# Li-Yuetao/ActiveSplat

Measured on AMD Instinct MI355X. Metric: render+backward frames/sec at 640x480, N Gaussians, higher is better.
Workload: dtype f32; 1 GPU; BASELINE configs[2]'s render (the north star's target configuration): 2000000 Gaussians, SH degree 3, 640x480, forward (colour+radii+depth+opacity) + backward (all input gradients), frames strictly one after the other; gaussians=2000000, sh_degree=3, width=640, height=480, tile_instances_D=4842856, streams=1, parallelism=single GPU

## Files before the change

activesplat_amd/_lib.py:

```python
from __future__ import annotations

import ctypes as C
import os

_HERE = os.path.dirname(os.path.abspath(__file__))
LIB_PATH = os.path.join(_HERE, "libgsplat_hip.so")

_lib = None
_emulated = False


class GsCamera(C.Structure):
    _fields_ = [("image_width", C.c_int32), ("image_height", C.c_int32), ("sh_degree", C.c_int32),
                ("sh_coeffs", C.c_int32), ("tanfovx", C.c_float), ("tanfovy", C.c_float),
                ("scale_modifier", C.c_float), ("num_views", C.c_int32), ("bg", C.c_void_p),
                ("viewmatrix", C.c_void_p), ("projmatrix", C.c_void_p), ("campos", C.c_void_p)]


class GsGeomLayout(C.Structure):
    _fields_ = [(n, C.c_uint64) for n in ("total_bytes", "geom", "rect", "tiles_touched", "offsets", "block_sums", "clamped",
                                          "tile_total", "tile_base", "sh_jac", "depth_bits")]


class GsImageLayout(C.Structure):
    _fields_ = [(n, C.c_uint64) for n in ("total_bytes", "ranges", "final_T", "n_contrib", "split_state")]


class GsAdamTensor(C.Structure):
    _fields_ = [("n", C.c_int64), ("param", C.c_void_p), ("grad", C.c_void_p), ("exp_avg", C.c_void_p), ("exp_avg_sq", C.c_void_p),
                ("lr", C.c_double), ("beta1", C.c_double), ("beta2", C.c_double), ("eps", C.c_double), ("step", C.c_int32),
                ("reserved", C.c_int32)]


class GsRowTensor(C.Structure):
    _fields_ = [("param", C.c_void_p), ("exp_avg", C.c_void_p), ("exp_avg_sq", C.c_void_p), ("grad", C.c_void_p),
                ("lr", C.c_double), ("beta1", C.c_double), ("beta2", C.c_double), ("eps", C.c_double), ("width", C.c_int32),
                ("step", C.c_int32)]


class GsBinLayout(C.Structure):
    _fields_ = [(n, C.c_uint64) for n in ("total_bytes", "path", "pairs", "keys_unsorted", "vals_unsorted", "keys_sorted",
                                          "sort_temp", "segments", "seg_T", "pairs_alt")]


class GsDbscanLayout(C.Structure):
    _fields_ = [(n, C.c_uint64) for n in ("total_bytes", "mask_bits", "core_bits", "root_bits", "word_prefix", "parent", "root", "row_range")]


class GsEvalLayout(C.Structure):
    _fields_ = [("total_bytes", C.c_uint64), ("ms_ssim_defined", C.c_int32), ("levels", C.c_int32), ("level_width", C.c_int32 * 5),
                ("level_height", C.c_int32 * 5)]


class GsHullLayout(C.Structure):
    _fields_ = [(n, C.c_uint64) for n in ("total_bytes", "cluster_status")]


class GsMeshLayout(C.Structure):
    _fields_ = [(n, C.c_uint64) for n in ("total_bytes", "total", "records", "rects", "tile_count", "tile_offset", "list")]


class GsImageGrads(C.Structure):
    _fields_ = [(n, C.c_void_p) for n in ("dL_dcolor", "dL_ddepth", "dL_dopacity", "dL_ddepth_sq")]


SORT_AUTO, SORT_TILE_LDS, SORT_RADIX = 0, 1, 2


ABI_VERSION = 23

vp, i32, u32, i64, u64, f32, f64, cint = C.c_void_p, C.c_int32, C.c_uint32, C.c_int64, C.c_uint64, C.c_float, C.c_double, C.c_int

BINDINGS = {
    "gs_atlas_layout": (cint, [i32, i32, i32, C.POINTER(i32), C.POINTER(i32), C.POINTER(i32)]),
    "gs_geom_layout": (cint, [i32, i32, i32, C.POINTER(GsGeomLayout)]),
    "gs_image_layout": (cint, [i32, i32, C.POINTER(GsImageLayout)]),
    "gs_bin_layout": (cint, [i64, u32, i32, i32, C.POINTER(GsBinLayout)]),
    "gs_set_sort_path": (cint, [i32]),
    "gs_set_forward_segments": (cint, [i32]),
    "gs_set_half_quadrants": (cint, [i32]),
    "gs_set_backward_chain": (cint, [i32, i32]),
    "gs_set_backward_chain_tickets": (cint, [i32]),
    "gs_set_backward_chain_polls": (cint, [i32]),
    "gs_set_forward_priority": (cint, [i32, f32]),
    "gs_async_status_word": (cint, [C.POINTER(C.POINTER(u32))]),
    "gs_async_status_clear": (cint, []),
    "gs_recorded_cut": (cint, [u32, C.POINTER(u32), C.POINTER(i32)]),
    "gs_set_backward_segments": (cint, [i32]),
    "gs_backward_scratch_bytes": (u64, [i32]),
    "gs_last_error": (C.c_char_p, []),
    "gs_version": (C.c_char_p, []),
    "gs_abi_version": (i32, []),
    "gs_profile_enable": (cint, [i32]),
    "gs_profile_stage_count": (i32, []),
    "gs_profile_stage_name": (C.c_char_p, [i32]),
    "gs_profile_collect": (cint, [vp, vp, i32]),
    "gs_preprocess_forward": (cint, [C.POINTER(GsCamera), i32] + [vp] * 12 + [i32, vp]),
    "gs_render_forward": (cint, [C.POINTER(GsCamera), i32, i64, u32] + [vp] * 10),
    "gs_render_backward": (cint, [C.POINTER(GsCamera), i32, i64] + [vp] * 21 + [i32, i32, vp]),
    "gs_preprocess_forward_raw": (cint, [C.POINTER(GsCamera), i32] + [vp] * 7 + [i32] + [vp] * 7 + [i32, vp]),
    "gs_render_backward_raw": (cint, [C.POINTER(GsCamera), i32, i64] + [vp] * 7 + [i32, i32] + [vp] * 14 + [i32, i32, vp]),
    "gs_pose_grad_scratch_bytes": (u64, [i32]),
    "gs_render_backward_raw_pose": (cint, [C.POINTER(GsCamera), i32, i64] + [vp] * 7 + [i32, i32] + [vp] * 14 + [i32, i32, i32, vp, vp, vp]),
    "gs_render_backward_grads": (cint, [C.POINTER(GsCamera), i32, i64] + [vp] * 10 + [C.POINTER(GsImageGrads)] + [vp] * 9 + [i32, i32, vp]),
    "gs_render_backward_raw_grads": (cint, [C.POINTER(GsCamera), i32, i64] + [vp] * 7 + [i32, i32] + [vp] * 4 + [C.POINTER(GsImageGrads)] + [vp] * 8 + [i32, i32, vp]),
    "gs_render_backward_raw_pose_grads": (cint, [C.POINTER(GsCamera), i32, i64] + [vp] * 7 + [i32, i32] + [vp] * 4 + [C.POINTER(GsImageGrads)] + [vp] * 8 + [i32, i32, i32, vp, vp, vp]),
    "gs_adam_step": (cint, [i64] + [vp] * 4 + [f64] * 4 + [i32, vp]),
    "gs_adam_step_multi": (cint, [i32, C.POINTER(GsAdamTensor), vp]),
    "gs_render_backward_raw_adam": (cint, [C.POINTER(GsCamera), i32, i64] + [vp] * 7 + [i32] + [vp] * 8 + [i32, i32, C.POINTER(GsAdamTensor), vp]),
    "gs_pack_columns": (cint, [i32, C.POINTER(GsRowTensor), i64, i64, vp, vp]),
    "gs_adam_rows": (cint, [i32, C.POINTER(GsRowTensor), i64, i64, i64, vp, vp, vp]),
    "gs_unpack_columns": (cint, [i32, C.POINTER(GsRowTensor), i64, vp, vp]),
    "gs_activate_forward": (cint, [i32, i32] + [vp] * 10),
    "gs_activate_backward": (cint, [i32, i32] + [vp] * 13),
    "gs_activate_backward_accumulate": (cint, [i32, i32] + [vp] * 13),
    "gs_activate_backward_pose": (cint, [i32, i32] + [vp] * 13 + [i32, i32, vp, vp, vp]),
    "gs_mapping_loss_scratch_bytes": (u64, [i32, i32]),
    "gs_mapping_loss": (cint, [i32, i32] + [vp] * 5 + [f32, f32] + [vp] * 4 + [i64, vp]),
    "gs_depth_error_median_scratch_bytes": (u64, [i32, i32]),
    "gs_depth_error_median": (cint, [i32, i32] + [vp] * 5),
    "gs_depth_error_median_grid": (cint, [i32, i32] + [vp] * 4 + [i32, vp]),
    "gs_depth_error_median_workgroups": (i32, [i32, i32]),
    "gs_mapping_loss_outlier": (cint, [i32, i32] + [vp] * 5 + [f32, f32] + [vp] * 4 + [i64, vp, vp]),
    "gs_tracking_loss_scratch_bytes": (u64, [i32, i32]),
    "gs_tracking_loss": (cint, [i32, i32] + [vp] * 6 + [i32, f32, f32, f32] + [vp] * 5),
    "gs_tracking_loss_outlier": (cint, [i32, i32] + [vp] * 6 + [i32, f32, f32, f32] + [vp] * 6),
    "gs_preprocess_forward_raw_dev": (cint, [C.POINTER(GsCamera), i32] + [vp] * 8 + [i64, i64, i32] + [vp] * 7 + [i32, vp]),
    "gs_preprocess_forward_topdown": (cint, [C.POINTER(GsCamera), i32] + [vp] * 5 + [i32, f32, f32] + [vp] * 6),
    "gs_render_forward_topdown": (cint, [C.POINTER(GsCamera), i32, i64, u32] + [vp] * 9),
    "gs_render_backward_raw_pose_dev": (cint, [C.POINTER(GsCamera), i32, i64] + [vp] * 8 + [i64, i64, i32] + [vp] * 8 + [i32, i32, vp, vp, vp]),
    "gs_tracking_state_bytes": (u64, []),
    "gs_tracking_begin": (cint, [vp, vp, i64, i64, vp, vp]),
    "gs_tracking_step": (cint, [i32, vp, i32, i32, vp, f32, f32, vp, vp, i64, i64, f64, f64, i32, vp, vp, vp]),
    "gs_compact_scratch_bytes": (u64, [i64]),
    "gs_compact_index": (cint, [i64] + [vp] * 5),
    "gs_gather_rows": (cint, [i64, i32] + [vp] * 4),
    "gs_gather_rows_zero_tail": (cint, [i64, i64, i32] + [vp] * 4),
    "gs_densify_classify": (cint, [i32, i32] + [vp] * 5 + [f32, f32, i32, i32] + [vp] * 5),
    "gs_densify_children": (cint, [i32, i32, i32, vp, vp, u64, vp, vp, vp]),
    "gs_compact3_scratch_bytes": (u64, [i64]),
    "gs_compact_index3": (cint, [i64, vp, vp, vp, i32] + [vp] * 4),
    "gs_visibility_stats": (cint, [i32] + [vp] * 4),
    "gs_accumulate_grad2d": (cint, [i32] + [vp] * 5),
    "gs_grid_dbscan_layout": (cint, [i32] * 4 + [C.POINTER(GsDbscanLayout)]),
    "gs_grid_dbscan": (cint, [i32, i32, i32, vp, i64, i64, f32] + [i32] * 4 + [vp] * 7),
    "gs_cluster_hulls_layout": (cint, [i32] * 5 + [C.POINTER(GsHullLayout)]),
    "gs_cluster_hulls": (cint, [i32, i32, i32, vp, vp, i64, i64, vp, vp, i32, C.POINTER(u32), i32, i32, f32, f64, f64, i32] + [vp] * 8),
    "gs_high_loss_grid": (cint, [i32, i32, vp, vp, vp, f32, f32, i32, i32, vp, vp, vp]),
    "gs_grow_scratch_bytes": (u64, [i32, i32]),
    "gs_grow_gaussians": (cint, [i32, i32] + [vp] * 6 + [f32, i32] + [vp] * 8),
    "gs_keyframe_overlap": (cint, [i32, vp, i32, vp, vp, i32, i32, i32, vp, vp]),
    "gs_frame_ingest": (cint, [i32, i32, vp, vp, vp, i32, C.POINTER(i32)] + [vp] * 5),
    "gs_mesh_render_layout": (cint, [i32, i32, i32, u32, C.POINTER(GsMeshLayout)]),
    "gs_mesh_render": (cint, [i32, vp, i32, vp, vp, C.POINTER(f32), C.POINTER(f32), f32, i32, i32, vp, u32, vp, vp, vp, vp, vp]),
    "gs_depth_cloud": (cint, [i32, i32, vp, C.POINTER(f32), C.POINTER(f32), vp, vp, vp]),
    "gs_cloud_nearest_scratch_bytes": (u64, [i64, i64]),
    "gs_cloud_nearest": (cint, [i64, vp, vp, i64, vp, vp, i32, vp, vp, vp]),
    "gs_completion_row_scratch_bytes": (u64, []),
    "gs_completion_row": (cint, [i64, vp, i64, vp, vp, f64, vp, vp, vp]),
    "gs_eval_frame_layout": (cint, [i32, i32, i32, C.POINTER(GsEvalLayout)]),
    "gs_eval_frame": (cint, [i32, i32] + [vp] * 5 + [f32, i32, vp, vp, vp]),
}

SYMBOLS = tuple(BINDINGS)


def _bind(lib):
# ... 95 lines not shown
```

activesplat_amd/csrc/api.hip:

```cpp
#include <stdio.h>
#include <string.h>

#include <mutex>

#include "gs_common.h"

namespace {

thread_local char g_err[512] = "";

int fail(int code, const char* fmt, const char* a = "")
{
    snprintf(g_err, sizeof(g_err), fmt, a);
    return code;
}

int launched(const char* who, const char* what, hipError_t e)
{
    if (e == hipSuccess) return GS_OK;
    snprintf(g_err, sizeof(g_err), "%s: %s%s%s", who, what, *what ? " " : "", hipGetErrorString(e));
    return GS_ELAUNCH;
}

bool adam_aligned16(const void* p, const void* g, const void* m, const void* v)
{
    return (((uintptr_t)p | (uintptr_t)g | (uintptr_t)m | (uintptr_t)v) & 15u) == 0;
}

int fail_adam_alignment(const char* who, int tensor)
{
    snprintf(g_err, sizeof(g_err), "%s: tensor %d: param / grad / exp_avg / exp_avg_sq must be 16-byte aligned (the kernel makes 128-bit accesses)", who, tensor);
    return GS_EINVAL;
}

uint64_t align_up(uint64_t v, uint64_t a = 256) { return (v + a - 1) / a * a; }

enum Stage { ST_PREPROCESS = 0, ST_TILE_COUNT, ST_EMIT, ST_SORT, ST_RANGES, ST_TILE_SCATTER_SORT, ST_BLEND_FWD, ST_BLEND_BWD, ST_PREPROCESS_BWD, ST_ADAM, ST_COUNT };
const char* kStageNames[ST_COUNT] = {"preprocess_forward+scan", "tile_count+scan", "emit", "sort", "ranges",
                                     "tile_scatter+sort", "blend_forward", "blend_backward", "preprocess_backward", "adam"};
std::atomic<int> g_sort_path{GS_SORT_AUTO};
std::atomic<bool> g_segments_enabled{true};

int choose_path(int tiles, uint32_t max_tile_instances)
{
    const bool fits = tiles <= gs::kMaxLdsTiles && max_tile_instances <= 65535u * (uint32_t)gs::kSortChunk;
    if (g_sort_path == GS_SORT_RADIX) return GS_SORT_RADIX;
    return fits ? GS_SORT_TILE_LDS : GS_SORT_RADIX;
}
constexpr int kMaxPairs = 8192;
struct Prof {
    bool on = false;
    int n = 0;
    hipEvent_t ev[kMaxPairs][2];
    int stage[kMaxPairs];
    int created = 0;
} g_prof;

struct ScopedStage {
    int idx = -1;
    hipStream_t st;
    ScopedStage(int stage, hipStream_t s) : st(s)
    {
        if (!g_prof.on || g_prof.n >= kMaxPairs) return;
        idx = g_prof.n++;
        if (idx >= g_prof.created) { (void)hipEventCreate(&g_prof.ev[idx][0]); (void)hipEventCreate(&g_prof.ev[idx][1]); g_prof.created = idx + 1; }
        g_prof.stage[idx] = stage;
        (void)hipEventRecord(g_prof.ev[idx][0], st);
    }
    ~ScopedStage() { if (idx >= 0) (void)hipEventRecord(g_prof.ev[idx][1], st); }
};

int tile_bits(int tiles)
{
    int b = 1;
    while ((1 << b) < tiles) b++;
    return b;
}

int32_t tiles_across(int32_t pixels) { return (pixels + gs::kTile - 1) / gs::kTile; }
uint64_t tiles_of(int32_t width, int32_t height) { return (uint64_t)tiles_across(width) * tiles_across(height); }
int32_t atlas_view_stride(int32_t view_width, int32_t V) { return V > 1 ? tiles_across(view_width) * gs::kTile : view_width; }
int32_t blocks_of(int32_t P) { return (P + gs::kBlock - 1) / gs::kBlock; }
int32_t virtual_rows(int32_t P, int32_t V) { return V > 1 ? V * blocks_of(P) * gs::kBlock : P; }

bool make_cam(const GsCamera* c, gs::Cam& k)
{
    if (!c || c->image_width <= 0 || c->image_height <= 0 || !c->bg || !c->viewmatrix || !c->projmatrix) return false;
    if (!(c->tanfovx > 0.f) || !(c->tanfovy > 0.f)) return false;
    if (c->num_views < 0 || c->num_views > 64) return false;
    k.V = c->num_views > 1 ? c->num_views : 1;
    k.Wv = c->image_width; k.H = c->image_height;
    k.gxv = tiles_across(k.Wv);
    k.gx = k.V * k.gxv; k.gy = tiles_across(k.H);
    k.W = k.V * atlas_view_stride(k.Wv, k.V);
    k.nbv = 0;
    if (k.gx >= 65536 || k.gy >= 65536) return false;
    k.tanfovx = c->tanfovx; k.tanfovy = c->tanfovy;
    k.fx = (float)k.Wv / (2.0f * c->tanfovx); k.fy = (float)k.H / (2.0f * c->tanfovy);
    k.mod = c->scale_modifier;
    k.sh_degree = c->sh_degree; k.sh_coeffs = c->sh_coeffs;
    k.bg = c->bg; k.view = c->viewmatrix; k.proj = c->projmatrix; k.campos = c->campos;
    k.half = 0; k.split = 0;
    k.act = k.act_iso = k.act_accumulate = 0;
    return true;
}

int32_t virtual_count(gs::Cam& k, int32_t P)
{
    k.nbv = blocks_of(P);
    return virtual_rows(P, k.V);
}

gs::GeomPtrs carve_geom(void* base, int32_t P, const gs::Cam& k)
{
    GsGeomLayout L;
    gs_geom_layout(P, k.W, k.H, &L);
    char* b = (char*)base;
    gs::GeomPtrs g;
    g.geom = (float4*)(b + L.geom); g.rect = (uint2*)(b + L.rect); g.tiles = (uint32_t*)(b + L.tiles_touched);
    g.offsets = (uint32_t*)(b + L.offsets); g.block_sums = (uint32_t*)(b + L.block_sums);
    g.clamped = (uint32_t*)(b + L.clamped);
    g.tile_total = (uint32_t*)(b + L.tile_total); g.tile_base = (uint32_t*)(b + L.tile_base);
    g.sh_jac = (float2*)(b + L.sh_jac);
    g.depth_bits = (uint32_t*)(b + L.depth_bits);
    g.vis_max = nullptr; g.vis_seen = nullptr;
    return g;
}

}

extern "C" {

const char* gs_last_error(void) { return g_err; }
const char* gs_version(void) { return "activesplat_amd gsplat_hip 0.4 (gfx950)"; }
int32_t gs_abi_version(void) { return GS_ABI_VERSION; }

int gs_profile_enable(int32_t on)
{
    g_prof.on = on != 0;
    g_prof.n = 0;
    return GS_OK;
}

int32_t gs_profile_stage_count(void) { return ST_COUNT; }

const char* gs_profile_stage_name(int32_t stage) { return stage >= 0 && stage < ST_COUNT ? kStageNames[stage] : ""; }

int gs_profile_collect(float* ms_sum, int32_t* calls, int32_t n_stages)
{
    if (!ms_sum || !calls || n_stages < ST_COUNT) return fail(GS_EINVAL, "gs_profile_collect: bad argument");
    for (int i = 0; i < n_stages; i++) { ms_sum[i] = 0.f; calls[i] = 0; }
    for (int i = 0; i < g_prof.n; i++) {
        if (hipEventSynchronize(g_prof.ev[i][1]) != hipSuccess) return fail(GS_ELAUNCH, "gs_profile_collect: event sync failed");
        float ms = 0.f;
        if (hipEventElapsedTime(&ms, g_prof.ev[i][0], g_prof.ev[i][1]) != hipSuccess) return fail(GS_ELAUNCH, "gs_profile_collect: elapsed failed");
        ms_sum[g_prof.stage[i]] += ms; calls[g_prof.stage[i]]++;
    }
    g_prof.n = 0;
    return GS_OK;
}

int gs_set_sort_path(int32_t path)
{
    if (path < GS_SORT_AUTO || path > GS_SORT_RADIX) return fail(GS_EINVAL, "gs_set_sort_path: bad path");
    g_sort_path = path;
    return GS_OK;
}

int gs_set_half_quadrants(int32_t max_tiles)
{
    gs::g_half_quadrant_tiles = max_tiles < 0 ? 0 : max_tiles;
    return GS_OK;
}

int gs_set_backward_chain(int32_t pieces, int32_t min_tiles)
{
    if (pieces < 1 || pieces > gs::kChainPieces) return fail(GS_EINVAL, "gs_set_backward_chain: pieces out of range");
    gs::g_chain_pieces = pieces;
    gs::g_chain_min_tiles = min_tiles < 0 ? gs::kChainMinTiles : min_tiles;
    return GS_OK;
}

int gs_set_backward_chain_tickets(int32_t on)
{
    gs::g_chain_tickets = on != 0;
    return GS_OK;
}

int gs_set_backward_chain_polls(int32_t polls)
{
    gs::g_chain_polls = polls == -1 ? gs::kChainPollsDefault : polls;
    return GS_OK;
}

int gs_set_forward_priority(int32_t mode, float param)
{
    if (mode > gs::kFwdPrioChunk) return fail(GS_EINVAL, "gs_set_forward_priority: mode out of range");
    if (mode == gs::kFwdPrioT && param >= 1.0f) return fail(GS_EINVAL, "gs_set_forward_priority: a transmittance threshold lies below 1");
    if (mode < 0) { mode = gs::kFwdPrioDefault; param = gs::kFwdPrioDefaultParam; }
    gs::g_fwd_prio_param = param > 0.0f ? param : 0.0f;
    gs::g_fwd_prio = mode;
    return GS_OK;
}

int gs_async_status_word(uint32_t** host_word)
{
    static uint32_t* word = nullptr;
    static std::mutex mu;
    std::lock_guard<std::mutex> lock(mu);
    if (!word) {
        void* h = nullptr;
        if (hipHostMalloc(&h, 64, hipHostMallocMapped | hipHostMallocPortable) != hipSuccess) {
            (void)hipGetLastError();
            return fail(GS_ELAUNCH, "gs_async_status_word: hipHostMalloc failed");
        }
        memset(h, 0, 64);
        void* d = nullptr;
        if (hipHostGetDevicePointer(&d, h, 0) != hipSuccess) { (void)hipGetLastError(); return fail(GS_ELAUNCH, "gs_async_status_word: no device view of the host word"); }
        void* f = nullptr;
        if (hipMalloc(&f, 64) == hipSuccess && hipMemset(f, 0, 64) == hipSuccess && hipGetDevice(&gs::g_chain_fail_device) == hipSuccess) gs::g_chain_fail_dev = (uint32_t*)f;
        else (void)hipGetLastError();
        word = (uint32_t*)h;
        gs::g_async_status_dev = (uint32_t*)d;
    }
    if (host_word) *host_word = word;
    return GS_OK;
}

int gs_async_status_clear(void)
{
    if (hipDeviceSynchronize() != hipSuccess) { (void)hipGetLastError(); return fail(GS_ELAUNCH, "gs_async_status_clear: device synchronisation failed"); }
    if (gs::g_chain_fail_dev && hipMemset(gs::g_chain_fail_dev, 0, 4) != hipSuccess) { (void)hipGetLastError(); return fail(GS_ELAUNCH, "gs_async_status_clear: hipMemset failed"); }
    return GS_OK;
}

int gs_recorded_cut(uint32_t target, uint32_t* nearest, int32_t* level)
{
    const uint32_t pos = gs::cut_nearest(target);
    if (nearest) *nearest = pos;
    if (level) *level = pos ? gs::cut_level(pos) : -1;
    return GS_OK;
}

int gs_set_backward_segments(int32_t segments)
{
    if (segments < 1 || segments > gs::kFewSegmentsMax) return fail(GS_EINVAL, "gs_set_backward_segments: 1, 2 or 3");
    gs::g_few_segments = segments;
    return GS_OK;
}

int gs_set_forward_segments(int32_t on)
{
    g_segments_enabled = on != 0;
    return GS_OK;
}

int gs_atlas_layout(int32_t P, int32_t view_width, int32_t num_views, int32_t* virtual_P, int32_t* atlas_width, int32_t* view_stride)
{
    if (P < 0 || view_width <= 0 || num_views < 1 || num_views > 64) return fail(GS_EINVAL, "gs_atlas_layout: bad argument");
    const int32_t stride = atlas_view_stride(view_width, num_views);
    if (virtual_P) *virtual_P = virtual_rows(P, num_views);
    if (atlas_width) *atlas_width = num_views * stride;
    if (view_stride) *view_stride = stride;
    return GS_OK;
}

int gs_geom_layout(int32_t P, int32_t width, int32_t height, GsGeomLayout* out)
{
    if (!out || P < 0 || width <= 0 || height <= 0) return fail(GS_EINVAL, "gs_geom_layout: bad argument");
    const uint64_t n = (uint64_t)(P > 0 ? P : 1);
    const uint64_t nb = (n + gs::kBlock - 1) / gs::kBlock;
    const uint64_t tiles = tiles_of(width, height);
    const uint64_t rows = (n + 1023) / 1024;
    uint64_t o = 0;
    out->geom = o; o = align_up(o + n * GS_GEOM_FLOATS * 4);
    out->rect = o; o = align_up(o + n * 8);
    out->tiles_touched = o; o = align_up(o + n * 4);
    out->offsets = o; o = align_up(o + n * 4);
    out->block_sums = o; o = align_up(o + (nb + 1) * 4);
    out->clamped = o; o = align_up(o + n * 4);
    out->tile_total = o; o = align_up(o + tiles * 4);
    out->tile_base = o; o = align_up(o + (tiles <= (uint64_t)gs::kMaxLdsTiles ? rows * tiles * 4 : 4));
    out->sh_jac = o; o = align_up(o + n * gs::kShJacFloats * 4);
    out->depth_bits = o; o = align_up(o + n * 4);
    out->total_bytes = o;
    return GS_OK;
}

int gs_image_layout(int32_t width, int32_t height, GsImageLayout* out)
{
    if (!out || width <= 0 || height <= 0) return fail(GS_EINVAL, "gs_image_layout: bad argument");
    const uint64_t tiles = tiles_of(width, height);
    const uint64_t hw = (uint64_t)width * height;
    uint64_t o = 0;
    out->ranges = o; o = align_up(o + tiles * 8);
    out->final_T = o; o = align_up(o + hw * 4);
    out->n_contrib = o; o = align_up(o + hw * 4);
    out->split_state = o; o = align_up(o + (tiles <= (uint64_t)gs::kFewTiles ? ((uint64_t)gs::kCutLevels * 5 + 4) * hw + 4
                                             : (uint64_t)gs::chain_state_words(tiles)) * 4);
    out->total_bytes = o;
    return GS_OK;
}

int gs_bin_layout(int64_t D, uint32_t max_tile_instances, int32_t width, int32_t height, GsBinLayout* out)
{
    if (!out || D < 0 || width <= 0 || height <= 0) return fail(GS_EINVAL, "gs_bin_layout: bad argument");
    const int tiles = (int)tiles_of(width, height);
    const uint64_t n = (uint64_t)(D > 0 ? D : 1);
    memset(out, 0, sizeof(*out));
    out->path = (uint64_t)choose_path(tiles, max_tile_instances);
    uint64_t o = 0;
    if (out->path == GS_SORT_TILE_LDS) {
        out->pairs = o; o = align_up(o + n * 8);
        if (max_tile_instances > (uint32_t)gs::kSortCapMax) { out->pairs_alt = o; o = align_up(o + n * 8); }
    } else {
        out->keys_unsorted = o; o = align_up(o + n * 8);
        out->vals_unsorted = o; o = align_up(o + n * 4);
        out->keys_sorted = o; o = align_up(o + n * 8);
        out->sort_temp = o; o = align_up(o + gs::sort_temp_bytes(D, 32 + tile_bits(tiles)));
    }
    out->segments = 1;
    const bool few_tiles = tiles * 4 * 8 <= gs::kWaveSlots && max_tile_instances >= 8192;
    const bool long_lists = tiles * 4 * 2 <= gs::kWaveSlots && max_tile_instances >= 32768;
    if (g_segments_enabled && max_tile_instances != 0xffffffffu && (few_tiles || long_lists)) {
        uint64_t S = 3 * (uint64_t)gs::kWaveSlots / ((uint64_t)tiles * 4);
        const uint64_t by_len = max_tile_instances / 1024;
        if (S > by_len) S = by_len;
        if (S > 32) S = 32;
        if (S >= 2) { out->segments = S; out->seg_T = o; o = align_up(o + (uint64_t)tiles * S * gs::kBlock * 4 + (uint64_t)tiles * 16); }
    }
    out->total_bytes = o;
    return GS_OK;
}

uint64_t gs_backward_scratch_bytes(int32_t P) { return align_up((uint64_t)(P > 0 ? P : 1) * gs::kGradStride * 4); }

static void set_input_activation(gs::Cam& k, const gs::PoseRequest& pose, int32_t isotropic, int32_t accumulate)
{
    static const float world[7] = {1.f, 0.f, 0.f, 0.f, 0.f, 0.f, 0.f};
    const float* p = pose.source == gs::POSE_HOST ? pose.pose7 : world;
    k.act = pose.source != gs::POSE_NONE;
    k.act_iso = k.act && isotropic != 0; k.act_accumulate = k.act && accumulate != 0;
    for (int c = 0; c < 4; c++) k.act_q[c] = p[c];
    for (int c = 0; c < 3; c++) k.act_t[c] = p[4 + c];
}

static bool dev_pose(const float* cam_unnorm_rots, const float* cam_trans, int64_t num_frames, int64_t time_idx, gs::DevPose& dp)
{
    if (!cam_unnorm_rots || !cam_trans || num_frames < 1 || time_idx < 0 || time_idx >= num_frames) return false;
    dp.q = cam_unnorm_rots + time_idx; dp.t = cam_trans + time_idx; dp.stride = num_frames;
    return true;
}

static gs::CamDP with_dev_pose(const gs::Cam& k, const gs::DevPose& dp)
{
    gs::CamDP kd;
    static_cast<gs::Cam&>(kd) = k;
    kd.dev_q = dp.q; kd.dev_t = dp.t; kd.stride = dp.stride;
    return kd;
}

struct ForwardCall {
    int32_t P;
    gs::GaussianInputs in;
    gs::PoseRequest pose;
    int32_t isotropic;
    float* max_2D_radius; uint8_t* seen;
    int32_t* radii;
    void* geom_state; void* image_state;
    uint32_t* d_counts; uint32_t* h_counts;
    int32_t want_backward;
};

static int preprocess_forward_impl(const GsCamera* cam, const ForwardCall& c, gs_stream_t stream)
{
    const gs::GaussianInputs& in = c.in;
    const int32_t P = c.P;
    gs::Cam k;
    if (!make_cam(cam, k)) return fail(GS_EINVAL, "gs_preprocess_forward: invalid camera settings");
    set_input_activation(k, c.pose, c.isotropic, 0);
    if (k.act && k.V != 1) return fail(GS_EINVAL, "gs_preprocess_forward_raw: one view only");
    if (k.act && (in.cov3D || (in.shs && k.sh_coeffs != 16)))
        return fail(GS_EINVAL, "gs_preprocess_forward_raw: scale / rotation parameters with colours or 16-coefficient SH rows only");
    if (P < 0 || !c.geom_state || !c.image_state || !c.d_counts) return fail(GS_EINVAL, "gs_preprocess_forward: null state pointer");
    if (P > 0 && (!in.means3D || !in.opac || !c.radii)) return fail(GS_EINVAL, "gs_preprocess_forward: null input pointer");
    if ((in.shs == nullptr) == (in.colors == nullptr) && P > 0)
        return fail(GS_EINVAL, "Please provide excatly one of either SHs or precomputed colors!");
    const bool have_sr = in.scales != nullptr && in.rots != nullptr;
    if (P > 0 && (have_sr == (in.cov3D != nullptr) || ((in.scales != nullptr) != (in.rots != nullptr))))
        return fail(GS_EINVAL, "Please provide exactly one of either scale/rotation pair or precomputed 3D covariance!");
    if (in.shs && (k.sh_degree < 0 || k.sh_degree > 3 || k.sh_coeffs < (k.sh_degree + 1) * (k.sh_degree + 1) || k.sh_coeffs > 16 || !k.campos))
        return fail(GS_EINVAL, "gs_preprocess_forward: sh_degree / sh_coeffs / campos inconsistent");
    hipStream_t st = (hipStream_t)stream;
    const int32_t Pv = virtual_count(k, P);
    gs::GeomPtrs gp = carve_geom(c.geom_state, Pv, k);
    if (!(c.want_backward && in.shs)) gp.sh_jac = nullptr;
    gp.vis_max = k.act ? c.max_2D_radius : nullptr; gp.vis_seen = k.act ? c.seen : nullptr;
    GsImageLayout IL; gs_image_layout(k.W, k.H, &IL);
    uint2* ranges = (uint2*)((char*)c.image_state + IL.ranges);
    const int tiles = k.gx * k.gy;
    hipError_t e;
    {
        ScopedStage ps(ST_PREPROCESS, st);
        if (c.pose.source == gs::POSE_BAND) {
            gs::CamBand kb;
            static_cast<gs::Cam&>(kb) = k;
            kb.band_upper = c.pose.band_upper; kb.band_lower = c.pose.band_lower;
            e = gs::launch_preprocess_forward(kb, P, in, c.radii, gp, st);
        } else if (c.pose.source == gs::POSE_DEVICE)
            e = gs::launch_preprocess_forward(with_dev_pose(k, c.pose.dev), P, in, c.radii, gp, st);
        else
            e = gs::launch_preprocess_forward(k, P, in, c.radii, gp, st);
    }
    if (int rc = launched("gs_preprocess_forward", "", e)) return rc;
    bool mirrored = false;
    if (tiles <= gs::kMaxLdsTiles) {
        uint32_t* host_dev = nullptr;
        if (c.h_counts && hipHostGetDevicePointer((void**)&host_dev, c.h_counts, 0) != hipSuccess) { host_dev = nullptr; (void)hipGetLastError(); }
        mirrored = host_dev != nullptr;
        ScopedStage ps(ST_TILE_COUNT, st);
        e = gs::launch_tile_count(k, Pv, gp, gp.tile_total, gp.tile_base, ranges, c.d_counts, host_dev, st);
        if (int rc = launched("gs_preprocess_forward", "tile count", e)) return rc;
    } else {
        e = gs::launch_scan_block_sums(Pv, gp, c.d_counts, st);
        if (int rc = launched("gs_preprocess_forward", "scan", e)) return rc;
        e = hipMemsetAsync(c.d_counts + 1, 0xff, sizeof(uint32_t), st);
        if (int rc = launched("gs_preprocess_forward", "memset", e)) return rc;
    }
    if (c.h_counts && !mirrored) {
        e = hipMemcpyAsync(c.h_counts, c.d_counts, 2 * sizeof(uint32_t), hipMemcpyDeviceToHost, st);
        if (int rc = launched("gs_preprocess_forward", "D2H", e)) return rc;
    }
    return GS_OK;
}

int gs_preprocess_forward(const GsCamera* cam, int32_t P, const float* means3D, const float* shs,
                          const float* colors_precomp, const float* opacities, const float* scales,
                          const float* rotations, const float* cov3D_precomp, int32_t* radii, void* geom_state,
                          void* image_state, uint32_t* d_counts, uint32_t* h_counts, int32_t want_backward, gs_stream_t stream)
{
    ForwardCall c{};
    c.in.means3D = means3D; c.in.shs = shs; c.in.colors = colors_precomp; c.in.opac = opacities; c.in.scales = scales; c.in.rots = rotations;
    c.in.cov3D = cov3D_precomp; c.P = P;
    c.radii = radii; c.geom_state = geom_state; c.image_state = image_state; c.d_counts = d_counts; c.h_counts = h_counts; c.want_backward = want_backward;
    return preprocess_forward_impl(cam, c, stream);
}

int gs_preprocess_forward_raw(const GsCamera* cam, int32_t P, const float* means3D, const float* shs, const float* colors_precomp,
                              const float* logit_opacities, const float* log_scales, const float* unnorm_rotations,
                              const float* h_pose7, int32_t isotropic, float* max_2D_radius, uint8_t* seen, int32_t* radii, void* geom_state,
                              void* image_state, uint32_t* d_counts, uint32_t* h_counts, int32_t want_backward, gs_stream_t stream)
{
    if (!h_pose7) return fail(GS_EINVAL, "gs_preprocess_forward_raw: null pose");
    ForwardCall c{};
    c.in.means3D = means3D; c.in.shs = shs; c.in.colors = colors_precomp; c.in.opac = logit_opacities; c.in.scales = log_scales; c.in.rots = unnorm_rotations;
    c.P = P; c.pose.source = gs::POSE_HOST; c.pose.pose7 = h_pose7; c.isotropic = isotropic; c.max_2D_radius = max_2D_radius; c.seen = seen;
    c.radii = radii; c.geom_state = geom_state; c.image_state = image_state; c.d_counts = d_counts; c.h_counts = h_counts; c.want_backward = want_backward;
    return preprocess_forward_impl(cam, c, stream);
}

int gs_preprocess_forward_raw_dev(const GsCamera* cam, int32_t P, const float* means3D, const float* shs, const float* colors_precomp,
                                  const float* logit_opacities, const float* log_scales, const float* unnorm_rotations,
                                  const float* cam_unnorm_rots, const float* cam_trans, int64_t num_frames, int64_t time_idx, int32_t isotropic,
                                  float* max_2D_radius, uint8_t* seen, int32_t* radii, void* geom_state, void* image_state, uint32_t* d_counts,
                                  uint32_t* h_counts, int32_t want_backward, gs_stream_t stream)
{
    ForwardCall c{};
    c.pose.source = gs::POSE_DEVICE;
    if (!dev_pose(cam_unnorm_rots, cam_trans, num_frames, time_idx, c.pose.dev))
        return fail(GS_EINVAL, "gs_preprocess_forward_raw_dev: null pose columns or time index outside [0, num_frames)");
    if (P > 0 && (!log_scales || !unnorm_rotations)) return fail(GS_EINVAL, "gs_preprocess_forward_raw_dev: null scale / rotation parameters");
    c.in.means3D = means3D; c.in.shs = shs; c.in.colors = colors_precomp; c.in.opac = logit_opacities; c.in.scales = log_scales; c.in.rots = unnorm_rotations;
    c.P = P; c.isotropic = isotropic; c.max_2D_radius = max_2D_radius; c.seen = seen;
    c.radii = radii; c.geom_state = geom_state; c.image_state = image_state; c.d_counts = d_counts; c.h_counts = h_counts; c.want_backward = want_backward;
    return preprocess_forward_impl(cam, c, stream);
}

static int bin_tile_lists(const char* who, const gs::Cam& k, int32_t P, int64_t D, uint32_t max_tile_instances, gs::GeomPtrs gp, uint2* ranges,
                          const GsBinLayout& BL, char* bb, uint32_t* point_list, hipStream_t st)
{
    hipError_t e;
    if (BL.path == GS_SORT_TILE_LDS) {
        if (D > 0) {
            ScopedStage ps(ST_TILE_SCATTER_SORT, st);
            e = gs::launch_tile_scatter_sort(k, P, gp, gp.tile_base, ranges, max_tile_instances,
                                             (unsigned long long*)(bb + BL.pairs), (unsigned long long*)(bb + BL.pairs_alt), point_list, (uint32_t)D, st);
            if (int rc = launched(who, "tile scatter/sort", e)) return rc;
        }
    } else {
        e = hipMemsetAsync(ranges, 0, (size_t)k.gx * k.gy * 8, st);
        if (int rc = launched(who, "memset", e)) return rc;
        if (k.gx * k.gy <= gs::kMaxLdsTiles) {
            e = gs::launch_scan_block_sums(P, gp, gp.block_sums + (P + gs::kBlock - 1) / gs::kBlock, st);
            if (int rc = launched(who, "scan", e)) return rc;
        }
        if (D == 0) {
            e = gs::launch_emit(k, P, gp, nullptr, nullptr, st);
            if (int rc = launched(who, "emit", e)) return rc;
        } else {
            uint64_t* ku = (uint64_t*)(bb + BL.keys_unsorted); uint32_t* vu = (uint32_t*)(bb + BL.vals_unsorted);
            uint64_t* ks = (uint64_t*)(bb + BL.keys_sorted);
            { ScopedStage ps(ST_EMIT, st); e = gs::launch_emit(k, P, gp, ku, vu, st); }
            if (int rc = launched(who, "emit", e)) return rc;
            const int end_bit = 32 + tile_bits(k.gx * k.gy);
            {
                ScopedStage ps(ST_SORT, st);
                e = gs::sort_pairs(bb + BL.sort_temp, (size_t)(BL.total_bytes - BL.sort_temp), ku, ks, vu, point_list, D, end_bit, st);
            }
            if (int rc = launched(who, "sort", e)) return rc;
            { ScopedStage ps(ST_RANGES, st); e = gs::launch_ranges(D, ks, ranges, st); }
            if (int rc = launched(who, "ranges", e)) return rc;
        }
    }
    return GS_OK;
}

int gs_render_forward(const GsCamera* cam, int32_t P, int64_t D, uint32_t max_tile_instances, void* geom_state,
                      void* bin_state, uint32_t* point_list, void* image_state, float* out_color, float* out_depth,
                      float* out_opacity, float* out_depth_sq, void* backward_scratch, gs_stream_t stream)
{
    gs::Cam k;
    if (!make_cam(cam, k)) return fail(GS_EINVAL, "gs_render_forward: invalid camera settings");
    if (P < 0 || D < 0 || !geom_state || !image_state || !out_color || !out_depth || !out_opacity)
        return fail(GS_EINVAL, "gs_render_forward: null pointer");
    if (D > 0 && (!bin_state || !point_list)) return fail(GS_EINVAL, "gs_render_forward: null binning workspace");
    if (D >= (int64_t)1 << 32) return fail(GS_ECAPACITY, "gs_render_forward: more than 2^32 tile instances");
    hipStream_t st = (hipStream_t)stream;
    const int32_t Pin = P;
    P = virtual_count(k, Pin);
    gs::GeomPtrs gp = carve_geom(geom_state, P, k);
    GsImageLayout IL; gs_image_layout(k.W, k.H, &IL);
    char* ib = (char*)image_state;
    uint2* ranges = (uint2*)(ib + IL.ranges);
    GsBinLayout BL; gs_bin_layout(D, max_tile_instances, k.W, k.H, &BL);
    char* bb = (char*)bin_state;
    if (int rc = bin_tile_lists("gs_render_forward", k, P, D, max_tile_instances, gp, ranges, BL, bb, point_list, st)) return rc;
    ScopedStage ps(ST_BLEND_FWD, st);
    return launched("gs_render_forward", "blend", gs::launch_blend_forward(k, ranges, point_list, gp.geom, out_color, out_depth, out_opacity,
                    (float*)(ib + IL.final_T), (uint32_t*)(ib + IL.n_contrib), out_depth_sq, BL.path == GS_SORT_TILE_LDS ? (uint32_t)D : 0xffffffffu,
                    (int)BL.segments, BL.segments > 1 ? (float*)(bb + BL.seg_T) : nullptr, (float*)(ib + IL.split_state), (uint32_t)P,
                    (float*)backward_scratch, st));
}

int gs_preprocess_forward_topdown(const GsCamera* cam, int32_t P, const float* means3D, const float* colors_precomp, const float* logit_opacities,
                                  const float* log_scales, const float* unnorm_rotations, int32_t isotropic, float band_upper, float band_lower,
                                  int32_t* radii, void* geom_state, void* image_state, uint32_t* d_counts, uint32_t* h_counts, gs_stream_t stream)
{
    if (cam && cam->num_views > 1) return fail(GS_EINVAL, "gs_preprocess_forward_topdown: one view only");
    if (P > 0 && (!colors_precomp || !log_scales || !unnorm_rotations))
        return fail(GS_EINVAL, "gs_preprocess_forward_topdown: null colour / scale / rotation parameters");
    if (band_upper != band_upper || band_lower != band_lower) return fail(GS_EINVAL, "gs_preprocess_forward_topdown: NaN height band");
    ForwardCall c{};
    c.in.means3D = means3D; c.in.colors = colors_precomp; c.in.opac = logit_opacities; c.in.scales = log_scales; c.in.rots = unnorm_rotations;
    c.P = P; c.pose.source = gs::POSE_BAND; c.pose.band_upper = band_upper; c.pose.band_lower = band_lower; c.isotropic = isotropic;
    c.radii = radii; c.geom_state = geom_state; c.image_state = image_state; c.d_counts = d_counts; c.h_counts = h_counts;
    return preprocess_forward_impl(cam, c, stream);
}

int gs_render_forward_topdown(const GsCamera* cam, int32_t P, int64_t D, uint32_t max_tile_instances, void* geom_state, void* bin_state,
                              uint32_t* point_list, void* image_state, float* free_opacity, uint8_t* free_map_binary, uint8_t* visible_rgb,
                              uint8_t* visible_map_binary, gs_stream_t stream)
{
    gs::Cam k;
    if (!make_cam(cam, k)) return fail(GS_EINVAL, "gs_render_forward_topdown: invalid camera settings");
    if (k.V != 1) return fail(GS_EINVAL, "gs_render_forward_topdown: one view only");
    if (P < 0 || D < 0 || !geom_state || !image_state || !free_opacity || !free_map_binary || !visible_rgb || !visible_map_binary)
        return fail(GS_EINVAL, "gs_render_forward_topdown: null pointer");
    if (((uintptr_t)free_map_binary | (uintptr_t)visible_rgb | (uintptr_t)visible_map_binary | (uintptr_t)free_opacity) & 3)
        return fail(GS_EINVAL, "gs_render_forward_topdown: output maps must be 4-byte aligned");
    if (D > 0 && (!bin_state || !point_list)) return fail(GS_EINVAL, "gs_render_forward_topdown: null binning workspace");
    if (D >= (int64_t)1 << 32) return fail(GS_ECAPACITY, "gs_render_forward_topdown: more than 2^32 tile instances");
    hipStream_t st = (hipStream_t)stream;
    virtual_count(k, P);
    gs::GeomPtrs gp = carve_geom(geom_state, P, k);
    GsImageLayout IL; gs_image_layout(k.W, k.H, &IL);
    uint2* ranges = (uint2*)((char*)image_state + IL.ranges);
    GsBinLayout BL; gs_bin_layout(D, max_tile_instances, k.W, k.H, &BL);
    if (int rc = bin_tile_lists("gs_render_forward_topdown", k, P, D, max_tile_instances, gp, ranges, BL, (char*)bin_state, point_list, st)) return rc;
    ScopedStage ps(ST_BLEND_FWD, st);
    return launched("gs_render_forward_topdown", "blend", gs::launch_blend_topdown(k, ranges, point_list, gp.geom, free_opacity, free_map_binary, visible_rgb,
                    visible_map_binary, BL.path == GS_SORT_TILE_LDS ? (uint32_t)D : 0xffffffffu, (uint32_t)P, st));
}

struct BackwardCall {
    int32_t P;
    int64_t D;
    gs::GaussianBackward g;
    gs::PoseRequest pose;
    int32_t isotropic, accumulate;
    const void* geom_state; const uint32_t* point_list; const void* image_state;
    const float* dL_dcolor; const float* dL_ddepth;
    const float* dL_dopacity; const float* dL_ddepth_sq;
    void* scratch; int32_t scratch_zeroed, have_sh_jacobian;
    const GsAdamTensor* adam5;
};

static int render_backward_impl(const GsCamera* cam, const BackwardCall& c, gs_stream_t stream)
{
    gs::GaussianBackward g = c.g;
    const gs::GaussianInputs& in = g.in;
    const gs::GaussianGrads& out = g.out;
    const gs::PoseRequest& pose = c.pose;
    const int32_t P = c.P;
    const bool pose_only = pose.grad == gs::POSE_GRAD_ONLY;
    gs::Cam k;
    if (!make_cam(cam, k)) return fail(GS_EINVAL, "gs_render_backward: invalid camera settings");
    set_input_activation(k, pose, c.isotropic, pose_only ? 0 : c.accumulate);
    if (k.act && k.V != 1) return fail(GS_EINVAL, "gs_render_backward_raw: one view only");
    if (k.act && (!in.opac || in.cov3D || (in.shs && k.sh_coeffs != 16)))
        return fail(GS_EINVAL, "gs_render_backward_raw: scale / rotation parameters with colours or 16-coefficient SH rows only");
    if (k.V > 1) return fail(GS_EINVAL, "gs_render_backward: multi-view atlas renders are forward-only");
    if (P < 0 || c.D < 0 || !c.geom_state || !c.image_state || !c.dL_dcolor || !c.scratch)
        return fail(GS_EINVAL, "gs_render_backward: null pointer");
    if (pose.grad && (!k.act || c.adam5 || (!pose.dL_dpose7 && pose.source != gs::POSE_DEVICE) || !pose.pose_scratch))
        return fail(GS_EINVAL, "gs_render_backward_raw_pose: raw-parameter mode with a pose-gradient output and its scratch only");
    if (pose.source == gs::POSE_DEVICE && !pose_only) return fail(GS_EINVAL, "gs_render_backward_raw_pose_dev: the pose-only backward only");
    if ((c.dL_dopacity || c.dL_ddepth_sq) && (c.adam5 || pose.source == gs::POSE_DEVICE))
        return fail(GS_EINVAL, "gs_render_backward: opacity / depth_sq gradients have no optimiser-step or device-pose form");
    if (P == 0) {
        if (pose.grad && pose.dL_dpose7)
            return launched("gs_render_backward_raw_pose", "memset", hipMemsetAsync(pose.dL_dpose7, 0, 7 * sizeof(float), (hipStream_t)stream));
        return GS_OK;
    }
    gs::FusedAdam fa{};
    if (c.adam5) {
        if (!k.act || c.accumulate) return fail(GS_EINVAL, "gs_render_backward_raw_adam: raw-parameter mode without accumulation only");
        if (!in.means3D || !g.radii || !out.dmeans2D || !in.scales || !in.rots || (in.shs == nullptr) == (in.colors == nullptr))
            return fail(GS_EINVAL, "gs_render_backward_raw_adam: null input/output pointer");
        if (in.shs && !c.have_sh_jacobian) return fail(GS_EINVAL, "gs_render_backward_raw_adam: SH rows need the forward's saved Jacobian (have_sh_jacobian = 1)");
        const float* par[5] = {in.means3D, in.opac, in.scales, in.rots, in.shs ? in.shs : in.colors};
        const int64_t width[5] = {3, 1, c.isotropic ? 1 : 3, 4, in.shs ? 48 : 3};
        for (int t = 0; t < 5; ++t) {
            const GsAdamTensor& a = c.adam5[t];
            if (a.param != par[t] || !a.exp_avg || !a.exp_avg_sq || a.step < 1 || a.n != width[t] * (int64_t)P)
                return fail(GS_EINVAL, "gs_render_backward_raw_adam: descriptor of %s does not describe the input tensor (param / moments / n / step)",
                            t == 0 ? "means3D" : t == 1 ? "logit_opacities" : t == 2 ? "log_scales" : t == 3 ? "unnorm_rotations" : "the colours");
            if (P > 0 && (t == 3 || (t == 4 && in.shs)) && !adam_aligned16(a.param, a.param, a.exp_avg, a.exp_avg_sq))
                return fail_adam_alignment("gs_render_backward_raw_adam", t);
            fa.p[t] = a.param; fa.m[t] = a.exp_avg; fa.v[t] = a.exp_avg_sq;
            fa.c[t] = gs::adam_coef(a.lr, a.beta1, a.beta2, a.eps, a.step);
        }
        fa.fail = gs::chain_fail_word();
        g.adam = &fa;
    } else if (pose_only) {
        if (!in.means3D || !g.radii || !out.dmeans2D || !in.scales || !in.rots || (in.shs == nullptr) == (in.colors == nullptr))
            return fail(GS_EINVAL, "gs_render_backward_raw_pose: null input/output pointer");
    } else {
        if (!in.means3D || !g.radii || !out.dmeans2D || !out.dmeans3D || !out.dopac)
            return fail(GS_EINVAL, "gs_render_backward: null input/output pointer");
        if (in.shs ? !out.dshs : !out.dcolors) return fail(GS_EINVAL, "gs_render_backward: missing colour gradient output");
        if (in.cov3D ? !out.dcov3D : (!in.scales || !in.rots || !out.dscales || !out.drots))
            return fail(GS_EINVAL, "gs_render_backward: missing covariance inputs/outputs");
    }
    hipStream_t st = (hipStream_t)stream;
    gs::GeomPtrs gp = carve_geom(const_cast<void*>(c.geom_state), P, k);
    GsImageLayout IL; gs_image_layout(k.W, k.H, &IL);
    const char* ib = (const char*)c.image_state;
    float* grad2d = (float*)c.scratch;
    hipError_t e = c.scratch_zeroed ? hipSuccess : hipMemsetAsync(grad2d, 0, (size_t)P * gs::kGradStride * 4, st);
    if (int rc = launched("gs_render_backward", "memset", e)) return rc;
    if (c.D > 0) {
        ScopedStage ps(ST_BLEND_BWD, st);
        e = gs::launch_blend_backward(k, (const uint2*)(ib + IL.ranges), c.point_list, gp.geom,
                                      (const float*)(ib + IL.split_state),
                                      (const float*)(ib + IL.final_T),
                                      (const uint32_t*)(ib + IL.n_contrib), c.dL_dcolor, c.dL_ddepth, grad2d, st, c.dL_dopacity, c.dL_ddepth_sq);
        if (int rc = launched("gs_render_backward", "blend", e)) return rc;
    }
    g.clamped = gp.clamped; g.sh_jac = (in.shs && c.have_sh_jacobian) ? gp.sh_jac : nullptr; g.grad2d = grad2d;
    {
        ScopedStage ps(ST_PREPROCESS_BWD, st);
        if (pose.source == gs::POSE_DEVICE) e = gs::launch_preprocess_backward(with_dev_pose(k, pose.dev), P, g, pose, st);
        else e = gs::launch_preprocess_backward(k, P, g, pose, st);
    }
    if (int rc = launched("gs_render_backward", "preprocess", e)) return rc;
    const int64_t pose_rows = gs::pose_rows_count(P);
    if (pose.source == gs::POSE_DEVICE) {
        if (pose.dL_dpose7)
            return launched("gs_render_backward_raw_pose_dev", "pose reduction", gs::launch_pose_grad_finish_dev(pose_rows, pose.dev.q, pose.dev.stride,
                            (const float*)pose.pose_scratch, pose.dL_dpose7, st));
    } else if (pose.grad)
        return launched("gs_render_backward_raw_pose", "pose reduction", gs::launch_pose_grad_finish(pose_rows, pose.pose7, (const float*)pose.pose_scratch,
                        pose.dL_dpose7, st));
    return GS_OK;
}

int gs_render_backward_grads(const GsCamera* cam, int32_t P, int64_t D, const float* means3D, const float* shs,
                       const float* colors_precomp, const float* scales, const float* rotations,
                       const float* cov3D_precomp, const int32_t* radii, const void* geom_state,
                       const uint32_t* point_list, const void* image_state, const GsImageGrads* grads, float* dL_dmeans2D, float* dL_dmeans3D, float* dL_dopacities, float* dL_dcolors_precomp,
                       float* dL_dshs, float* dL_dscales, float* dL_drotations, float* dL_dcov3D, void* scratch,
                       int32_t scratch_zeroed, int32_t have_sh_jacobian, gs_stream_t stream)
{
    if (!grads) return fail(GS_EINVAL, "gs_render_backward_grads: null image-gradient block");
    BackwardCall c{};
    c.P = P; c.D = D;
    c.g.in.means3D = means3D; c.g.in.shs = shs; c.g.in.colors = colors_precomp; c.g.in.scales = scales; c.g.in.rots = rotations; c.g.in.cov3D = cov3D_precomp;
    c.g.radii = radii; c.geom_state = geom_state; c.point_list = point_list; c.image_state = image_state; c.dL_dcolor = grads->dL_dcolor; c.dL_ddepth = grads->dL_ddepth; c.dL_dopacity = grads->dL_dopacity; c.dL_ddepth_sq = grads->dL_ddepth_sq;
    c.g.out.dmeans2D = dL_dmeans2D; c.g.out.dmeans3D = dL_dmeans3D; c.g.out.dopac = dL_dopacities; c.g.out.dcolors = dL_dcolors_precomp;
    c.g.out.dshs = dL_dshs; c.g.out.dscales = dL_dscales; c.g.out.drots = dL_drotations; c.g.out.dcov3D = dL_dcov3D;
    c.scratch = scratch; c.scratch_zeroed = scratch_zeroed; c.have_sh_jacobian = have_sh_jacobian;
    return render_backward_impl(cam, c, stream);
}

int gs_render_backward(const GsCamera* cam, int32_t P, int64_t D, const float* means3D, const float* shs,
                       const float* colors_precomp, const float* scales, const float* rotations,
                       const float* cov3D_precomp, const int32_t* radii, const void* geom_state,
                       const uint32_t* point_list, const void* image_state, const float* dL_dcolor,
                       const float* dL_ddepth, float* dL_dmeans2D, float* dL_dmeans3D, float* dL_dopacities, float* dL_dcolors_precomp,
                       float* dL_dshs, float* dL_dscales, float* dL_drotations, float* dL_dcov3D, void* scratch,
                       int32_t scratch_zeroed, int32_t have_sh_jacobian, gs_stream_t stream)
{
    const GsImageGrads grads{dL_dcolor, dL_ddepth, nullptr, nullptr};
    return gs_render_backward_grads(cam, P, D, means3D, shs, colors_precomp, scales, rotations, cov3D_precomp, radii, geom_state, point_list, image_state, &grads, dL_dmeans2D, dL_dmeans3D, dL_dopacities, dL_dcolors_precomp, dL_dshs, dL_dscales, dL_drotations, dL_dcov3D, scratch, scratch_zeroed, have_sh_jacobian, stream);
}

int gs_render_backward_raw_grads(const GsCamera* cam, int32_t P, int64_t D, const float* means3D, const float* shs, const float* colors_precomp,
                           const float* logit_opacities, const float* log_scales, const float* unnorm_rotations, const float* h_pose7,
                           int32_t isotropic, int32_t accumulate, const int32_t* radii, const void* geom_state, const uint32_t* point_list,
                           const void* image_state, const GsImageGrads* grads, float* dL_dmeans2D, float* dL_dmeans3D,
                           float* dL_dlogit_opacities, float* dL_dcolors_precomp, float* dL_dshs, float* dL_dlog_scales,
                           float* dL_dunnorm_rotations, void* scratch, int32_t scratch_zeroed, int32_t have_sh_jacobian, gs_stream_t stream)
{
    if (!grads) return fail(GS_EINVAL, "gs_render_backward_raw_grads: null image-gradient block");
    if (!h_pose7 || (P > 0 && !logit_opacities)) return fail(GS_EINVAL, "gs_render_backward_raw: null pose / opacity parameters");
    BackwardCall c{};
    c.g.in.means3D = means3D; c.g.in.shs = shs; c.g.in.colors = colors_precomp; c.g.in.opac = logit_opacities; c.g.in.scales = log_scales; c.g.in.rots = unnorm_rotations;
    c.P = P; c.D = D; c.pose.source = gs::POSE_HOST; c.pose.pose7 = h_pose7; c.isotropic = isotropic; c.accumulate = accumulate;
    c.g.radii = radii; c.geom_state = geom_state; c.point_list = point_list; c.image_state = image_state; c.dL_dcolor = grads->dL_dcolor; c.dL_ddepth = grads->dL_ddepth; c.dL_dopacity = grads->dL_dopacity; c.dL_ddepth_sq = grads->dL_ddepth_sq;
    c.g.out.dmeans2D = dL_dmeans2D; c.g.out.dmeans3D = dL_dmeans3D; c.g.out.dopac = dL_dlogit_opacities; c.g.out.dcolors = dL_dcolors_precomp;
    c.g.out.dshs = dL_dshs; c.g.out.dscales = dL_dlog_scales; c.g.out.drots = dL_dunnorm_rotations;
    c.scratch = scratch; c.scratch_zeroed = scratch_zeroed; c.have_sh_jacobian = have_sh_jacobian;
    return render_backward_impl(cam, c, stream);
}

int gs_render_backward_raw(const GsCamera* cam, int32_t P, int64_t D, const float* means3D, const float* shs, const float* colors_precomp,
                           const float* logit_opacities, const float* log_scales, const float* unnorm_rotations, const float* h_pose7,
                           int32_t isotropic, int32_t accumulate, const int32_t* radii, const void* geom_state, const uint32_t* point_list,
                           const void* image_state, const float* dL_dcolor, const float* dL_ddepth, float* dL_dmeans2D, float* dL_dmeans3D,
                           float* dL_dlogit_opacities, float* dL_dcolors_precomp, float* dL_dshs, float* dL_dlog_scales,
                           float* dL_dunnorm_rotations, void* scratch, int32_t scratch_zeroed, int32_t have_sh_jacobian, gs_stream_t stream)
{
    const GsImageGrads grads{dL_dcolor, dL_ddepth, nullptr, nullptr};
    return gs_render_backward_raw_grads(cam, P, D, means3D, shs, colors_precomp, logit_opacities, log_scales, unnorm_rotations, h_pose7, isotropic, accumulate, radii, geom_state, point_list, image_state, &grads, dL_dmeans2D, dL_dmeans3D, dL_dlogit_opacities, dL_dcolors_precomp, dL_dshs, dL_dlog_scales, dL_dunnorm_rotations, scratch, scratch_zeroed, have_sh_jacobian, stream);
}
// ... 669 lines not shown
```

activesplat_amd/csrc/blend.hip:

```cpp
#include "gs_common.h"
#include <atomic>

namespace gs {

constexpr int kFwdStreams = 4;

constexpr float kAlphaMin = 1.0f / 255.0f;
constexpr float kTmin = 0.0001f;
constexpr float kLog2e = 1.4426950408889634f;
constexpr uint32_t kNoId = 0xffffffffu;

struct TileCtx {
    int tile, tx, ty, px, py, quad, seg;
    float qx0, qy0, pxf, pyf;
    bool inside;
};

template <int NW>
__device__ __forceinline__ bool tile_ctx_at(const Cam& cam, unsigned block, int wave, int lane, TileCtx& c, int segments = 0)
{
    const int G = (segments > 1 ? 4 * segments : 4) / NW;
    const int ntiles = cam.gx * cam.gy, per = (ntiles + 7) >> 3;
    const int idx = (int)(block >> 3);
    c.tile = (int)(block & 7) * per + idx / G;
// ... 143 lines not shown
template <bool DEPTH_SQ>
__device__ __forceinline__ void store_pixel_outputs(const Cam& cam, int px, int py, float T, uint32_t last, float C0, float C1, float C2, float Dp, float Dq,
                                                    float* out_color, float* out_depth, float* out_opacity, float* final_T, uint32_t* n_contrib,
                                                    float* out_depth_sq)
{
    const size_t pix = (size_t)py * cam.W + px, HW = (size_t)cam.H * cam.W;
    final_T[pix] = T;
    n_contrib[pix] = last;
    out_color[pix] = C0 + T * cam.bg[0];
    out_color[HW + pix] = C1 + T * cam.bg[1];
    out_color[2 * HW + pix] = C2 + T * cam.bg[2];
    out_depth[pix] = Dp;
    out_opacity[pix] = 1.0f - T;
    if (DEPTH_SQ) out_depth_sq[pix] = Dq;
}
__device__ __forceinline__ void set_wave_priority(int level)
{
    level = __builtin_amdgcn_readfirstlane(level);
    if (level >= 3) __builtin_amdgcn_s_setprio(3);
    else if (level == 2) __builtin_amdgcn_s_setprio(2);
    else if (level == 1) __builtin_amdgcn_s_setprio(1);
    else __builtin_amdgcn_s_setprio(0);
}
constexpr int kRoundSlack = 4;

template <bool DEPTH_SQ, int NS, int SEG, int NW>
__global__ __launch_bounds__(NW * kWave) void blend_forward_streams_kernel(
    Cam cam, const uint2* __restrict__ ranges, const uint32_t* __restrict__ point_list,
    const float4* __restrict__ geom, float* __restrict__ out_color, float* __restrict__ out_depth,
    float* __restrict__ out_opacity, float* __restrict__ final_T, uint32_t* __restrict__ n_contrib,
    float* __restrict__ out_depth_sq, uint32_t cap, float* __restrict__ seg_T, float* __restrict__ split_state, uint32_t P,
    float4* __restrict__ zero_fill)
{
    static_assert(NS == 4 && kWave / NS == 16, "the scan tests the four 4x4 blocks of a quadrant");
    __shared__ float4 s_rec[NW][3][kWave + 1];
    __shared__ __attribute__((aligned(16))) uint8_t s_list[NW][4 * kWave + 16];
    const int tid = threadIdx.x, lane = tid & 63, wave = tid >> 6;
    GradFill fill = grad_fill_start(SEG == 0 ? zero_fill : nullptr, P, tid);
    TileCtx c;
    if (SEG == 0 && cam.chain > 1 && split_state && blockIdx.x == 0 && tid < 8)
        reinterpret_cast<uint32_t*>(split_state)[(size_t)cam.gx * cam.gy * 4 * (kChainStateFloats + kChainPieces - 1) + (size_t)tid * kChainTicketStride] = 0u;
    if (!tile_ctx_nw<NW>(cam, wave, lane, c)) { if (SEG == 0) grad_fill_rest(zero_fill, fill, NW * kWave); return; }
    if (SEG == 0 && cam.chain > 1 && split_state && lane < kChainPieces - 1)
        reinterpret_cast<uint32_t*>(split_state)[(size_t)cam.gx * cam.gy * 4 * kChainStateFloats + (size_t)(c.tile * 4 + c.quad) * (kChainPieces - 1) + lane] = 0u;
    const StreamPixel sp = stream_pixel(cam, c.qx0, c.qy0, lane);
    const int px = sp.px, py = sp.py;
    const bool inside = sp.inside;
    const float pxf = sp.pxf, pyf = sp.pyf;
    float4* s0 = s_rec[wave][0]; float4* s1 = s_rec[wave][1]; float4* s2 = s_rec[wave][2];
    write_sentinel(s0, s1, s2, lane);
    uint8_t* my_list = s_list[wave] + sp.sid * kWave;
    uint2 range = ranges[c.tile];
    range.x = min(range.x, cap); range.y = min(range.y, cap);
    const uint32_t n_all = range.y - range.x;
    const uint32_t* list = point_list + range.x;
    uint32_t first = 0, n = n_all;
    float T = 1.0f;
    bool next_stopped = true;
    float* my_seg_T = nullptr;
    uint32_t* seg_flag = nullptr;
    if (SEG != 0) {
        const uint32_t S = gridDim.y, seg = blockIdx.y;
        const uint32_t L = (((n_all + S - 1) / S + kWave - 1) / kWave) * kWave;
        first = min(n_all, seg * L);
        n = min(n_all, first + L);
        float* tile_T = seg_T + ((size_t)c.tile * S) * kBlock + c.quad * kWave + lane;
        my_seg_T = tile_T + (size_t)seg * kBlock;
        if (SEG == 1) {
            seg_flag = reinterpret_cast<uint32_t*>(seg_T + (size_t)cam.gx * cam.gy * S * kBlock) + c.tile * 4 + c.quad;
            const uint32_t f = __hip_atomic_load(seg_flag, __ATOMIC_RELAXED, __HIP_MEMORY_SCOPE_AGENT);
            if (f & ((1u << seg) - 1u)) { my_seg_T[0] = 1.0f; return; }
        }
        if (SEG == 2) {
            for (uint32_t q = 0; q < seg; q++) T *= tile_T[(size_t)q * kBlock];
            next_stopped = seg + 1 == S ? true : (T * my_seg_T[0] < kTmin);
        }
    }
    float C0 = 0.f, C1 = 0.f, C2 = 0.f, Dp = 0.f, Dq = 0.f;
    uint32_t last = 0;
    const bool stopped_at_entry = SEG == 2 && T < kTmin;
    bool done = !inside || stopped_at_entry;

    if (SEG == 1 || !__all(done)) {
        uint32_t id_next = first + (uint32_t)lane < n ? list[first + lane] : kNoId;
        uint32_t id_next2 = first + (uint32_t)lane + 64u < n ? list[first + lane + 64] : kNoId;
        if (id_next >= P) id_next = kNoId;
        if (id_next2 >= P) id_next2 = kNoId;
        float4 r0 = make_float4(0.f, 0.f, 0.f, 0.f), r1 = r0, r2 = make_float4(0.f, 0.f, -1.f, -1.f);
        if (first < n) {
            const float4* gr = geom + (size_t)(id_next != kNoId ? id_next : 0u) * 3;
            r0 = gr[0]; r1 = gr[1]; r2 = gr[2];
        }
        for (uint32_t base = first; base < n; base += kWave) {
            if (SEG == 0) fill = grad_fill_step(zero_fill, fill, NW * kWave);
            if (SEG == 0 && cam.fwd_prio != kFwdPrioOff) {
                const float chunks = (float)((base - first) >> 6);
                const float p = cam.fwd_prio_param;
                int level;
                if (cam.fwd_prio == kFwdPrioChunk) {
                    level = (chunks >= p ? 1 : 0) + (chunks >= 2.0f * p ? 1 : 0) + (chunks >= 3.0f * p ? 1 : 0);
                } else {
                    float t1 = p, t2 = p * p, t3 = p * p * p;
                    if (cam.fwd_prio == kFwdPrioDecay) {
                        constexpr float kLog2Tmin = -13.287712f;
                        t1 = __builtin_amdgcn_exp2f(kLog2Tmin * chunks * __builtin_amdgcn_rcpf(chunks + p));
                        t2 = __builtin_amdgcn_exp2f(kLog2Tmin * chunks * __builtin_amdgcn_rcpf(chunks + 2.0f * p));
                        t3 = __builtin_amdgcn_exp2f(kLog2Tmin * chunks * __builtin_amdgcn_rcpf(chunks + 4.0f * p));
                    }
                    level = (__ballot(!done && T > t1) != 0ull ? 1 : 0) + (__ballot(!done && T > t2) != 0ull ? 1 : 0) +
                            (__ballot(!done && T > t3) != 0ull ? 1 : 0);
                    const uint32_t left = (n - base) >> 6;
                    level = min(level, (left > kFwdPrioListChunks ? 1 : 0) + (left > 2u * kFwdPrioListChunks ? 1 : 0) + (left > 3u * kFwdPrioListChunks ? 1 : 0));
                }
                set_wave_priority(level);
            }
            const float4 q0 = r0, q1 = r1, q2 = r2;
            const uint32_t id_cur = id_next;
            id_next = id_next2;
            id_next2 = base + 128u + (uint32_t)lane < n ? list[base + 128u + lane] : kNoId;
            if (id_next2 >= P) id_next2 = kNoId;
            {
                const float4* gr = geom + (size_t)(id_next != kNoId ? id_next : 0u) * 3;
                r0 = gr[0]; r1 = gr[1]; r2 = gr[2];
            }

            const unsigned long long going = SEG == 1 ? ~0ull : ~__ballot(done);
            unsigned long long m_any, mb[4];
            scan_going_blocks(q0, q2, id_cur != kNoId, c.qx0, c.qy0, going, m_any, mb);
            if (m_any == 0ull) continue;
            stage_record(s0, s1, s2, lane, q0, q1, q2, id_cur);
            const int ntrips = build_stream_lists(s_list[wave], mb, lane);
            __builtin_amdgcn_wave_barrier();
            uint32_t jj2_next = *reinterpret_cast<const uint16_t*>(my_list);
            int lj = -1;
            for (int t = 0; t < ntrips; t += 2) {
                const uint32_t jj2 = jj2_next;
                jj2_next = *reinterpret_cast<const uint16_t*>(my_list + t + 2);
                const int jj[2] = {(int)(jj2 & 0xffu), (int)(jj2 >> 8)};
                float4 a0[2], a1[2], a2[2];
#pragma unroll
                for (int u = 0; u < 2; u++) { a0[u] = s0[jj[u]]; a1[u] = s1[jj[u]]; a2[u] = s2[jj[u]]; }
#pragma unroll
                for (int u = 0; u < 2; u++) {
                    const SplatAlpha a = splat_alpha(a0[u], a1[u].x, a1[u].y, pxf, pyf);
                    if (SEG == 1) {
                        T = a.hit ? T * (1.0f - a.alpha) : T;
                        continue;
                    }
                    const Composite k = composite_step(T, done, a.alpha, a.hit);
                    T = k.T; done = k.done;
                    C0 += a1[u].z * k.w; C1 += a1[u].w * k.w; C2 += a2[u].x * k.w; Dp += a2[u].y * k.w;
                    if (DEPTH_SQ) Dq += a2[u].y * a2[u].y * k.w;
                    lj = k.ok ? jj[u] : lj;
                }
            }
            last = lj >= 0 ? base + (uint32_t)lj + 1u : last;
            __builtin_amdgcn_wave_barrier();
            if (SEG != 1 && __all(done)) break;
            if (SEG == 1 && __all(!inside || T < kTmin)) break;
        }
        if (SEG == 0 && cam.fwd_prio != kFwdPrioOff) __builtin_amdgcn_s_setprio(0);
    }
    if (SEG == 0) grad_fill_rest(zero_fill, fill, NW * kWave);
    if (SEG == 1) {
        my_seg_T[0] = T;
        if (__all(!inside || T < kTmin) && lane == 0) atomicOr(seg_flag, 1u << blockIdx.y);
        return;
    }
    if (SEG == 2) {
        if (inside && !stopped_at_entry) {
            const size_t pix = (size_t)py * cam.W + px, HW = (size_t)cam.H * cam.W;
            const float tb = next_stopped ? T : 0.0f;
            atomicAdd(out_color + pix, C0 + tb * cam.bg[0]);
            atomicAdd(out_color + HW + pix, C1 + tb * cam.bg[1]);
            atomicAdd(out_color + 2 * HW + pix, C2 + tb * cam.bg[2]);
            atomicAdd(out_depth + pix, Dp);
            if (DEPTH_SQ) atomicAdd(out_depth_sq + pix, Dq);
            if (last) atomicMax(n_contrib + pix, last);
            if (next_stopped) { final_T[pix] = T; out_opacity[pix] = 1.0f - T; }
        }
        return;
    }
    if (inside) store_pixel_outputs<DEPTH_SQ>(cam, px, py, T, last, C0, C1, C2, Dp, Dq, out_color, out_depth, out_opacity, final_T, n_contrib, out_depth_sq);
}

__host__ __device__ __forceinline__ uint32_t rgb_to_grey_u8(uint32_t r, uint32_t g, uint32_t b)
{
    return (4899u * r + 9617u * g + 1868u * b + 8192u) >> 14;
}
__device__ __forceinline__ uint32_t unit_to_u8(float c)
{
    return (uint32_t)(fminf(fmaxf(c, 0.0f), 1.0f) * 255.0f);
}

__global__ __launch_bounds__(kBlock) void blend_topdown_kernel(
    Cam cam, const uint2* __restrict__ ranges, const uint32_t* __restrict__ point_list, const float4* __restrict__ geom,
    float* __restrict__ free_opacity, uint8_t* __restrict__ free_binary, uint8_t* __restrict__ visible_rgb, uint8_t* __restrict__ visible_binary,
    uint32_t cap, uint32_t P)
{
    constexpr int NW = 4;
    static_assert(kFwdStreams == 4, "the scan tests the four 4x4 blocks of a quadrant");
    __shared__ float4 s_rec[NW][3][kWave + 1];
    __shared__ __attribute__((aligned(16))) uint8_t s_list[NW][4 * kWave + 16];
    const int tid = threadIdx.x, lane = tid & 63, wave = tid >> 6;
    TileCtx c;
    if (!tile_ctx_nw<NW>(cam, wave, lane, c)) return;
    const StreamPixel sp = stream_pixel(cam, c.qx0, c.qy0, lane);
    const int px = sp.px, py = sp.py, l = sp.l;
    const bool inside = sp.inside;
    const float pxf = sp.pxf, pyf = sp.pyf;
    float4* s0 = s_rec[wave][0]; float4* s1 = s_rec[wave][1]; float4* s2 = s_rec[wave][2];
    write_sentinel(s0, s1, s2, lane);
    uint8_t* my_list = s_list[wave] + sp.sid * kWave;
// ... 328 lines not shown
    uint32_t wmax = last;
#pragma unroll
    for (int m = 32; m >= 1; m >>= 1) wmax = max(wmax, (uint32_t)__shfl_xor(wmax, m));
    if (wmax == 0) return;
    uint32_t seg_lo = 0u, seg_hi = wmax;
    int k_hi = -1;
    if (nseg > 1) {
        const bool recorded = split_state && reinterpret_cast<const uint32_t*>(split_state + (kCutLevels * 5 + 4) * HW)[0] == 1u;
        uint32_t cut1 = recorded ? cut_nearest((uint32_t)((unsigned long long)wmax / (unsigned)nseg)) : 0u;
        if (cut1 >= wmax) cut1 = 0u;
        uint32_t cut2 = (recorded && nseg > 2) ? cut_nearest((uint32_t)((unsigned long long)wmax * 2u / (unsigned)nseg)) : cut1;
        if (cut2 >= wmax || cut2 <= cut1) cut2 = cut1;
        const int s_ = c.seg;
        seg_lo = s_ == 0 ? 0u : (s_ == 1 ? cut1 : cut2);
        seg_hi = s_ >= nseg - 1 ? wmax : (s_ == 0 ? cut1 : cut2);
        if (s_ >= nseg || seg_hi <= seg_lo) return;
        if (seg_hi < wmax) k_hi = cut_level(seg_hi);
    }
    const bool resumed = k_hi >= 0 && last > seg_hi;
    if (k_hi >= 0) { last = min(last, seg_hi); wmax = min(wmax, seg_hi); }
    const float d0 = inside ? dL_dcolor[pix] : 0.f, d1 = inside ? dL_dcolor[HW + pix] : 0.f,
                d2 = inside ? dL_dcolor[2 * HW + pix] : 0.f;
    float dz_ = 0.f, do_ = 0.f, dq_ = 0.f;
    if constexpr (OUT != 0) {
        const float* const dL_dopacity = extra_image(0, extra...);
        const float* const dL_ddepth_sq = extra_image(1, extra...);
        if (inside && dL_ddepth) dz_ = dL_ddepth[pix];
        if (inside && dL_dopacity) do_ = dL_dopacity[pix];
        if (DSQ && inside && dL_ddepth_sq) dq_ = dL_ddepth_sq[pix];
    } else {
        dz_ = (DEPTH_GRAD && inside) ? dL_ddepth[pix] : 0.f;
    }
    const float tfbg = OUT != 0 ? Tf * ((cam.bg[0] * d0 + cam.bg[1] * d1 + cam.bg[2] * d2) - do_)
                                : Tf * (cam.bg[0] * d0 + cam.bg[1] * d1 + cam.bg[2] * d2);
    float T = Tf, S = 0.f;
    if (resumed) {
        const float* st = split_state + (size_t)k_hi * 5 * HW + pix;
        const float* tot = split_state + (size_t)kCutLevels * 5 * HW + pix;
        T = st[0];
        const float it = 1.0f / T;
        S = ((tot[0] - st[HW]) * it) * d0 + ((tot[HW] - st[2 * HW]) * it) * d1 + ((tot[2 * HW] - st[3 * HW]) * it) * d2;
        if (DEPTH_GRAD) S += ((tot[3 * HW] - st[4 * HW]) * it) * dz_;
    }
    int cmin = (int)(seg_lo / kWave);
    int ctop = (int)((wmax - 1) / kWave);
    const int chain_q = __builtin_amdgcn_readfirstlane(c.tile * 4 + c.quad);
    float* const chain_st = const_cast<float*>(split_state) + (size_t)chain_q * kChainStateFloats;
    uint32_t* const chain_fl = reinterpret_cast<uint32_t*>(const_cast<float*>(split_state) + (size_t)cam.gx * cam.gy * 4 * kChainStateFloats) +
                               (size_t)chain_q * (kChainPieces - 1);
    if (pieces > 1) {
        const int n = __builtin_amdgcn_readfirstlane(ctop + 1);
        ctop = n - (n * piece) / pieces - 1; cmin = n - (n * (piece + 1)) / pieces;
    }
    uint32_t rmax = last;
#pragma unroll
    for (int m = 8; m >= 1; m >>= 1) rmax = max(rmax, (uint32_t)__shfl_xor(rmax, m));
    const uint32_t rm0 = (uint32_t)__builtin_amdgcn_readlane((int)rmax, 0), rm1 = (uint32_t)__builtin_amdgcn_readlane((int)rmax, 16);
    const uint32_t rm2 = (uint32_t)__builtin_amdgcn_readlane((int)rmax, 32), rm3 = (uint32_t)__builtin_amdgcn_readlane((int)rmax, 48);

    const int tb = lane >> 2, rb = lane & 3;
    const int bxb = (int)c.qx0 + (rb & 1) * 4, byb = (int)c.qy0 + (rb >> 1) * 4;
    float e0[16], e1[16], e2[16];
    {
        float* xs = s_m[wave][0];
        xs[lane] = d0; xs[kWave + lane] = d1; xs[2 * kWave + lane] = d2;
        if (DEPTH_GRAD) s_ez[wave][lane] = dz_;
        if (DSQ) s_eq[wave][lane] = dq_;
        __builtin_amdgcn_wave_barrier();
        const float4* x4 = reinterpret_cast<const float4*>(xs + rb * 16);
#pragma unroll
        for (int v = 0; v < 4; v++) {
            const float4 a = x4[v], b = x4[kWave / 4 + v], cc = x4[2 * (kWave / 4) + v];
            e0[4 * v] = a.x; e0[4 * v + 1] = a.y; e0[4 * v + 2] = a.z; e0[4 * v + 3] = a.w;
            e1[4 * v] = b.x; e1[4 * v + 1] = b.y; e1[4 * v + 2] = b.z; e1[4 * v + 3] = b.w;
            e2[4 * v] = cc.x; e2[4 * v + 1] = cc.y; e2[4 * v + 2] = cc.z; e2[4 * v + 3] = cc.w;
        }
        __builtin_amdgcn_wave_barrier();
    }
    const float bxf = (float)bxb, byf = (float)byb;
    const int m_rd = tb * kMT + rb * 16;
    const uint8_t* list_b = s_list[wave] + rb * kWave + tb;

    const int cmax = ctop;
    uint32_t id_next = (cmax >= cmin && (uint32_t)cmax * kWave + lane < wmax) ? list[cmax * kWave + lane] : kNoId;
    uint32_t id_next2 = cmax >= cmin + 1 ? list[(cmax - 1) * kWave + lane] : kNoId;
    float4 r0 = make_float4(0.f, 0.f, 0.f, 0.f), r1 = r0, r2 = make_float4(0.f, 0.f, -1.f, -1.f);
    if (id_next != kNoId) { r0 = geom[(size_t)id_next * 3]; r1 = geom[(size_t)id_next * 3 + 1]; r2 = geom[(size_t)id_next * 3 + 2]; }
    if (pieces > 1 && piece > 0) {
        int polls = 0;
        bool handed = cam.chain_polls >= 0;
        while (handed && __hip_atomic_load(chain_fl + piece - 1, __ATOMIC_RELAXED, __HIP_MEMORY_SCOPE_AGENT) != cam.chain_epoch) {
            __builtin_amdgcn_s_sleep(16);
            if (++polls > cam.chain_polls) handed = false;
        }
        if (!handed && lane == 0) {
            if (cam.async_status) __hip_atomic_store(cam.async_status, 1u, __ATOMIC_RELAXED, __HIP_MEMORY_SCOPE_SYSTEM);
            if (cam.chain_fail) __hip_atomic_store(cam.chain_fail, 1u, __ATOMIC_RELAXED, __HIP_MEMORY_SCOPE_AGENT);
        }
        GS_WAIT_VMEM();
        const float* in = chain_st + (piece - 1) * 2 * kWave;
        T = __hip_atomic_load(in + lane, __ATOMIC_RELAXED, __HIP_MEMORY_SCOPE_AGENT);
        S = __hip_atomic_load(in + kWave + lane, __ATOMIC_RELAXED, __HIP_MEMORY_SCOPE_AGENT);
        if (!handed) T = __builtin_nanf("");
    }
    int cnt = 0;
    int upto = kWave;
    const int cmin_u = __builtin_amdgcn_readfirstlane(cmin);
    for (int ch = __builtin_amdgcn_readfirstlane(cmax); ch >= cmin_u;) {
        const float4 q0 = r0, q1 = r1, q2 = r2;
        const uint32_t id_cur = id_next;
        id_next = id_next2;
        id_next2 = ch >= cmin_u + 2 ? list[(ch - 2) * kWave + lane] : kNoId;
        {
            const float4* gr = geom + (size_t)(id_next != kNoId ? id_next : 0u) * 3;
            r0 = gr[0]; r1 = gr[1]; r2 = gr[2];
        }

        const uint32_t cpos = (uint32_t)ch * kWave;
        unsigned long long m_any;
        const unsigned hf = scan_blocks(q0, q2, id_cur != kNoId && lane < upto, c.qx0, c.qy0, cpos < rm0, cpos < rm1, cpos < rm2, cpos < rm3, m_any);
        const int n_hit = (int)__popcll(m_any);
        bool split = false;
        if (m_any != 0ull) {
            const int room = kWave - cnt;
            split = n_hit > room;
            const int n_stage = split ? room : n_hit;
            const int rel = n_hit - 1 - (int)__builtin_amdgcn_mbcnt_hi((uint32_t)(m_any >> 32), __builtin_amdgcn_mbcnt_lo((uint32_t)m_any, 0u));
            const bool stage = hf != 0u && rel < n_stage;
            if (stage) {
                const int slot = cnt + rel;
                const StagedConic k = staged_conic(q0, q1);
                s0[slot] = k.s0;
                s1[slot] = make_float4(k.c, q1.y, q1.z, q1.w);
                s2[slot] = make_float4(q2.x, __uint_as_float(cpos + (uint32_t)lane), q2.y, __uint_as_float(id_cur));
                s_flag[wave][slot] = (uint8_t)hf;
            }
            cnt = __builtin_amdgcn_readfirstlane(cnt + n_stage);
            if (split) upto = (int)__ffsll((unsigned long long)__ballot(stage)) - 1;
        }
        if (!split) upto = kWave;
        if (split) {
            r0 = q0; r1 = q1; r2 = q2; id_next2 = id_next; id_next = id_cur;
        } else {
            ch--;
        }
        if (cnt == 0 || !(split || ch < cmin_u || (m_any != 0ull && cnt + n_hit + kRoundSlack > kWave))) continue;

        __builtin_amdgcn_wave_barrier();
        const unsigned fl = lane < cnt ? (unsigned)s_flag[wave][lane] : 0u;
        const unsigned long long mb[4] = {__ballot((fl & 1u) != 0u), __ballot((fl & 2u) != 0u), __ballot((fl & 4u) != 0u), __ballot((fl & 8u) != 0u)};
        int rank[4];
        const int ntrips = build_stream_lists(s_list[wave], mb, lane, rank);
        const int p0 = rank[0], p1 = rank[1], p2 = rank[2], p3 = rank[3];
        float racc[10] = {0.f, 0.f, 0.f, 0.f, 0.f, 0.f, 0.f, 0.f, 0.f, 0.f};
        __builtin_amdgcn_wave_barrier();
        for (int t0 = 0; t0 < ntrips; t0 += kBT) {
            const int tend = min(kBT, ntrips - t0);
            uint32_t jj2_next = *reinterpret_cast<const uint16_t*>(my_list + t0);
            for (int t = 0; t < tend; t += 2) {
                const uint32_t jj2 = jj2_next;
                jj2_next = *reinterpret_cast<const uint16_t*>(my_list + t0 + t + 2);
                const int jj[2] = {(int)(jj2 & 0xffu), (int)(jj2 >> 8)};
                float4 a0[2], a1[2], a2[2];
                float G[2], alpha[2];
                bool ok[2];
#pragma unroll
                for (int u = 0; u < 2; u++) { a0[u] = s0[jj[u]]; a1[u] = s1[jj[u]]; a2[u] = s2[jj[u]]; }
#pragma unroll
                for (int u = 0; u < 2; u++) {
                    const SplatAlpha a = splat_alpha(a0[u], a1[u].x, a1[u].y, pxf, pyf);
                    G[u] = a.G; alpha[u] = a.alpha;
                    ok[u] = __float_as_uint(a2[u].y) < last && a.hit;
                }
                float* w1 = m1p + (t * kMT + lane); float* w2 = m2p + (t * kMT + lane);
#pragma unroll
                for (int u = 0; u < 2; u++) {
                    const float a_eff = ok[u] ? alpha[u] : 0.0f;
                    const float G_eff = ok[u] ? G[u] : 0.0f;
                    const float rcp = __builtin_amdgcn_rcpf(1.0f - a_eff);
                    T = T * rcp;
                    float cd = a1[u].z * d0 + a1[u].w * d1 + a2[u].x * d2;
                    if (DEPTH_GRAD) cd += a2[u].z * dz_;
                    if (DSQ) cd += (a2[u].z * a2[u].z) * dq_;
                    const float dot = cd - S;
                    const float dL_dalpha = dot * T - tfbg * rcp;
                    S += a_eff * dot;
                    const float GdA = G_eff * dL_dalpha;
                    w1[u * kMT] = GdA;
                    w2[u * kMT] = a_eff * T;
                }
            }
            __builtin_amdgcn_wave_barrier();
            {
                const int jjb = (int)list_b[t0];
                const float4 rc = s0[jjb];
                const float opb = s1[jjb].y;
                const float4* gp4 = reinterpret_cast<const float4*>(m1p + m_rd);
                const float4* wp4 = reinterpret_cast<const float4*>(m2p + m_rd);
                const float4 g0 = gp4[0], g1 = gp4[1], g2 = gp4[2], g3 = gp4[3];
                const float4 v0 = wp4[0], v1 = wp4[1], v2 = wp4[2], v3 = wp4[3];
                const float gg[16] = {g0.x, g0.y, g0.z, g0.w, g1.x, g1.y, g1.z, g1.w, g2.x, g2.y, g2.z, g2.w, g3.x, g3.y, g3.z, g3.w};
                const float ww[16] = {v0.x, v0.y, v0.z, v0.w, v1.x, v1.y, v1.z, v1.w, v2.x, v2.y, v2.z, v2.w, v3.x, v3.y, v3.z, v3.w};
                const float ddx[4] = {rc.x - bxf, rc.x - (bxf + 1.0f), rc.x - (bxf + 2.0f), rc.x - (bxf + 3.0f)};
                const float ddy[4] = {rc.y - byf, rc.y - (byf + 1.0f), rc.y - (byf + 2.0f), rc.y - (byf + 3.0f)};
                float gc[4], gr[4], rx[4];
#pragma unroll
                for (int q = 0; q < 4; q++) {
                    gc[q] = (gg[q] + gg[4 + q]) + (gg[8 + q] + gg[12 + q]);
                    gr[q] = (gg[4 * q] + gg[4 * q + 1]) + (gg[4 * q + 2] + gg[4 * q + 3]);
                    rx[q] = fmaf(gg[4 * q + 3], ddx[3], fmaf(gg[4 * q + 2], ddx[2], fmaf(gg[4 * q + 1], ddx[1], gg[4 * q] * ddx[0])));
                }
                const float t0x = gc[0] * ddx[0], t1x = gc[1] * ddx[1], t2x = gc[2] * ddx[2], t3x = gc[3] * ddx[3];
                const float u0 = gr[0] * ddy[0], u1 = gr[1] * ddy[1], u2 = gr[2] * ddy[2], u3 = gr[3] * ddy[3];
                float sm[10];
                sm[0] = opb * ((rx[0] + rx[1]) + (rx[2] + rx[3]));
                sm[1] = opb * ((u0 + u1) + (u2 + u3));
                sm[2] = opb * fmaf(t3x, ddx[3], fmaf(t2x, ddx[2], fmaf(t1x, ddx[1], t0x * ddx[0])));
// ... 11 lines not shown
                    for (int v = 0; v < 4; v++) {
                        const float4 z = z4[v];
                        sm[9] = fmaf(ww[4 * v + 3], z.w, fmaf(ww[4 * v + 2], z.z, fmaf(ww[4 * v + 1], z.y, fmaf(ww[4 * v], z.x, sm[9]))));
                    }
                }
                if (DSQ) {
                    const float4* q4 = reinterpret_cast<const float4*>(s_eq[wave] + rb * 16);
                    float sq = 0.0f;
#pragma unroll
                    for (int v = 0; v < 4; v++) {
                        const float4 z = q4[v];
                        sq = fmaf(ww[4 * v + 3], z.w, fmaf(ww[4 * v + 2], z.z, fmaf(ww[4 * v + 1], z.y, fmaf(ww[4 * v], z.x, sq))));
                    }
                    sm[9] = fmaf(2.0f * s2[jjb].z, sq, sm[9]);
                }
                __builtin_amdgcn_wave_barrier();
                float4* ps = reinterpret_cast<float4*>(pair_lds + lane * kPairStride);
                ps[0] = make_float4(sm[0], sm[1], sm[2], sm[3]);
                ps[1] = make_float4(sm[4], 0.f, sm[5], sm[6]);
                ps[2] = make_float4(sm[7], sm[8], sm[9], 0.f);
            }
            __builtin_amdgcn_wave_barrier();
            {
                const int pr[4] = {p0 - t0, p1 - t0, p2 - t0, p3 - t0};
#pragma unroll
                for (int r = 0; r < 4; r++) {
                    if ((unsigned)pr[r] < (unsigned)kBT) {
                        const float4* q = reinterpret_cast<const float4*>(pair_lds + (pr[r] * 4 + r) * kPairStride);
                        const float4 qa = q[0], qb = q[1], qc = q[2];
                        racc[0] += qa.x; racc[1] += qa.y; racc[2] += qa.z; racc[3] += qa.w; racc[4] += qb.x;
                        racc[5] += qb.z; racc[6] += qb.w; racc[7] += qc.x; racc[8] += qc.y; racc[9] += qc.z;
                    }
                }
            }
            __builtin_amdgcn_wave_barrier();
        }
        __builtin_amdgcn_wave_barrier();
        {
            float* fls = s_m[wave][0];
            if (lane < cnt) {
                float4* f4 = reinterpret_cast<float4*>(fls + lane * kPairStride);
                f4[0] = make_float4(racc[0], racc[1], racc[2], racc[3]);
                f4[1] = make_float4(racc[4], 0.f, racc[5], racc[6]);
                f4[2] = make_float4(racc[7], racc[8], racc[9], 0.f);
            }
            __builtin_amdgcn_wave_barrier();
            const int krec = min(fl_rec, 5);
            for (int g = 0; g < cnt; g += 24) {
                float val[4];
                uint32_t id[4];
#pragma unroll
                for (int u = 0; u < 4; u++) {
                    const int slot = g + 6 * u + krec, sl = min(slot, kWave);
                    const float v = fls[sl * kPairStride + fl_off];
                    id[u] = __float_as_uint(s2[sl].w);
                    val[u] = (lane < 60 && slot < cnt) ? v : 0.0f;
                }
                asm volatile("" ::: "memory");
#pragma unroll
                for (int u = 0; u < 4; u++)
                    if (val[u] != 0.0f) atomicAdd(grad2d + (size_t)id[u] * kGradStride + fl_comp, val[u]);
            }
        }
        __builtin_amdgcn_wave_barrier();
        cnt = 0;
    }
    if (pieces > 1 && piece < pieces - 1) {
        float* out = chain_st + piece * 2 * kWave;
        __hip_atomic_store(out + lane, T, __ATOMIC_RELAXED, __HIP_MEMORY_SCOPE_AGENT);
        __hip_atomic_store(out + kWave + lane, S, __ATOMIC_RELAXED, __HIP_MEMORY_SCOPE_AGENT);
        GS_WAIT_VMEM();
        __builtin_amdgcn_wave_barrier();
        if (lane == 0) __hip_atomic_store(chain_fl + piece, cam.chain_epoch, __ATOMIC_RELAXED, __HIP_MEMORY_SCOPE_AGENT);
    }
}

std::atomic<int> g_half_quadrant_tiles{256};
std::atomic<int> g_chain_pieces{kChainPieces};
std::atomic<int> g_chain_min_tiles{kChainMinTiles};
std::atomic<int> g_chain_tickets{0};
std::atomic<int> g_chain_polls{kChainPollsDefault};
std::atomic<int> g_fwd_prio{kFwdPrioDefault};
std::atomic<float> g_fwd_prio_param{kFwdPrioDefaultParam};
uint32_t* g_async_status_dev = nullptr;
uint32_t* g_chain_fail_dev = nullptr;
int g_chain_fail_device = -1;
std::atomic<int> g_few_segments{kFewSegmentsMax};

static hipError_t clear_handover_flags(const Cam& cam, float* split_state, hipStream_t st)
{
    return hipMemsetAsync(split_state + (size_t)cam.gx * cam.gy * 4 * kChainStateFloats, 0, chain_flag_words((size_t)cam.gx * cam.gy) * sizeof(uint32_t), st);
}
static hipError_t mark_nothing_recorded(const Cam& cam, float* split_state, hipStream_t st)
{
    return hipMemsetAsync(split_state + (kCutLevels * 5 + 4) * ((size_t)cam.W * cam.H), 0, sizeof(uint32_t), st);
}

hipError_t launch_blend_forward(const Cam& cam_in, const uint2* ranges, const uint32_t* point_list, const float4* geom,
                                float* out_color, float* out_depth, float* out_opacity, float* final_T,
                                uint32_t* n_contrib, float* out_depth_sq, uint32_t cap, int segments, float* seg_T, float* split_state, uint32_t P,
                                float* zero_fill, hipStream_t st)
{
    Cam cam = cam_in;
    const int k_half = g_half_quadrant_tiles.load(std::memory_order_relaxed), k_fseg = g_few_segments.load(std::memory_order_relaxed);
    cam.half = (segments <= 1 || !seg_T) && cam.gx * cam.gy <= k_half;
    cam.split = (cam.V == 1 && split_state && cam.gx * cam.gy <= min(k_half, kFewTiles)) && k_fseg > 1 ? k_fseg : 0;
    cam.chain = (cam.V == 1 && split_state && cam.gx * cam.gy > kFewTiles) ? kChainPieces : 0;
    cam.fwd_prio = g_fwd_prio.load(std::memory_order_relaxed);
    cam.fwd_prio_param = g_fwd_prio_param.load(std::memory_order_relaxed);
    if (!(cam.fwd_prio_param > 0.0f)) cam.fwd_prio_param = fwd_prio_default_param(cam.fwd_prio);
    const int nb = ((cam.gx * cam.gy + 7) >> 3) << 3;
#define GS_FWD(DSQ, SEG, GRID)                                                                                                     \
    hipLaunchKernelGGL((blend_forward_streams_kernel<DSQ, kFwdStreams, SEG, 4>), GRID, dim3(kBlock), 0, st, cam, ranges, point_list, geom, \
                       out_color, out_depth, out_opacity, final_T, n_contrib, out_depth_sq, cap, seg_T, split_state, P, (float4*)zero_fill)
    const size_t HW = (size_t)cam.W * cam.H;
    if (segments > 1 && seg_T) {
        hipError_t e = zero_fill ? hipMemsetAsync(zero_fill, 0, (size_t)P * kGradStride * sizeof(float), st) : hipSuccess;
        if (e == hipSuccess)
            e = hipMemsetAsync(seg_T + (size_t)cam.gx * cam.gy * segments * kBlock, 0, (size_t)cam.gx * cam.gy * 4 * sizeof(uint32_t), st);
        if (e == hipSuccess) e = hipMemsetAsync(out_color, 0, 3 * HW * sizeof(float), st);
        if (e == hipSuccess) e = hipMemsetAsync(out_depth, 0, HW * sizeof(float), st);
        if (e == hipSuccess && out_depth_sq) e = hipMemsetAsync(out_depth_sq, 0, HW * sizeof(float), st);
        if (e == hipSuccess) e = hipMemsetAsync(n_contrib, 0, HW * sizeof(uint32_t), st);
        if (e == hipSuccess && split_state && cam.gx * cam.gy <= kFewTiles) e = mark_nothing_recorded(cam, split_state, st);
        if (e == hipSuccess && cam.chain > 1) e = clear_handover_flags(cam, split_state, st);
        if (e != hipSuccess) return e;
        const dim3 grid(nb, segments);
        if (out_depth_sq) { GS_FWD(true, 1, grid); GS_FWD(true, 2, grid); }
        else { GS_FWD(false, 1, grid); GS_FWD(false, 2, grid); }
    } else if (cam.half || cam.split) {
        if (cam.chain > 1) {
            hipError_t e = clear_handover_flags(cam, split_state, st);
            if (e != hipSuccess) return e;
        }
        const dim3 grid(((cam.gx * cam.gy + 7) >> 3) << 3), block(kPcWaves * kWave);
        if (out_depth_sq)
            hipLaunchKernelGGL((blend_forward_pc_kernel<true>), grid, block, 0, st, cam, ranges, point_list, geom, out_color, out_depth, out_opacity,
                               final_T, n_contrib, out_depth_sq, cap, split_state, P, (float4*)zero_fill);
        else
            hipLaunchKernelGGL((blend_forward_pc_kernel<false>), grid, block, 0, st, cam, ranges, point_list, geom, out_color, out_depth, out_opacity,
                               final_T, n_contrib, out_depth_sq, cap, split_state, P, (float4*)zero_fill);
    } else {
        if (split_state && cam.gx * cam.gy <= kFewTiles) {
            hipError_t e = mark_nothing_recorded(cam, split_state, st);
            if (e != hipSuccess) return e;
        }
        if (out_depth_sq) GS_FWD(true, 0, dim3(nb)); else GS_FWD(false, 0, dim3(nb));
    }
#undef GS_FWD
    return hipGetLastError();
}

hipError_t launch_blend_topdown(const Cam& cam_in, const uint2* ranges, const uint32_t* point_list, const float4* geom, float* free_opacity,
                                uint8_t* free_binary, uint8_t* visible_rgb, uint8_t* visible_binary, uint32_t cap, uint32_t P, hipStream_t st)
{
    Cam cam = cam_in;
    cam.half = 0; cam.split = 0; cam.chain = 0;
    if (cam.V != 1) return hipErrorInvalidValue;
    const int nb = ((cam.gx * cam.gy + 7) >> 3) << 3;
    hipLaunchKernelGGL(blend_topdown_kernel, dim3(nb), dim3(kBlock), 0, st, cam, ranges, point_list, geom, free_opacity, free_binary, visible_rgb,
                       visible_binary, cap, P);
    return hipGetLastError();
}

hipError_t launch_blend_backward(const Cam& cam_in, const uint2* ranges, const uint32_t* point_list, const float4* geom, const float* split_state,
                                 const float* final_T, const uint32_t* n_contrib, const float* dL_dcolor,
                                 const float* dL_ddepth, float* grad2d, hipStream_t st, const float* dL_dopacity, const float* dL_ddepth_sq)
{
    Cam cam = cam_in;
    cam.half = 0;
    const int k_half = g_half_quadrant_tiles.load(std::memory_order_relaxed), k_fseg = g_few_segments.load(std::memory_order_relaxed);
    const int k_pieces = g_chain_pieces.load(std::memory_order_relaxed), k_min = g_chain_min_tiles.load(std::memory_order_relaxed);
    cam.split = (split_state != nullptr && cam.gx * cam.gy <= min(k_half, kFewTiles) && k_fseg > 1) ? k_fseg : 0;
    if (dL_ddepth_sq) cam.split = 0;
    cam.chain = (cam.V == 1 && split_state && cam.gx * cam.gy > max(k_min, kFewTiles) && k_pieces > 1) ? k_pieces : 0;
    static std::atomic<unsigned> epoch{0};
    do { cam.chain_epoch = ++epoch; } while (cam.chain_epoch == 0u);
    cam.chain_ticket = g_chain_tickets.load(std::memory_order_relaxed); cam.chain_polls = g_chain_polls.load(std::memory_order_relaxed);
    cam.async_status = g_async_status_dev;
    cam.chain_fail = chain_fail_word();
    const int per = ((cam.gx * cam.gy + 7) >> 3) * (cam.split ? cam.split : cam.chain > 1 ? cam.chain : 1);
#define GS_BWD(DG, FEW)                                                                                                          \
    hipLaunchKernelGGL((blend_backward_kernel<DG, 1, FEW>), dim3(per * 8 * 4), dim3(kWave), 0, st, cam, ranges, point_list, geom, final_T, \
                       n_contrib, dL_dcolor, dL_ddepth, grad2d, split_state)
#define GS_BWD_OUT(FEW, OUT)                                                                                                     \
    hipLaunchKernelGGL((blend_backward_kernel<true, 1, FEW, OUT, const float*, const float*>), dim3(per * 8 * 4), dim3(kWave), 0, st, cam, ranges, \
                       point_list, geom, final_T, n_contrib, dL_dcolor, dL_ddepth, grad2d, split_state, dL_dopacity, dL_ddepth_sq)
    if (dL_ddepth_sq) GS_BWD_OUT(false, 2);
// ... 10 lines not shown
```

activesplat_amd/csrc/gs_common.h:

```cpp
#pragma once
#include <hip/hip_runtime.h>
#include <stdint.h>
#include <math.h>

#include <atomic>
#include <type_traits>

#include "../../include/gsplat_hip.h"

namespace gs {

constexpr int kTile = GS_TILE;
constexpr int kBlock = 256;
constexpr int kWave = 64;
constexpr int kQuad = 8;
#ifndef GS_BIN_CHUNK
#define GS_BIN_CHUNK 2048
#endif
constexpr int kBinChunk = GS_BIN_CHUNK;
constexpr int kMaxLdsTiles = 8192;
constexpr int kSortChunk = 2048;
constexpr int kSortCapMax = 16384;

struct Cam {
    int W, H, gx, gy;
    int V, Wv, gxv, nbv;
    float tanfovx, tanfovy, fx, fy, mod;
    int sh_degree, sh_coeffs;
    const float* bg;
    const float* view;
    const float* proj;
    const float* campos;
    int half;
    int fwd_prio;
    float fwd_prio_param;
    int split;
    int chain;
    unsigned chain_epoch;
    int chain_ticket, chain_polls;
    uint32_t* async_status;
    uint32_t* chain_fail;
    int act, act_iso, act_accumulate;
    float act_q[4], act_t[3];
};

struct CamDP : Cam {
    const float* dev_q;
    const float* dev_t;
    int64_t stride;
};
struct CamBand : Cam {
    float band_upper, band_lower;
};
__device__ __forceinline__ void normalize_pose_column(const float* x, int64_t stride, float (&u)[4], float& norm)
{
#pragma clang fp contract(off)
    const float a = x[0], b = x[stride], c = x[2 * stride], d = x[3 * stride];
    norm = sqrtf(((a * a + b * b) + c * c) + d * d);
    const float n = fmaxf(norm, 1e-12f);
    u[0] = a / n; u[1] = b / n; u[2] = c / n; u[3] = d / n;
}
template <class T> struct CamArg { typedef T type; };
__device__ __forceinline__ void load_device_pose(Cam&) {}
__device__ __forceinline__ void load_device_pose(CamDP& c)
{
    float n;
    normalize_pose_column(c.dev_q, c.stride, c.act_q, n);
    for (int k = 0; k < 3; k++) c.act_t[k] = c.dev_t[k * c.stride];
}

__device__ __forceinline__ void quat_to_rot(const float* q, float (&R)[3][3])
{
    const float r = q[0], x = q[1], y = q[2], z = q[3];
    R[0][0] = 1.f - 2.f * (y * y + z * z); R[0][1] = 2.f * (x * y - r * z); R[0][2] = 2.f * (x * z + r * y);
    R[1][0] = 2.f * (x * y + r * z); R[1][1] = 1.f - 2.f * (x * x + z * z); R[1][2] = 2.f * (y * z - r * x);
    R[2][0] = 2.f * (x * z - r * y); R[2][1] = 2.f * (y * z + r * x); R[2][2] = 1.f - 2.f * (x * x + y * y);
}
__device__ __forceinline__ void qmul(const float* a, const float* b, float* m)
{
    m[0] = a[0] * b[0] - a[1] * b[1] - a[2] * b[2] - a[3] * b[3];
    m[1] = a[0] * b[1] + a[1] * b[0] + a[2] * b[3] - a[3] * b[2];
    m[2] = a[0] * b[2] - a[1] * b[3] + a[2] * b[0] + a[3] * b[1];
    m[3] = a[0] * b[3] + a[1] * b[2] - a[2] * b[1] + a[3] * b[0];
}
__device__ __forceinline__ void qmul_bwd_rhs(const float* a, const float* dm, float* du)
{
    du[0] = a[0] * dm[0] + a[1] * dm[1] + a[2] * dm[2] + a[3] * dm[3];
    du[1] = -a[1] * dm[0] + a[0] * dm[1] + a[3] * dm[2] - a[2] * dm[3];
    du[2] = -a[2] * dm[0] - a[3] * dm[1] + a[0] * dm[2] + a[1] * dm[3];
    du[3] = -a[3] * dm[0] + a[2] * dm[1] - a[1] * dm[2] + a[0] * dm[3];
}
__device__ __forceinline__ void activate_rotation(const float* cam_q, int iso, const float* q, float* out)
{
    const float inv = 1.0f / fmaxf(sqrtf(q[0] * q[0] + q[1] * q[1] + q[2] * q[2] + q[3] * q[3]), 1e-12f);
    const float u[4] = {q[0] * inv, q[1] * inv, q[2] * inv, q[3] * inv};
    if (iso) { for (int k = 0; k < 4; k++) out[k] = u[k]; return; }
    float m[4];
    qmul(cam_q, u, m);
    const float invm = 1.0f / fmaxf(sqrtf(m[0] * m[0] + m[1] * m[1] + m[2] * m[2] + m[3] * m[3]), 1e-12f);
    for (int k = 0; k < 4; k++) out[k] = m[k] * invm;
}
__device__ __forceinline__ void activate_rotation_bwd(const float* cam_q, int iso, const float* q, const float* g, float* dq)
{
    const float nq = fmaxf(sqrtf(q[0] * q[0] + q[1] * q[1] + q[2] * q[2] + q[3] * q[3]), 1e-12f);
    const float u[4] = {q[0] / nq, q[1] / nq, q[2] / nq, q[3] / nq};
    float du[4];
    if (iso) {
        for (int k = 0; k < 4; k++) du[k] = g[k];
    } else {
        float m[4];
        qmul(cam_q, u, m);
        const float nm = fmaxf(sqrtf(m[0] * m[0] + m[1] * m[1] + m[2] * m[2] + m[3] * m[3]), 1e-12f);
        const float r[4] = {m[0] / nm, m[1] / nm, m[2] / nm, m[3] / nm};
        const float dot = r[0] * g[0] + r[1] * g[1] + r[2] * g[2] + r[3] * g[3];
        float dm[4];
        for (int k = 0; k < 4; k++) dm[k] = (g[k] - r[k] * dot) / nm;
        qmul_bwd_rhs(cam_q, dm, du);
    }
    const float dotu = u[0] * du[0] + u[1] * du[1] + u[2] * du[2] + u[3] * du[3];
    for (int k = 0; k < 4; k++) dq[k] = (du[k] - u[k] * dotu) / nq;
}

__device__ __forceinline__ void qmul_bwd_lhs(const float* b, const float* dm, float* da)
{
    da[0] = b[0] * dm[0] + b[1] * dm[1] + b[2] * dm[2] + b[3] * dm[3];
    da[1] = -b[1] * dm[0] + b[0] * dm[1] - b[3] * dm[2] + b[2] * dm[3];
    da[2] = -b[2] * dm[0] + b[3] * dm[1] + b[0] * dm[2] - b[1] * dm[3];
    da[3] = -b[3] * dm[0] - b[2] * dm[1] + b[1] * dm[2] + b[0] * dm[3];
}
constexpr int kPoseAcc = 16;
__device__ __forceinline__ void pose_grad_accumulate(const float* cam_q, int iso, const float* w, const float* dmean, const float* q,
                                                     const float* g, float (&acc)[kPoseAcc])
{
    for (int a = 0; a < 3; a++) {
        acc[a] += dmean[a];
        for (int b = 0; b < 3; b++) acc[3 + 3 * a + b] += dmean[a] * w[b];
    }
    if (iso) return;
    const float nq = fmaxf(sqrtf(q[0] * q[0] + q[1] * q[1] + q[2] * q[2] + q[3] * q[3]), 1e-12f);
    const float u[4] = {q[0] / nq, q[1] / nq, q[2] / nq, q[3] / nq};
    float m[4];
    qmul(cam_q, u, m);
    const float nm = fmaxf(sqrtf(m[0] * m[0] + m[1] * m[1] + m[2] * m[2] + m[3] * m[3]), 1e-12f);
    const float r[4] = {m[0] / nm, m[1] / nm, m[2] / nm, m[3] / nm};
    const float dot = r[0] * g[0] + r[1] * g[1] + r[2] * g[2] + r[3] * g[3];
    float dm[4], da[4];
    for (int k = 0; k < 4; k++) dm[k] = (g[k] - r[k] * dot) / nm;
    qmul_bwd_lhs(u, dm, da);
    for (int k = 0; k < 4; k++) acc[12 + k] += da[k];
}

struct AdamCoef { float one_m_b1, b2, one_m_b2, step_size, inv_bc2s, eps; };
struct FusedAdam {
    float* p[5];
    float* m[5];
    float* v[5];
    AdamCoef c[5];
    const uint32_t* fail;
};

struct GeomPtrs {
    float4* geom;
    uint2* rect;
    uint32_t* tiles;
    uint32_t* offsets;
    uint32_t* block_sums;
    uint32_t* clamped;
    uint32_t* tile_total;
    uint32_t* tile_base;
    uint32_t* depth_bits;
    float2* sh_jac;
    float* vis_max;
    uint8_t* vis_seen;
};

#ifndef GS_WAIT_VMEM
#define GS_WAIT_VMEM() asm volatile("s_waitcnt vmcnt(0)" ::: "memory")
#endif

__device__ __forceinline__ float wave_sum(float v)
{
#pragma unroll
    for (int m = 32; m >= 1; m >>= 1) v += __shfl_xor(v, m);
    return v;
}
__device__ __forceinline__ uint32_t wave_sum_u32(uint32_t v)
{
#pragma unroll
    for (int m = 32; m >= 1; m >>= 1) v += __shfl_xor(v, m);
    return v;
}
__device__ __forceinline__ uint32_t wave_inclusive_scan(uint32_t v, int lane)
{
#pragma unroll
    for (int d = 1; d < 64; d <<= 1) {
        uint32_t o = __shfl_up(v, d);
        if (lane >= d) v += o;
    }
    return v;
}
__device__ __forceinline__ void pose_grad_block_row(float (&acc)[kPoseAcc], float* __restrict__ row)
{
    __shared__ float s_red[kBlock / kWave][kPoseAcc];
    const int lane = threadIdx.x & (kWave - 1), wave = threadIdx.x / kWave;
    for (int k = 0; k < kPoseAcc; k++) {
        const float v = wave_sum(acc[k]);
        if (lane == 0) s_red[wave][k] = v;
    }
    __syncthreads();
    if (threadIdx.x < kPoseAcc) {
        float s = 0.f;
        for (int w = 0; w < kBlock / kWave; w++) s += s_red[w][threadIdx.x];
        row[threadIdx.x] = s;
    }
}
template <class PoseT, class OutT>
__device__ __forceinline__ void pose_grad_finish_block(int64_t nrows, const PoseT& pose, const float* __restrict__ rows, OutT* __restrict__ out)
{
    constexpr int kSlices = kBlock / kPoseAcc;
    __shared__ double s[kSlices][kPoseAcc];
    const int c = threadIdx.x % kPoseAcc, sl = threadIdx.x / kPoseAcc;
    double acc = 0.0;
    for (int64_t r = sl; r < nrows; r += kSlices) acc += (double)rows[r * kPoseAcc + c];
    s[sl][c] = acc;
    __syncthreads();
    if (threadIdx.x != 0) return;
    double t[kPoseAcc];
    for (int k = 0; k < kPoseAcc; k++) {
        double v = 0.0;
        for (int j = 0; j < kSlices; j++) v += s[j][k];
        t[k] = v;
    }
    const double* dR = t + 3;
    const double q0 = pose.q[0], q1 = pose.q[1], q2 = pose.q[2], q3 = pose.q[3];
    const double nq = sqrt(q0 * q0 + q1 * q1 + q2 * q2 + q3 * q3);
    const double r = q0 / nq, x = q1 / nq, y = q2 / nq, z = q3 / nq;
    const double d0 = 2.0 * (-z * dR[1] + y * dR[2] + z * dR[3] - x * dR[5] - y * dR[6] + x * dR[7]);
    const double d1 = 2.0 * (y * dR[1] + z * dR[2] + y * dR[3] - 2.0 * x * dR[4] - r * dR[5] + z * dR[6] + r * dR[7] - 2.0 * x * dR[8]);
    const double d2 = 2.0 * (-2.0 * y * dR[0] + x * dR[1] + r * dR[2] + x * dR[3] + z * dR[5] - r * dR[6] + z * dR[7] - 2.0 * y * dR[8]);
    const double d3 = 2.0 * (-2.0 * z * dR[0] - r * dR[1] + x * dR[2] + r * dR[3] - 2.0 * z * dR[4] + y * dR[5] + x * dR[6] + y * dR[7]);
    const double dot = r * d0 + x * d1 + y * d2 + z * d3;
    out[0] = (OutT)((d0 - r * dot) / nq + t[12]); out[1] = (OutT)((d1 - x * dot) / nq + t[13]);
    out[2] = (OutT)((d2 - y * dot) / nq + t[14]); out[3] = (OutT)((d3 - z * dot) / nq + t[15]);
    out[4] = (OutT)t[0]; out[5] = (OutT)t[1]; out[6] = (OutT)t[2];
}

__device__ __forceinline__ double strided_record_sum(const double* __restrict__ part, int64_t records, int stride)
{
    double a = 0.0;
    for (int64_t r = threadIdx.x; r < records; r += kBlock) a += part[r * stride];
    return a;
}

template <int K>
__device__ __forceinline__ void block_tree_sum(double (&a)[K], double (&s_tree)[K][kBlock])
{
    const int tid = threadIdx.x;
// ... 327 lines not shown
__device__ __forceinline__ void store_sh_jac(float2* base, size_t i, const float (&J)[9], uint32_t clamp_bits)
{
    float2* o = base + i * (kShJacFloats / 2);
    o[0] = make_float2(J[0], J[1]); o[1] = make_float2(J[2], J[3]); o[2] = make_float2(J[4], J[5]); o[3] = make_float2(J[6], J[7]);
    o[4] = make_float2(J[8], __uint_as_float(clamp_bits));
}
__device__ __forceinline__ void load_sh_jac(const float2* base, size_t i, float (&J)[9], uint32_t& clamp_bits)
{
    const float2* o = base + i * (kShJacFloats / 2);
    const float2 a = o[0], b = o[1], c = o[2], d = o[3], e = o[4];
    J[0] = a.x; J[1] = a.y; J[2] = b.x; J[3] = b.y; J[4] = c.x; J[5] = c.y; J[6] = d.x; J[7] = d.y; J[8] = e.x;
    clamp_bits = __float_as_uint(e.y);
}

struct GaussianInputs {
    const float* means3D;
    const float* shs;
    const float* colors;
    const float* opac;
    const float* scales;
    const float* rots;
    const float* cov3D;
};
struct GaussianGrads { float *dmeans2D, *dmeans3D, *dopac, *dcolors, *dshs, *dscales, *drots, *dcov3D; };
struct DevPose { const float* q; const float* t; int64_t stride; };
enum PoseSource { POSE_NONE = 0, POSE_HOST, POSE_DEVICE, POSE_BAND };
enum PoseGrad { POSE_GRAD_NONE = 0, POSE_GRAD_WITH_PARAMS = 1, POSE_GRAD_ONLY = 2 };
struct PoseRequest {
    PoseSource source;
    const float* pose7;
    DevPose dev;
    float band_upper, band_lower;
    PoseGrad grad;
    float* dL_dpose7;
    void* pose_scratch;
};
struct GaussianBackward {
    GaussianInputs in;
    GaussianGrads out;
    const int32_t* radii;
    const uint32_t* clamped;
    const float2* sh_jac;
    const float* grad2d;
    const FusedAdam* adam;
};

template <class CamT>
hipError_t launch_preprocess_forward(const CamT& cam, int P, const GaussianInputs& in, int32_t* radii, GeomPtrs gp, hipStream_t st);
hipError_t launch_scan_block_sums(int P, GeomPtrs gp, uint32_t* d_total, hipStream_t st);
template <class CamT>
hipError_t launch_preprocess_backward(const CamT& cam, int P, const GaussianBackward& g, const PoseRequest& pose, hipStream_t st);
hipError_t launch_tile_count(const Cam& cam, int P, GeomPtrs gp, uint32_t* tile_total, uint32_t* tile_base,
                             uint2* ranges, uint32_t* d_counts, uint32_t* host_counts, hipStream_t st);
hipError_t launch_tile_scatter_sort(const Cam& cam, int P, GeomPtrs gp, uint32_t* tile_base, const uint2* ranges,
                                    uint32_t max_tile_instances, unsigned long long* pairs, unsigned long long* pairs_alt,
                                    uint32_t* point_list, uint32_t cap, hipStream_t st);
extern std::atomic<int> g_half_quadrant_tiles;
extern std::atomic<int> g_chain_pieces;
extern std::atomic<int> g_chain_min_tiles;
extern std::atomic<int> g_chain_tickets;
extern std::atomic<int> g_chain_polls;
enum { kFwdPrioOff = 0, kFwdPrioT = 1, kFwdPrioDecay = 2, kFwdPrioChunk = 3 };
constexpr int kFwdPrioDefault = kFwdPrioT;
constexpr float kFwdPrioDefaultParam = 0.0f;
constexpr uint32_t kFwdPrioListChunks = 3;
extern std::atomic<int> g_fwd_prio;
extern std::atomic<float> g_fwd_prio_param;
inline float fwd_prio_default_param(int mode)
{
    return mode == kFwdPrioT ? 0.1f : mode == kFwdPrioDecay ? 3.0f : 6.0f;
}
extern uint32_t* g_async_status_dev;
extern uint32_t* g_chain_fail_dev;
extern int g_chain_fail_device;
inline uint32_t* chain_fail_word()
{
    if (!g_chain_fail_dev) return nullptr;
    int dev = -1;
    if (hipGetDevice(&dev) != hipSuccess) { (void)hipGetLastError(); return nullptr; }
    return dev == g_chain_fail_device ? g_chain_fail_dev : nullptr;
}
extern std::atomic<int> g_few_segments;
constexpr int kFewTiles = 256;
constexpr int kChainPieces = 3;
constexpr int kChainMinTiles = 768;
constexpr int kChainStateFloats = (kChainPieces - 1) * 2 * kWave;
constexpr int kChainTicketStride = 32;
constexpr int kChainTicketWords = 8 * kChainTicketStride;
inline size_t chain_flag_words(size_t tiles) { return tiles * 4 * (kChainPieces - 1) + kChainTicketWords; }
inline size_t chain_state_words(size_t tiles) { return tiles * 4 * kChainStateFloats + chain_flag_words(tiles); }
constexpr int kChainPollsDefault = 1 << 21;
constexpr int kCutStep = 256;
constexpr int kCutLinear = 4096;
constexpr int kCutLast = 131072;
constexpr int kCutLevels = kCutLinear / kCutStep + 5;
constexpr int kFewSegmentsMax = 3;
__host__ __device__ inline int cut_level(uint32_t pos)
{
    if (pos >= (uint32_t)kCutStep && pos <= (uint32_t)kCutLinear) return pos % kCutStep == 0 ? (int)(pos / kCutStep) - 1 : -1;
    if (pos > (uint32_t)kCutLinear && pos <= (uint32_t)kCutLast && (pos & (pos - 1u)) == 0u) {
        int l = kCutLinear / kCutStep - 1;
        for (uint32_t q = kCutLinear; q < pos; q <<= 1) ++l;
        return l;
    }
    return -1;
}
__host__ __device__ inline uint32_t cut_nearest(uint32_t target)
{
    if (target < (uint32_t)kCutStep / 2) return 0u;
    if (target <= (uint32_t)kCutLinear + kCutStep / 2) {
        uint32_t k = (target + kCutStep / 2) / kCutStep;
        if (k < 1u) k = 1u;
        if (k > (uint32_t)(kCutLinear / kCutStep)) k = kCutLinear / kCutStep;
        return k * kCutStep;
    }
    uint32_t pos = kCutLinear;
    while (pos < (uint32_t)kCutLast && (unsigned long long)target * 46341ull >= ((unsigned long long)pos << 16)) pos <<= 1;
    return pos;
}
hipError_t launch_emit(const Cam& cam, int P, GeomPtrs gp, uint64_t* keys, uint32_t* vals, hipStream_t st);
hipError_t launch_ranges(int64_t D, const uint64_t* keys_sorted, uint2* ranges, hipStream_t st);
hipError_t launch_blend_forward(const Cam& cam, const uint2* ranges, const uint32_t* point_list, const float4* geom,
                                float* out_color, float* out_depth, float* out_opacity, float* final_T,
                                uint32_t* n_contrib, float* out_depth_sq, uint32_t cap, int segments, float* seg_T, float* split_state, uint32_t P, float* zero_fill,
                                hipStream_t st);
hipError_t launch_blend_topdown(const Cam& cam, const uint2* ranges, const uint32_t* point_list, const float4* geom, float* free_opacity,
                                uint8_t* free_binary, uint8_t* visible_rgb, uint8_t* visible_binary, uint32_t cap, uint32_t P, hipStream_t st);
hipError_t launch_blend_backward(const Cam& cam, const uint2* ranges, const uint32_t* point_list, const float4* geom, const float* split_state,
                                 const float* final_T, const uint32_t* n_contrib, const float* dL_dcolor,
                                 const float* dL_ddepth, float* grad2d, hipStream_t st, const float* dL_dopacity = nullptr,
                                 const float* dL_ddepth_sq = nullptr);
hipError_t launch_adam_multi(int count, const GsAdamTensor* tensors, hipStream_t st);
hipError_t launch_rows(int mode, int count, const GsRowTensor* t, int64_t row0, int64_t n_valid, int64_t n_rows, const float* in, float* out,
                       hipStream_t st);
hipError_t launch_adam(int64_t n, float* p, const float* g, float* m, float* v, double lr, double b1, double b2,
                       double eps, int step, hipStream_t st);

hipError_t launch_activate_forward(int P, int iso, const float* pose7, const float* means3D, const float* rots, const float* logit_op,
                                   const float* log_scales, float* o_means, float* o_rots, float* o_op, float* o_scales, hipStream_t st);
hipError_t launch_activate_backward(int P, int iso, const float* pose7, const float* rots, const float* o_op, const float* o_scales,
                                    const float* g_means, const float* g_rots, const float* g_op, const float* g_scales, float* d_means,
                                    float* d_rots, float* d_logit, float* d_logs, int accumulate, hipStream_t st);
hipError_t launch_activate_backward_pose(int P, int iso, const float* pose7, const float* means3D, const float* rots, const float* o_op,
                                         const float* o_scales, const float* g_means, const float* g_rots, const float* g_op,
                                         const float* g_scales, float* d_means, float* d_rots, float* d_logit, float* d_logs, int accumulate,
                                         int pose_mode, float* pose_rows, hipStream_t st);
inline int64_t pose_rows_count(int64_t P) { return (P + kBlock - 1) / kBlock; }
hipError_t launch_pose_grad_finish(int64_t nrows, const float* pose7, const float* pose_rows, float* dpose7, hipStream_t st);
hipError_t launch_pose_grad_finish_dev(int64_t nrows, const float* dev_q, int64_t stride, const float* pose_rows, float* dpose7, hipStream_t st);
constexpr int kTrackState = 32;
struct TrackAdam { float one_m_b1, b2, one_m_b2, bc2_sqrt, eps, neg_step_size[2]; };
hipError_t launch_tracking_begin(const float* rots_col, const float* trans_col, int64_t stride, float* state, hipStream_t st);
hipError_t launch_tracking_step(int64_t pose_nrows, const float* pose_rows, int64_t loss_nrows, const float* loss_rows, float w_im, float w_depth,
                                float* rots_col, float* trans_col, int64_t stride, const TrackAdam& c, float* state, float* history_row,
                                hipStream_t st);
inline int64_t tracking_loss_rows(int64_t npix) { return (npix + kBlock - 1) / kBlock; }
hipError_t launch_tracking_loss(int W, int H, const float* im, const float* gt, const float* depth, const float* depth_sq, const float* gt_depth,
                                const float* sil, int use_sil, float sil_thres, float w_im, float w_depth, float* dL_dim, float* dL_ddepth,
                                float* rows, float* losses, hipStream_t st, const float* d_median = nullptr);
constexpr int kLossAccSlots = 256;
hipError_t launch_mapping_loss(int W, int H, const float* im, const float* gt, const float* depth, const float* depth_sq,
                               const float* gt_depth, float w_im, float w_depth, float* losses, float* dL_dim,
                               float* dL_ddepth, float* scratch, int64_t persistent_call, hipStream_t st, const float* d_median = nullptr);
__device__ __forceinline__ float depth_error(float g, float d)
{
#pragma clang fp contract(off)
// ... 107 lines not shown
```

activesplat_amd/csrc/preprocess.hip:

```cpp
#include "gs_common.h"
#include <type_traits>

#pragma clang fp contract(off)

namespace gs {

__device__ __forceinline__ int clamp_tile(float v, int hi)
{
    v = fminf(fmaxf(v, -1048576.0f), 1048576.0f);
    int i = (int)v;
    return min(hi, max(0, i));
}

__device__ __forceinline__ void sh_basis(int deg, float x, float y, float z, float* b)
{
    b[0] = 0.28209479177387814f;
    if (deg > 0) {
        b[1] = -0.4886025119029199f * y; b[2] = 0.4886025119029199f * z; b[3] = -0.4886025119029199f * x;
        if (deg > 1) {
            const float xx = x * x, yy = y * y, zz = z * z, xy = x * y, yz = y * z, xz = x * z;
            b[4] = 1.0925484305920792f * xy;
            b[5] = -1.0925484305920792f * yz;
            b[6] = 0.31539156525252005f * (2.0f * zz - xx - yy);
            b[7] = -1.0925484305920792f * xz;
// ... 42 lines not shown
            const float cy_ = fminf(limy, fmaxf(-limy, tytz)) * tz;
            const float J00 = cam.fx / tz, J02 = -(cam.fx * cx_) / (tz * tz);
            const float J11 = cam.fy / tz, J12 = -(cam.fy * cy_) / (tz * tz);
            const float T00 = J00 * m[0] + J02 * m[2], T01 = J00 * m[4] + J02 * m[6], T02 = J00 * m[8] + J02 * m[10];
            const float T10 = J11 * m[1] + J12 * m[2], T11 = J11 * m[5] + J12 * m[6], T12 = J11 * m[9] + J12 * m[10];
            float k00, k01, k11, det;
            if (has_cov) {
                const float c0 = s_cov[tid * 6], c1 = s_cov[tid * 6 + 1], c2 = s_cov[tid * 6 + 2];
                const float c3 = s_cov[tid * 6 + 3], c4 = s_cov[tid * 6 + 4], c5 = s_cov[tid * 6 + 5];
                const float v00 = (c0 * T00 + c1 * T01) + c2 * T02;
                const float v01 = (c1 * T00 + c3 * T01) + c4 * T02;
                const float v02 = (c2 * T00 + c4 * T01) + c5 * T02;
                const float v10 = (c0 * T10 + c1 * T11) + c2 * T12;
                const float v11 = (c1 * T10 + c3 * T11) + c4 * T12;
                const float v12 = (c2 * T10 + c4 * T11) + c5 * T12;
                k00 = ((T00 * v00 + T01 * v01) + T02 * v02) + 0.3f;
                k01 = (T10 * v00 + T11 * v01) + T12 * v02;
                k11 = ((T10 * v10 + T11 * v11) + T12 * v12) + 0.3f;
                det = k00 * k11 - k01 * k01;
            } else {
                const float sx = cam.mod * s_scale[tid * 3], sy = cam.mod * s_scale[tid * 3 + 1], sz = cam.mod * s_scale[tid * 3 + 2];
                const float4 rq = reinterpret_cast<const float4*>(s_rot)[tid];
                const float r = rq.x, x = rq.y, y = rq.z, z = rq.w;
                const float R00 = 1.0f - 2.0f * (y * y + z * z), R01 = 2.0f * (x * y - r * z), R02 = 2.0f * (x * z + r * y);
                const float R10 = 2.0f * (x * y + r * z), R11 = 1.0f - 2.0f * (x * x + z * z), R12 = 2.0f * (y * z - r * x);
                const float R20 = 2.0f * (x * z - r * y), R21 = 2.0f * (y * z + r * x), R22 = 1.0f - 2.0f * (x * x + y * y);
                const float M00 = R00 * sx, M01 = R01 * sy, M02 = R02 * sz;
                const float M10 = R10 * sx, M11 = R11 * sy, M12 = R12 * sz;
                const float M20 = R20 * sx, M21 = R21 * sy, M22 = R22 * sz;
                const float a10 = (T00 * M00 + T01 * M10) + T02 * M20, a11 = (T00 * M01 + T01 * M11) + T02 * M21, a12 = (T00 * M02 + T01 * M12) + T02 * M22;
                const float a20 = (T10 * M00 + T11 * M10) + T12 * M20, a21 = (T10 * M01 + T11 * M11) + T12 * M21, a22 = (T10 * M02 + T11 * M12) + T12 * M22;
                const float n1 = (a10 * a10 + a11 * a11) + a12 * a12, n2 = (a20 * a20 + a21 * a21) + a22 * a22;
                const float xc = a11 * a22 - a12 * a21, yc = a12 * a20 - a10 * a22, zc = a10 * a21 - a11 * a20;
                k00 = n1 + 0.3f;
                k01 = (a10 * a20 + a11 * a21) + a12 * a22;
                k11 = n2 + 0.3f;
                det = (((xc * xc + yc * yc) + zc * zc) + 0.3f * (n1 + n2)) + 0.09f;
            }
            if (det > 0.0f) {
                const float det_inv = 1.0f / det;
                const float mid = 0.5f * (k00 + k11);
                const float sq = sqrtf(fmaxf(0.1f, mid * mid - det));
                const float lam = fmaxf(mid + sq, mid - sq);
                float rf = ceilf(3.0f * sqrtf(lam));
                rf = fminf(rf, 16777216.0f);
                const float pxv = ((ndcx + 1.0f) * (float)cam.Wv - 1.0f) * 0.5f;
                const float pyy = ((ndcy + 1.0f) * (float)cam.H - 1.0f) * 0.5f;
                const int xs = view * cam.gxv;
                const int x0 = clamp_tile((pxv - rf) / 16.0f, cam.gxv) + xs, x1 = clamp_tile(((pxv + rf) + 15.0f) / 16.0f, cam.gxv) + xs;
                const float pxx = cam.V > 1 ? pxv + (float)(xs * kTile) : pxv;
                const int y0 = clamp_tile((pyy - rf) / 16.0f, cam.gy), y1 = clamp_tile(((pyy + rf) + 15.0f) / 16.0f, cam.gy);
                const int area = (x1 - x0) * (y1 - y0);
                float cr, cg, cb;
                if (HAS_SH) { cr = sh_rgb[0]; cg = sh_rgb[1]; cb = sh_rgb[2]; }
                else { cr = s_col[tid * 3]; cg = s_col[tid * 3 + 1]; cb = s_col[tid * 3 + 2]; }
                const float con_a = k11 * det_inv, con_b = -k01 * det_inv, con_c = k00 * det_inv;
                const bool finite = __builtin_isfinite(pxx) && __builtin_isfinite(pyy) && __builtin_isfinite(con_a) && __builtin_isfinite(con_b) &&
                                    __builtin_isfinite(con_c) && __builtin_isfinite(o) && __builtin_isfinite(cr) && __builtin_isfinite(cg) &&
                                    __builtin_isfinite(cb) && __builtin_isfinite(tz);
                if (area > 0 && finite) {
                    radius = (int)rf;
                    ntiles = (uint32_t)area;
                    rc = make_uint2((uint32_t)x0 | ((uint32_t)x1 << 16), (uint32_t)y0 | ((uint32_t)y1 << 16));
                    if (HAS_SH) clampbits = sh_clamp;
                    float ex = -1.0f, ey = -1.0f;
                    const float o255 = o * 255.0f;
                    if (o255 > 1.0f) {
                        const float tau2 = 2.0f * (__logf(o255) + 0.02f);
                        ex = sqrtf(tau2 * k00) + 0.01f;
                        ey = sqrtf(tau2 * k11) + 0.01f;
                    }
                    g0 = make_float4(pxx, pyy, con_a, con_b);
                    g1 = make_float4(con_c, band ? -o : o, cr, cg);
                    g2 = make_float4(cb, tz, ex, ey);
                }
            }
        }
        radii[io] = radius;
        if (radius_out) *radius_out = radius;
        if (ntiles) {
            gp.geom[(size_t)io * 3] = g0; gp.geom[(size_t)io * 3 + 1] = g1; gp.geom[(size_t)io * 3 + 2] = g2;
            gp.rect[io] = rc;
            gp.depth_bits[io] = __float_as_uint(g2.y);
        }
        gp.tiles[io] = ntiles;
        if (HAS_SH && !gp.sh_jac) gp.clamped[io] = clampbits;
    } else if (cam.V > 1) {
        radii[io] = 0;
        gp.geom[(size_t)io * 3] = gp.geom[(size_t)io * 3 + 1] = gp.geom[(size_t)io * 3 + 2] = make_float4(0.f, 0.f, 0.f, 0.f);
        gp.rect[io] = make_uint2(0u, 0u);
        gp.tiles[io] = 0u;
        gp.depth_bits[io] = 0u;
        if (HAS_SH) gp.clamped[io] = 0u;
    }
    return ntiles;
}

__device__ __forceinline__ float activate_staged_rows(const Cam& cam, int tid, bool row, float* s_mean, float* s_scale, float* s_rot, float logit)
{
    const float ls0 = s_scale[cam.act_iso ? tid : tid * 3];
    if (cam.act_iso) __syncthreads();
    if (row) {
        float R[3][3];
        quat_to_rot(cam.act_q, R);
        const float px = s_mean[tid * 3], py = s_mean[tid * 3 + 1], pz = s_mean[tid * 3 + 2];
        s_mean[tid * 3] = R[0][0] * px + R[0][1] * py + R[0][2] * pz + cam.act_t[0];
        s_mean[tid * 3 + 1] = R[1][0] * px + R[1][1] * py + R[1][2] * pz + cam.act_t[1];
        s_mean[tid * 3 + 2] = R[2][0] * px + R[2][1] * py + R[2][2] * pz + cam.act_t[2];
        if (cam.act_iso) {
            const float e = __expf(ls0);
            s_scale[tid * 3] = e; s_scale[tid * 3 + 1] = e; s_scale[tid * 3 + 2] = e;
        } else {
            s_scale[tid * 3] = __expf(ls0); s_scale[tid * 3 + 1] = __expf(s_scale[tid * 3 + 1]); s_scale[tid * 3 + 2] = __expf(s_scale[tid * 3 + 2]);
        }
        const float4 q4 = reinterpret_cast<const float4*>(s_rot)[tid];
        const float q[4] = {q4.x, q4.y, q4.z, q4.w};
        float out[4];
        activate_rotation(cam.act_q, cam.act_iso, q, out);
        reinterpret_cast<float4*>(s_rot)[tid] = make_float4(out[0], out[1], out[2], out[3]);
    }
    return 1.0f / (1.0f + __expf(-logit));
}

template <int SH, bool ACT = false, class CamT = Cam>
__global__ __launch_bounds__(kBlock) void preprocess_forward_kernel(
    typename CamArg<CamT>::type cam, int P, const float* __restrict__ means3D, const float* __restrict__ shs,
    const float* __restrict__ colors, const float* __restrict__ opac, const float* __restrict__ scales,
    const float* __restrict__ rots, const float* __restrict__ cov3Dp, int32_t* __restrict__ radii, GeomPtrs gp)
{
    load_device_pose(cam);
    constexpr bool HAS_SH = SH != 0;
    constexpr bool SLAB = SH == 1;
    constexpr int kGeoFloats = kBlock * 7, kColFloats = SLAB ? 0 : kBlock * 3;
    constexpr int kSlabFloats = SLAB ? (kBlock / kWave) * kShHalf * kShPad : 0;
    constexpr int kPoolFloats = (kGeoFloats + kColFloats) > kSlabFloats ? (kGeoFloats + kColFloats) : kSlabFloats;
    __shared__ __attribute__((aligned(16))) float s_mean[kBlock * 3];
    __shared__ __attribute__((aligned(16))) float s_pool[kPoolFloats];
    __shared__ uint32_t s_wsum[kBlock / kWave];
    float* const s_scale = s_pool;
    float* const s_rot = s_pool + kBlock * 3;
    float* const s_cov = s_pool;
    float* const s_col = s_pool + kGeoFloats;
    float* const s_sh = s_pool;

    const int tid = threadIdx.x;
    const int vbase = blockIdx.x * kBlock;
    const int view = cam.V > 1 ? (int)blockIdx.x / cam.nbv : 0;
    const int base = (cam.V > 1 ? (int)blockIdx.x - view * cam.nbv : (int)blockIdx.x) * kBlock;
    const int nrows = max(0, min(kBlock, P - base));
    if (vbase + tid < cam.gx * cam.gy) gp.tile_total[vbase + tid] = 0u;
    const int i = base + tid, io = vbase + tid;
    float o_in = i < P ? opac[i] : 0.0f;
    stage_rows<3>(s_mean, means3D, base, nrows, tid);
    if (!SLAB) {
        if (cov3Dp) stage_rows<6>(s_cov, cov3Dp, base, nrows, tid);
        else {
            if (ACT && cam.act_iso) stage_rows<1>(s_scale, scales, base, nrows, tid); else stage_rows<3>(s_scale, scales, base, nrows, tid);
            stage_rows<4>(s_rot, rots, base, nrows, tid);
        }
        if (SH == 0) stage_rows<3>(s_col, colors, base, nrows, tid);
    }
    __syncthreads();
    constexpr bool BAND = std::is_same<CamT, CamBand>::value;
    bool in_band = false;
    if constexpr (BAND) {
        const float up = -s_mean[tid * 3 + 1];
// ... 206 lines not shown
```

activesplat_amd/csrc/tilebin.hip:

```cpp
#include "gs_common.h"


namespace gs {

template <class F>
__device__ __forceinline__ void expand_wave(const uint32_t* incl_w, const uint32_t* s_x0w, const uint32_t* s_y0,
                                            int wave, int lane, uint32_t total, int gx, F f)
{
    for (uint32_t t0 = 0; t0 < total; t0 += kWave) {
        const uint32_t t = t0 + lane;
        if (t < total) {
            int lo = 0, hi = 63;
#pragma unroll
            for (int s = 0; s < 6; s++) {
                const int mid = (lo + hi) >> 1;
                if (incl_w[mid] > t) hi = mid; else lo = mid + 1;
            }
            const int j = wave * kWave + lo;
            const uint32_t k = t - (lo ? incl_w[lo - 1] : 0u);
            const uint32_t xw = s_x0w[j];
            const uint32_t w = xw >> 16, x0 = xw & 0xffffu;
            const uint32_t tile = (s_y0[j] + k / w) * (uint32_t)gx + x0 + k % w;
            f(tile, j);
        }
    }
}

template <bool SCATTER, int THREADS>
__global__ __launch_bounds__(THREADS) void tile_bin_kernel(Cam cam, int P, GeomPtrs gp, int tiles, int chunk,
                                                          uint32_t* __restrict__ tile_total,
                                                          uint32_t* __restrict__ tile_base,
                                                          const uint2* __restrict__ ranges,
                                                          unsigned long long* __restrict__ pairs, uint32_t cap, int nchunks)
{
    __shared__ uint32_t s_hist[kMaxLdsTiles];
    __shared__ uint32_t s_incl[THREADS];
    __shared__ uint32_t s_x0w[THREADS];
    __shared__ uint32_t s_y0[THREADS];
    __shared__ uint32_t s_depth[THREADS];

    const int tid = threadIdx.x, lane = tid & 63, wave = tid >> 6;
  const int cper = (nchunks + 7) >> 3;
  for (int b = blockIdx.x; b < 8 * cper; b += gridDim.x) {
    const int cid = SCATTER ? (b & 7) * cper + (b >> 3) : b;
    if (cid >= nchunks) continue;
    uint32_t* my_base = tile_base + (size_t)cid * tiles;
    const int cbase = cid * chunk;
    constexpr int kBinRounds = SCATTER ? kBinChunk / THREADS : 1, kBinCursorRounds = SCATTER ? 2 : 1;
    uint32_t rn[kBinRounds], rd[kBinRounds], cur[kBinCursorRounds];
    uint2 rr[kBinRounds];
    if (SCATTER) {
#pragma unroll
        for (int q = 0; q < kBinRounds; q++) {
            const int ic = min(cbase + q * THREADS + tid, P - 1);
            rn[q] = gp.tiles[ic];
            rr[q] = gp.rect[ic];
            rd[q] = gp.depth_bits[ic];
        }
#pragma unroll
        for (int k = 0; k < kBinCursorRounds; k++) {
            const int tc = min(tid + k * THREADS, tiles - 1);
            cur[k] = ranges[tc].x + my_base[tc];
        }
    }
    __syncthreads();
    if (SCATTER) {
#pragma unroll
        for (int k = 0; k < kBinCursorRounds; k++) if (tid + k * THREADS < tiles) s_hist[tid + k * THREADS] = cur[k];
        for (int t = tid + kBinCursorRounds * THREADS; t < tiles; t += THREADS) s_hist[t] = ranges[t].x + my_base[t];
    } else {
        for (int t = tid; t < tiles; t += THREADS) s_hist[t] = 0u;
    }
    __syncthreads();
    for (int r = 0; r < chunk / THREADS; r++) {
        const int i = cbase + r * THREADS + tid;
        if (cbase + r * THREADS >= P) break;
        uint32_t n = 0, x0 = 0, w = 1, y0 = 0, dbits = 0;
        if (SCATTER) {
            uint32_t pn = rn[0], pd = rd[0];
            uint2 prc = rr[0];
#pragma unroll
            for (int q = 1; q < kBinRounds; q++) if (r == q) { pn = rn[q]; pd = rd[q]; prc = rr[q]; }
            n = i < P ? pn : 0u;
            if (n) { x0 = prc.x & 0xffffu; w = (prc.x >> 16) - x0; y0 = prc.y & 0xffffu; dbits = pd; }
        } else if (i < P) {
            n = gp.tiles[i];
            if (n) {
                const uint2 rc = gp.rect[i];
                x0 = rc.x & 0xffffu; w = (rc.x >> 16) - x0; y0 = rc.y & 0xffffu;
                if (SCATTER) dbits = gp.depth_bits[i];
            }
        }
        const int gbase = cbase + r * THREADS;
        auto place = [&](uint32_t tile, uint32_t depth_bits, uint32_t id) {
            if (SCATTER) {
                const uint32_t slot = atomicAdd(&s_hist[tile], 1u);
                if (slot < cap) pairs[slot] = ((unsigned long long)depth_bits << 32) | id;
            } else {
                atomicAdd(&s_hist[tile], 1u);
            }
        };
        if (!__any(n > 16u)) {
            uint32_t kx = 0, ky = 0;
            for (uint32_t k = 0; __any(k < n); k++) {
                if (k < n) {
                    place((y0 + ky) * (uint32_t)cam.gx + x0 + kx, dbits, (uint32_t)i);
                    if (++kx == w) { kx = 0; ++ky; }
                }
            }
            continue;
        }
        if (n) {
            s_x0w[tid] = x0 | (w << 16);
            s_y0[tid] = y0;
            if (SCATTER) s_depth[tid] = dbits;
        }
        const uint32_t incl = wave_inclusive_scan(n, lane);
        s_incl[tid] = incl;
        const uint32_t total = __shfl(incl, 63);
        __builtin_amdgcn_wave_barrier();
        expand_wave(s_incl + wave * kWave, s_x0w, s_y0, wave, lane, total, cam.gx, [&](uint32_t tile, int j) {
            place(tile, SCATTER ? s_depth[j] : 0u, (uint32_t)(gbase + j));
        });
        __builtin_amdgcn_wave_barrier();
    }
    if (!SCATTER) {
        __syncthreads();
        for (int t = tid; t < tiles; t += THREADS) my_base[t] = s_hist[t];
    }
  }
}

template <int TW>
__global__ __launch_bounds__(1024) void tile_colscan_kernel(uint32_t* __restrict__ base, int chunks, int tiles, uint32_t* __restrict__ tile_total)
{
    constexpr int SEG = 1024 / TW;
    __shared__ uint32_t s_sum[SEG][TW + 1];
    const int l = threadIdx.x % TW, sgm = threadIdx.x / TW;
    const int ngroups = (tiles + TW - 1) / TW, gper = (ngroups + 7) >> 3;
    const int grp = (int)(blockIdx.x & 7) * gper + (int)(blockIdx.x >> 3);
    const int t = ((int)(blockIdx.x >> 3) < gper && grp < ngroups) ? grp * TW + l : tiles;
    const int L = (chunks + SEG - 1) / SEG, r0 = min(chunks, sgm * L), r1 = min(chunks, r0 + L);
    uint32_t sum = 0;
    if (t < tiles) {
#pragma unroll 8
        for (int r = r0; r < r1; r++) sum += base[(size_t)r * tiles + t];
    }
    s_sum[sgm][l] = sum;
    __syncthreads();
    uint32_t run = 0;
    for (int q = 0; q < sgm; q++) run += s_sum[q][l];
    if (t < tiles) {
#pragma unroll 8
        for (int r = r0; r < r1; r++) {
            const size_t idx = (size_t)r * tiles + t;
            const uint32_t v = base[idx];
            base[idx] = run;
            run += v;
        }
        if (sgm == SEG - 1) tile_total[t] = run;
    }
}

constexpr int kScanPerThreadMax = 8;
__global__ __launch_bounds__(1024) void tile_scan_kernel(const uint32_t* __restrict__ tile_total, int tiles,
                                                         uint2* __restrict__ ranges, uint32_t* __restrict__ counts,
                                                         uint32_t* __restrict__ host_counts)
{
    __shared__ uint32_t s_w[16];
    __shared__ uint32_t s_m[16];
    const int tid = threadIdx.x, lane = tid & 63, wave = tid >> 6;
    const int per = (tiles + 1023) >> 10, t0 = tid * per;
    uint32_t v[kScanPerThreadMax];
    uint32_t sum = 0, vmax = 0;
#pragma unroll
    for (int k = 0; k < kScanPerThreadMax; k++) {
        v[k] = (k < per && t0 + k < tiles) ? tile_total[t0 + k] : 0u;
        sum += v[k];
        vmax = max(vmax, v[k]);
    }
    const uint32_t inc = wave_inclusive_scan(sum, lane);
#pragma unroll
    for (int m = 32; m >= 1; m >>= 1) vmax = max(vmax, (uint32_t)__shfl_xor(vmax, m));
    if (lane == 63) { s_w[wave] = inc; s_m[wave] = vmax; }
    __syncthreads();
    uint32_t start = inc - sum, total = 0, mx = 0;
    for (int w = 0; w < 16; w++) {
        if (w < wave) start += s_w[w];
        total += s_w[w];
        mx = max(mx, s_m[w]);
    }
#pragma unroll
    for (int k = 0; k < kScanPerThreadMax; k++) {
        if (k < per && t0 + k < tiles) ranges[t0 + k] = make_uint2(start, start + v[k]);
        start += v[k];
    }
    if (tid == 0) {
        counts[0] = total; counts[1] = mx;
        if (host_counts) { host_counts[0] = total; host_counts[1] = mx; }
    }
}

#ifndef GS_MIN_F64
#define GS_MIN_F64(a, b) ({ double r_; asm("v_min_f64 %0, %1, %2" : "=v"(r_) : "v"(a), "v"(b)); r_; })
#define GS_MAX_F64(a, b) ({ double r_; asm("v_max_f64 %0, %1, %2" : "=v"(r_) : "v"(a), "v"(b)); r_; })
// ... 482 lines not shown
```

activesplat_amd/rasterizer.py:

```python
from __future__ import annotations

import collections
import contextlib
import ctypes as C
import threading
from typing import NamedTuple

import torch
from torch import nn

from . import _lib


class GaussianRasterizationSettings(NamedTuple):
    image_height: int
    image_width: int
    tanfovx: float
    tanfovy: float
    bg: torch.Tensor
    scale_modifier: float
    viewmatrix: torch.Tensor
    projmatrix: torch.Tensor
    sh_degree: int
    campos: torch.Tensor
# ... 3 lines not shown

last_stats = {"num_rendered": 0, "P": 0}
_capacity = {}
optimistic = True

_tls = threading.local()
_capacity_lock = threading.Lock()


@contextlib.contextmanager
def capture():
    stack = getattr(_tls, "captures", None)
    if stack is None:
        stack = _tls.captures = []
    state = {}
    stack.append(state)
    try:
        yield state
    finally:
        stack.remove(state)


def _require_rocm(device):
    if device.type != "cuda":
        raise RuntimeError("activesplat_amd rasteriser needs ROCm device tensors (no CPU fallback)")


def _host_counters(device, stream_handle):
    pool = getattr(_tls, "pinned", None)
    if pool is None:
        pool = _tls.pinned = {}
    key = (device.index, stream_handle)
    buf = pool.get(key)
    if buf is None:
        if len(pool) >= 64:
            pool.pop(next(iter(pool)))
        buf = pool[key] = torch.zeros(2, dtype=torch.int32).pin_memory()
    return buf


def _ptr(t):
    return None if t is None else C.c_void_p(t.data_ptr())


def _f32(t, device):
    if t is None:
        return None
    if t.dtype != torch.float32 or t.device != device or not t.is_contiguous():
        t = t.to(device=device, dtype=torch.float32).contiguous()
    if t.data_ptr() % 16:
        t = t.clone()
    return t


def _stream(device):
    return _lib.stream_ptr(device)


_layouts = {}


def _frame_layouts(lib, P, W, H):
    key = (P, W, H)
    hit = _layouts.get(key)
    if hit is None:
        gl = _lib.GsGeomLayout(); _lib.check(lib.gs_geom_layout(P, W, H, C.byref(gl)))
        il = _lib.GsImageLayout(); _lib.check(lib.gs_image_layout(W, H, C.byref(il)))
        if len(_layouts) >= 64:
            _layouts.pop(next(iter(_layouts)))
        hit = _layouts[key] = (gl, il, int(lib.gs_backward_scratch_bytes(P)))
    return hit


def _camera(rs: GaussianRasterizationSettings, device, sh_coeffs: int):
    keep = dict(bg=_f32(rs.bg, device).reshape(-1), view=_f32(rs.viewmatrix, device).reshape(-1),
                proj=_f32(rs.projmatrix, device).reshape(-1), campos=_f32(rs.campos, device).reshape(-1))
    if keep["view"].numel() != 16 or keep["proj"].numel() != 16 or keep["bg"].numel() != 3:
        raise Exception("GaussianRasterizationSettings: viewmatrix/projmatrix must hold 16 values, bg 3")
    cam = _lib.GsCamera(int(rs.image_width), int(rs.image_height), int(rs.sh_degree), int(sh_coeffs),
                        float(rs.tanfovx), float(rs.tanfovy), float(rs.scale_modifier), 0,
                        keep["bg"].data_ptr(), keep["view"].data_ptr(), keep["proj"].data_ptr(),
                        keep["campos"].data_ptr())
    return cam, keep


def _capture_target():
    caps = getattr(_tls, "captures", None)
    return caps[-1] if caps else None


_Frame = collections.namedtuple("_Frame", "device cur st_handle st gl il scratch_bytes geom image radii d_num h_num")


def _begin_frame(lib, device, P, W, H, image_bytes=None):
    cur = torch.cuda.current_stream(device) if device.type == "cuda" else None
    st_handle = int(cur.cuda_stream) if cur is not None else 0
    gl, il, scratch_bytes = _frame_layouts(lib, P, W, H)
    return _Frame(device, cur, st_handle, C.c_void_p(st_handle), gl, il, scratch_bytes,
                  torch.empty(gl.total_bytes, dtype=torch.uint8, device=device),
                  torch.empty(il.total_bytes if image_bytes is None else image_bytes(il), dtype=torch.uint8, device=device),
                  torch.empty(P, dtype=torch.int32, device=device), torch.empty(2, dtype=torch.int32, device=device),
                  _host_counters(device, st_handle) if cur is not None else torch.zeros(2, dtype=torch.int32))


def _capacity_guess(key):
    if key is None or not optimistic:
        return None
    with _capacity_lock:
        return _capacity.get(key)


def _capacity_update(key, D, max_tile):
    with _capacity_lock:
        old = _capacity.get(key, (0, 0))
        if len(_capacity) >= 64 and key not in _capacity:
            _capacity.pop(next(iter(_capacity)))
        _capacity[key] = (max(old[0], int(D * 1.25) + 4096), max(old[1], max_tile + max_tile // 16 + 64))


def _record_launch(key, guess, hit, D, max_tile, P):
    if key is not None:
        if hit:
            last_stats["optimistic_hits"] = last_stats.get("optimistic_hits", 0) + 1
        else:
            last_stats["optimistic_misses"] = last_stats.get("optimistic_misses", 0) + (1 if guess is not None else 0)
        _capacity_update(key, D, max_tile)
    last_stats["num_rendered"], last_stats["P"], last_stats["max_tile_instances"] = D, P, max_tile


def _render_at(lib, frame, W, H, launch, cap_d, cap_tile, bl=None):
    if bl is None:
        bl = _lib.GsBinLayout(); _lib.check(lib.gs_bin_layout(cap_d, cap_tile, W, H, C.byref(bl)))
    binning = torch.empty(bl.total_bytes, dtype=torch.uint8, device=frame.device)
    point_list = torch.empty(max(cap_d, 1), dtype=torch.int32, device=frame.device)
    launch(cap_d, cap_tile, binning, point_list)
    return bl, binning, point_list


def _bin_and_render(lib, frame, key, P, W, H, launch, segmented_ok=False):
    cur, h_num = frame.cur, frame.h_num
    done = None
    guess = _capacity_guess(key)
    if guess is not None:
        if cur is not None:
            ev = torch.cuda.Event()
            ev.record(cur)
        bl_g = _lib.GsBinLayout(); _lib.check(lib.gs_bin_layout(guess[0], guess[1], W, H, C.byref(bl_g)))
        if bl_g.path == 1 and (segmented_ok or bl_g.segments <= 1):
            done = _render_at(lib, frame, W, H, launch, guess[0], guess[1], bl_g)
        if cur is not None:
            ev.synchronize()
    elif cur is not None:
        cur.synchronize()
    D = int(h_num[0].item()) & 0xFFFFFFFF
    max_tile = int(h_num[1].item()) & 0xFFFFFFFF
    hit = done is not None and D <= guess[0] and max_tile <= guess[1]
    if not hit:
        done = _render_at(lib, frame, W, H, launch, D, max_tile)
    _record_launch(key, guess, hit, D, max_tile, P)
    return (D, max_tile) + done


class RawInputs(NamedTuple):
    pose7: object
    isotropic: bool
    accumulate: bool = False
# ... 20 lines not shown
    return None if req == default else req


class _RasterizeGaussians(torch.autograd.Function):

    @staticmethod
    def forward(ctx, means3D, means2D, shs, colors_precomp, opacities, scales, rotations, cov3D_precomp, rs, fused=False, raw=None,
                cam_rot=None, cam_trans=None, outputs=None):
        lib = _lib.get()
        device = means3D.device
        leaves = (means3D, opacities, scales, rotations, colors_precomp)
        shs_in = shs
        _require_rocm(device)
        _lib.poll_async_status()
        P = int(means3D.shape[0])
        means3D = _f32(means3D, device)
        shs, colors_precomp = _f32(shs, device), _f32(colors_precomp, device)
        opacities, scales = _f32(opacities, device), _f32(scales, device)
        rotations, cov3D_precomp = _f32(rotations, device), _f32(cov3D_precomp, device)
        M = 0 if shs is None else int(shs.shape[1])
        cam, keep = _camera(rs, device, M)
        W, H = int(rs.image_width), int(rs.image_height)
        fr = _begin_frame(lib, device, P, W, H)
        st, geom, image, radii = fr.st, fr.geom, fr.image, fr.radii
        pose_req = None
        if raw is not None and cam_rot is not None and (cam_rot.requires_grad or cam_trans.requires_grad):
            pose_req = (not raw.gaussians_grad, cam_rot.shape, cam_trans.shape)
        ctx.pose_req = pose_req
        ctx.cam_inputs = cam_rot is not None
        ctx.outputs = outputs
        want_bwd = 1 if any(ctx.needs_input_grad[:8]) or pose_req is not None else 0
        pose = None
        ctx.devpose = raw.device_pose if raw is not None else None
        if raw is not None:
            iso = 1 if raw.isotropic else 0
            vis_max, vis_seen = raw.visibility if raw.visibility is not None else (None, None)
            tail = (_ptr(vis_max), _ptr(vis_seen), _ptr(radii), _ptr(geom), _ptr(image), _ptr(fr.d_num), _ptr(fr.h_num), want_bwd, st)
        if ctx.devpose is not None:
            rots_p, trans_p, t_idx = ctx.devpose
            _lib.check(lib.gs_preprocess_forward_raw_dev(C.byref(cam), P, _ptr(means3D), _ptr(shs), _ptr(colors_precomp), _ptr(opacities),
                                                         _ptr(scales), _ptr(rotations), _ptr(rots_p), _ptr(trans_p), int(rots_p.shape[-1]),
                                                         int(t_idx), iso, *tail))
        elif raw is not None:
            pose = (C.c_float * 7)(*[float(v) for v in raw.pose7])
            _lib.check(lib.gs_preprocess_forward_raw(C.byref(cam), P, _ptr(means3D), _ptr(shs), _ptr(colors_precomp), _ptr(opacities),
                                                     _ptr(scales), _ptr(rotations), pose, iso, *tail))
        else:
            _lib.check(lib.gs_preprocess_forward(C.byref(cam), P, _ptr(means3D), _ptr(shs), _ptr(colors_precomp),
                                                 _ptr(opacities), _ptr(scales), _ptr(rotations), _ptr(cov3D_precomp),
                                                 _ptr(radii), _ptr(geom), _ptr(image), _ptr(fr.d_num), _ptr(fr.h_num), want_bwd, st))
        color = torch.empty(3, H, W, dtype=torch.float32, device=device)
        depth = torch.empty(1, H, W, dtype=torch.float32, device=device)
        opacity = torch.empty(1, H, W, dtype=torch.float32, device=device)
        depth_sq = torch.empty(1, H, W, dtype=torch.float32, device=device) if fused else None
        scratch = None
        if want_bwd and P > 0:
            scratch = torch.empty(fr.scratch_bytes, dtype=torch.uint8, device=device)

        def launch(cap_d, cap_tile, binning_, plist_):
            _lib.check(lib.gs_render_forward(C.byref(cam), P, cap_d, cap_tile, _ptr(geom), _ptr(binning_), _ptr(plist_), _ptr(image),
                                             _ptr(color), _ptr(depth), _ptr(opacity), _ptr(depth_sq), _ptr(scratch), st))

        D, max_tile, bl, binning, point_list = _bin_and_render(lib, fr, (P, W, H, device.index), P, W, H, launch)
        ctx.rs, ctx.D, ctx.keep, ctx.fused, ctx.cam = rs, D, keep, fused, cam
        ctx.scratch, ctx.scratch_clean, ctx.sh_jac = scratch, scratch is not None, want_bwd
        ctx.has = (shs is not None, colors_precomp is not None, scales is not None, rotations is not None,
                   cov3D_precomp is not None)
        ctx.raw = None if raw is None else _RawCtx(pose, iso, bool(raw.accumulate), opacities)
        adam = raw.adam if raw is not None else None
        same = raw is not None and (raw.accumulate or adam is not None) and all(a is b for a, b in zip(leaves, (means3D, opacities, scales, rotations, colors_precomp)))
        ctx.leaves = leaves if same else None
        ctx.adam = None
        if adam is not None:
            if raw.accumulate:
                raise Exception("render_rgbd_raw: adam= and accumulate_grads= exclude each other")
            if pose_req is not None:
                raise Exception("render_rgbd_raw: adam= and a differentiable camera exclude each other (the library has no pose-gradient form of the "
                                "backward with the optimiser step)")
            if not same or (shs is not None and shs is not shs_in):
                raise Exception("render_rgbd_raw(adam=...): the parameters must be contiguous, 16-byte aligned fp32 tensors on the device (they are updated in place)")
            ctx.adam = (adam, leaves[:4] + (shs_in if shs_in is not None else leaves[4],))
        cap = _capture_target()
        if cap is not None:
            cap.update(geom=geom, image=image, binning=binning, point_list=point_list, gl=fr.gl, il=fr.il, bl=bl, D=D, P=P, W=W, H=H)
        e = torch.empty(0, device=device)
        ctx.save_for_backward(means3D, shs if shs is not None else e, colors_precomp if colors_precomp is not None else e,
                              scales if scales is not None else e, rotations if rotations is not None else e,
                              cov3D_precomp if cov3D_precomp is not None else e, radii, geom, point_list, image)
        ctx.set_materialize_grads(False)
        if outputs is not None:
            images = dict(depth=depth, opacity=opacity, depth_sq=depth_sq)
            ctx.mark_non_differentiable(radii, *[t for k, t in images.items() if t is not None and k not in outputs])
            return (color, radii, depth, opacity, depth_sq) if fused else (color, radii, depth, opacity)
        if fused:
            ctx.mark_non_differentiable(radii, opacity, depth_sq)
            return color, radii, depth, opacity, depth_sq
        ctx.mark_non_differentiable(radii, depth, opacity)
        return color, radii, depth, opacity

    @staticmethod
    def backward(ctx, grad_color, _gr=None, grad_depth=None, grad_opacity=None, grad_depth_sq=None):
        out = _RasterizeGaussians._backward(ctx, grad_color, grad_depth, grad_opacity, grad_depth_sq)
        if getattr(ctx, "cam_inputs", False) and len(out) == 11:
            out = out + (None, None)
        if getattr(ctx, "outputs", None) is not None:
            out = out + (None,) * (14 - len(out))
        return out

    @staticmethod
    def _backward(ctx, grad_color, grad_depth, grad_opacity=None, grad_depth_sq=None):
        lib = _lib.get()
        means3D, shs, colors, scales, rots, cov3Dp, radii, geom, point_list, image = ctx.saved_tensors
        has_sh, has_col, has_sc, has_rot, has_cov = ctx.has
        device = means3D.device
        P = int(means3D.shape[0])
        M = int(shs.shape[1]) if has_sh else 0
        cam = ctx.cam
        if grad_color is None:
            grad_color = torch.zeros(3, int(ctx.rs.image_height), int(ctx.rs.image_width), device=device)
        grad_color = _f32(grad_color, device)
        outs = getattr(ctx, "outputs", None)
        depth_on = ctx.fused if outs is None else "depth" in outs
        grad_depth = _f32(grad_depth, device) if (depth_on and grad_depth is not None) else None
        grad_opacity = _f32(grad_opacity, device) if (outs is not None and "opacity" in outs and grad_opacity is not None) else None
        grad_depth_sq = _f32(grad_depth_sq, device) if (outs is not None and "depth_sq" in outs and grad_depth_sq is not None) else None
        grads = None
        if grad_opacity is not None or grad_depth_sq is not None:
            grads = _lib.GsImageGrads(grad_color.data_ptr(), *[None if g is None else g.data_ptr() for g in (grad_depth, grad_opacity, grad_depth_sq)])
        scratch, clean = _take_scratch(ctx, lib, P, device)
        z = lambda *s: torch.empty(*s, dtype=torch.float32, device=device)
        pose_req = getattr(ctx, "pose_req", None)
        d_m2d = z(P, 3)
        if ctx.raw is not None:
            if ctx.adam == "stepped":
                raise RuntimeError("render_rgbd_raw(adam=...): this render's backward has already applied its optimiser step; a second backward "
                                   "through the same graph is refused -- render again, or use accumulate_grads / a separate optimizer.step()")
            rc = ctx.raw
            head = (C.byref(cam), P, ctx.D, _ptr(means3D), _ptr(shs if has_sh else None), _ptr(colors if has_col else None), _ptr(rc.logit),
                    _ptr(scales), _ptr(rots), rc.pose, rc.iso)
            mid = (_ptr(radii), _ptr(geom), _ptr(point_list), _ptr(image), _ptr(grad_color), _ptr(grad_depth), _ptr(d_m2d))
            if grads is not None:
                mid = mid[:4] + (C.byref(grads), mid[6])
            raw_backward = lib.gs_render_backward_raw if grads is None else lib.gs_render_backward_raw_grads
            pose_backward = lib.gs_render_backward_raw_pose if grads is None else lib.gs_render_backward_raw_pose_grads
            scr = (_ptr(scratch), 1 if clean else 0, int(ctx.sh_jac))
            if ctx.adam is not None:
                opt, tensors = ctx.adam
                desc = opt.backward_step_descriptors(tensors)
                ctx.adam = "stepped"
                try:
                    _lib.check(lib.gs_render_backward_raw_adam(*head, *mid, *scr, desc, _stream(device)))
                except Exception:
                    opt.rollback_backward_step(tensors)
                    ctx.adam = (opt, tensors)
                    raise
                torch.autograd.graph.increment_version([t for t in tensors if t is not None])
                return None, d_m2d, None, None, None, None, None, None, None, None, None
            if pose_req is not None:
                d_pose = z(7)
                pscr = torch.empty(int(lib.gs_pose_grad_scratch_bytes(P)), dtype=torch.uint8, device=device)
                pose_tail = (d_pose[:4].view(pose_req[1]), d_pose[4:].view(pose_req[2]))
                if pose_req[0]:
                    _lib.check(pose_backward(*head, 0, *mid, None, None, None, None, None, None, *scr, 1, _ptr(d_pose), _ptr(pscr), _stream(device)))
                    return (None, d_m2d) + (None,) * 9 + pose_tail
        d_m3d, d_op = z(P, 3), z(P, 1)
        d_col = z(P, 3) if has_col else None
        d_shs = z(P, M, 3) if has_sh else None
# ... 39 lines not shown
        return d_m3d, d_m2d, d_shs, d_col, d_op, d_sc, d_rot, d_cov, None, None, None


class _DirectCtx:
    needs_input_grad = (True,) * 8 + (False,) * (_RasterizeGaussians.forward.__code__.co_argcount - 1 - 8)
    saved_tensors = ()

    def save_for_backward(self, *tensors):
        self.saved_tensors = tensors

    def mark_non_differentiable(self, *tensors):
        pass

    def set_materialize_grads(self, value):
        pass


def render_rgbd_raw_direct(rs, means3D, means2D, logit_opacities, log_scales, unnorm_rotations, raw, shs=None, colors_precomp=None):
    ctx = _DirectCtx()
    return ctx, _RasterizeGaussians.forward(ctx, means3D, means2D, shs, colors_precomp, logit_opacities, log_scales, unnorm_rotations, None, rs,
                                            True, raw)


def backward_direct(ctx, grad_color, grad_depth):
    return _RasterizeGaussians._backward(ctx, grad_color, grad_depth)


def _take_scratch(ctx, lib, P, device):
    scratch, clean = ctx.scratch, ctx.scratch_clean
    if scratch is None:
        scratch, clean = torch.empty(int(lib.gs_backward_scratch_bytes(P)), dtype=torch.uint8, device=device), False
    ctx.scratch, ctx.scratch_clean = None, False
    return scratch, clean


def backward_pose_dev(ctx, grad_color, grad_depth, pose_scratch, d_pose=None):
    lib = _lib.get()
    means3D, shs, colors, scales, rots, _cov, radii, geom, point_list, image = ctx.saved_tensors
    has_sh, has_col = ctx.has[0], ctx.has[1]
    device = means3D.device
    P = int(means3D.shape[0])
    iso, logit = ctx.raw.iso, ctx.raw.logit
    rots_p, trans_p, t_idx = ctx.devpose
    scratch, clean = _take_scratch(ctx, lib, P, device)
    d_m2d = torch.empty(P, 3, dtype=torch.float32, device=device)
    _lib.check(lib.gs_render_backward_raw_pose_dev(
        C.byref(ctx.cam), P, ctx.D, _ptr(means3D), _ptr(shs if has_sh else None), _ptr(colors if has_col else None), _ptr(logit), _ptr(scales),
        _ptr(rots), _ptr(rots_p), _ptr(trans_p), int(rots_p.shape[-1]), int(t_idx), iso, _ptr(radii), _ptr(geom), _ptr(point_list), _ptr(image),
        _ptr(_f32(grad_color, device)), _ptr(None if grad_depth is None else _f32(grad_depth, device)), _ptr(d_m2d), _ptr(scratch),
        1 if clean else 0, int(ctx.sh_jac), _ptr(d_pose), _ptr(pose_scratch), _stream(device)))
    return d_m2d


use_frontend = True


_OUTPUT_BITS = {"depth": 1, "opacity": 2, "depth_sq": 4}


def _frontend_apply(means3D, means2D, shs, colors_precomp, opacities, scales, rotations, cov3D_precomp, rs, fused, outputs=None):
    if not use_frontend or _lib.emulated() or means3D.device.type != "cuda":
        return None
    cap = _capture_target()
    from . import _frontend
    _lib.get()
    ext = _frontend.get_or_none()
    if ext is None:
        return None
    device = means3D.device
    P, W, H = int(means3D.shape[0]), int(rs.image_width), int(rs.image_height)
    key = (P, W, H, device.index)
    guess = _capacity_guess(key)
    out, D, max_tile, hit, state, off = ext.rasterize(means3D, means2D, shs, colors_precomp, opacities, scales, rotations, cov3D_precomp, rs.bg,
                                                      rs.viewmatrix, rs.projmatrix, rs.campos, W, H, float(rs.tanfovx), float(rs.tanfovy),
                                                      float(rs.scale_modifier), int(rs.sh_degree), bool(fused), guess[0] if guess else 0,
                                                      guess[1] if guess else 0, cap is not None,
                                                      -1 if outputs is None else sum(_OUTPUT_BITS[k] for k in outputs))
    if cap is not None:
        lib = _lib.get()
        gl, il, _ = _frame_layouts(lib, P, W, H)
        ws, binning, plist2 = state
        cap_d, cap_tile = (guess if hit else (D, max_tile))
        bl = _lib.GsBinLayout(); _lib.check(lib.gs_bin_layout(cap_d, cap_tile, W, H, C.byref(bl)))
        cap.update(geom=ws[off[0]:off[0] + off[1]], image=ws[off[2]:off[2] + off[3]], gl=gl, il=il, bl=bl, D=D, P=P, W=W, H=H, binning=binning,
                   point_list=ws[off[4]:off[4] + 4 * off[5]].view(torch.int32) if hit else plist2)
    _record_launch(key, guess, hit, D, max_tile, P)
    return tuple(out)


def rasterize_gaussians(means3D, means2D, shs, colors_precomp, opacities, scales, rotations, cov3D_precomp,
                        raster_settings, differentiable_outputs=()):
    outputs = _output_request(differentiable_outputs, ("depth", "opacity"), frozenset(), "GaussianRasterizer") if differentiable_outputs else None
    out = _frontend_apply(means3D, means2D, shs, colors_precomp, opacities, scales, rotations, cov3D_precomp, raster_settings, False, outputs)
    if out is not None:
        return out
    if outputs is not None:
        return _RasterizeGaussians.apply(means3D, means2D, shs, colors_precomp, opacities, scales, rotations, cov3D_precomp, raster_settings,
                                         False, None, None, None, outputs)
    return _RasterizeGaussians.apply(means3D, means2D, shs, colors_precomp, opacities, scales, rotations,
                                     cov3D_precomp, raster_settings)


_FUSED_OUTPUTS = ("depth", "silhouette", "opacity", "depth_sq")
_FUSED_DEFAULT = frozenset(("depth",))


def render_rgbd(raster_settings, means3D, means2D, opacities, shs=None, colors_precomp=None, scales=None, rotations=None,
                cov3D_precomp=None, differentiable_outputs=("depth",)):
    if (shs is None) == (colors_precomp is None):
        raise Exception("Please provide excatly one of either SHs or precomputed colors!")
    if ((scales is None or rotations is None) and cov3D_precomp is None) or \
            ((scales is not None or rotations is not None) and cov3D_precomp is not None):
        raise Exception("Please provide exactly one of either scale/rotation pair or precomputed 3D covariance!")
    outputs = _output_request(differentiable_outputs, _FUSED_OUTPUTS, _FUSED_DEFAULT, "render_rgbd")
    out = _frontend_apply(means3D, means2D, shs, colors_precomp, opacities, scales, rotations, cov3D_precomp, raster_settings, True, outputs)
    if out is not None:
        return out
    if outputs is not None:
        return _RasterizeGaussians.apply(means3D, means2D, shs, colors_precomp, opacities, scales, rotations, cov3D_precomp,
                                         raster_settings, True, None, None, None, outputs)
    return _RasterizeGaussians.apply(means3D, means2D, shs, colors_precomp, opacities, scales, rotations, cov3D_precomp,
                                     raster_settings, True)


def render_rgbd_raw(raster_settings, means3D, means2D, logit_opacities, log_scales, unnorm_rotations, pose7, shs=None, colors_precomp=None,
                    accumulate_grads=False, visibility=None, adam=None, camera=None, gaussians_grad=True, differentiable_outputs=("depth",)):
    if (shs is None) == (colors_precomp is None):
        raise Exception("Please provide excatly one of either SHs or precomputed colors!")
    outputs = _output_request(differentiable_outputs, _FUSED_OUTPUTS, _FUSED_DEFAULT, "render_rgbd_raw")
    if adam is not None and outputs is not None and (outputs - _FUSED_DEFAULT):
        raise Exception("render_rgbd_raw: adam= takes differentiable_outputs=('depth',) only (the backward with the optimiser step inside "
                        "has no form for the silhouette / depth_sq gradients)")
    tail = () if outputs is None else (outputs,)
    if shs is not None and int(shs.shape[1]) != 16:
        raise Exception("render_rgbd_raw: SH rows of 16 coefficients only")
    iso = int(log_scales.shape[1]) == 1
    if visibility is not None:
        mx, seen = visibility
        P = int(means3D.shape[0])
        if not (mx.dtype == torch.float32 and mx.is_contiguous() and mx.numel() == P and seen.dtype == torch.bool and seen.is_contiguous()
                and seen.numel() == P and mx.device == means3D.device and seen.device == means3D.device):
            raise Exception("render_rgbd_raw: visibility = (float32 [P], bool [P]) contiguous tensors on the parameters' device")
    if camera is None:
        if not gaussians_grad:
            raise Exception("render_rgbd_raw: gaussians_grad=False is the pose-only backward: it needs camera=(cam_rot, cam_trans)")
        return _RasterizeGaussians.apply(means3D, means2D, shs, colors_precomp, logit_opacities, log_scales, unnorm_rotations, None,
                                         raster_settings, True, RawInputs(pose7, iso, accumulate=accumulate_grads, visibility=visibility, adam=adam),
                                         *((None, None) + tail if tail else ()))
    cam_rot, cam_trans = camera
    if cam_rot.numel() != 4 or cam_trans.numel() != 3:
        raise Exception("render_rgbd_raw: camera = (cam_rot with 4 values, cam_trans with 3)")
    if adam is not None:
        raise Exception("render_rgbd_raw: adam= and a differentiable camera exclude each other (the library has no pose-gradient form of the "
                        "backward with the optimiser step)")
    if pose7 is None:
        pose7 = torch.cat([cam_rot.detach().reshape(4), cam_trans.detach().reshape(3)]).float().cpu().tolist()
    if not gaussians_grad:
        d = lambda t: None if t is None else t.detach()
        means3D, shs, colors_precomp, logit_opacities, log_scales, unnorm_rotations = (d(means3D), d(shs), d(colors_precomp), d(logit_opacities),
                                                                                      d(log_scales), d(unnorm_rotations))
        accumulate_grads = False
    return _RasterizeGaussians.apply(means3D, means2D, shs, colors_precomp, logit_opacities, log_scales, unnorm_rotations, None,
                                     raster_settings, True, RawInputs(pose7, iso, accumulate=accumulate_grads, visibility=visibility, gaussians_grad=gaussians_grad),
                                     cam_rot, cam_trans, *tail)


class GaussianRasterizer(nn.Module):
    def __init__(self, raster_settings: GaussianRasterizationSettings, differentiable_outputs=()):
# ... 80 lines not shown
```

include/gsplat_hip.h:

```cpp
#ifndef GSPLAT_HIP_H
#define GSPLAT_HIP_H

#include <stddef.h>
#include <stdint.h>

#ifdef __cplusplus
extern "C" {
#endif

#define GS_OK 0
#define GS_EINVAL 1
#define GS_ELAUNCH 2
#define GS_ECAPACITY 3

#define GS_TILE 16
#define GS_GEOM_FLOATS 12

typedef void* gs_stream_t;

typedef struct GsCamera {
    int32_t image_width;
    int32_t image_height;
    int32_t sh_degree;
    int32_t sh_coeffs;
    float tanfovx;
    float tanfovy;
    float scale_modifier;
    int32_t num_views;
    const float* bg;
    const float* viewmatrix;
    const float* projmatrix;
    const float* campos;
} GsCamera;

typedef struct GsGeomLayout {
    uint64_t total_bytes;
    uint64_t geom;
    uint64_t rect;
    uint64_t tiles_touched;
    uint64_t offsets;
    uint64_t block_sums;
    uint64_t clamped;
    uint64_t tile_total;
    uint64_t tile_base;
    uint64_t sh_jac;
    uint64_t depth_bits;
} GsGeomLayout;

typedef struct GsImageLayout {
    uint64_t total_bytes;
    uint64_t ranges;
    uint64_t final_T;
    uint64_t n_contrib;
    uint64_t split_state;
} GsImageLayout;

#define GS_SORT_AUTO 0
#define GS_SORT_TILE_LDS 1
#define GS_SORT_RADIX 2

typedef struct GsBinLayout {
    uint64_t total_bytes;
    uint64_t path;
    uint64_t pairs;
    uint64_t keys_unsorted;
    uint64_t vals_unsorted;
    uint64_t keys_sorted;
    uint64_t sort_temp;
    uint64_t segments;
    uint64_t seg_T;
    uint64_t pairs_alt;
} GsBinLayout;

int gs_atlas_layout(int32_t P, int32_t view_width, int32_t num_views, int32_t* virtual_P, int32_t* atlas_width, int32_t* view_stride);
int gs_geom_layout(int32_t P, int32_t width, int32_t height, GsGeomLayout* out);
int gs_image_layout(int32_t width, int32_t height, GsImageLayout* out);
int gs_bin_layout(int64_t D, uint32_t max_tile_instances, int32_t width, int32_t height, GsBinLayout* out);
int gs_set_sort_path(int32_t path);
int gs_set_forward_segments(int32_t on);
int gs_set_half_quadrants(int32_t max_tiles);
int gs_set_backward_chain(int32_t pieces, int32_t min_tiles);
int gs_set_backward_chain_tickets(int32_t on);
int gs_set_backward_chain_polls(int32_t polls);
int gs_set_forward_priority(int32_t mode, float param);
int gs_async_status_word(uint32_t** host_word);
int gs_async_status_clear(void);
int gs_recorded_cut(uint32_t target, uint32_t* nearest, int32_t* level);
int gs_set_backward_segments(int32_t segments);
uint64_t gs_backward_scratch_bytes(int32_t P);

const char* gs_last_error(void);
const char* gs_version(void);
#define GS_ABI_VERSION 23
int32_t gs_abi_version(void);

int gs_profile_enable(int32_t on);
int32_t gs_profile_stage_count(void);
const char* gs_profile_stage_name(int32_t stage);
int gs_profile_collect(float* ms_sum, int32_t* calls, int32_t n_stages);

int gs_preprocess_forward(const GsCamera* cam, int32_t P,
                          const float* means3D, const float* shs, const float* colors_precomp,
                          const float* opacities, const float* scales, const float* rotations,
                          const float* cov3D_precomp,
                          int32_t* radii, void* geom_state, void* image_state, uint32_t* d_counts,
                          uint32_t* h_counts, int32_t want_backward, gs_stream_t stream);

int gs_render_forward(const GsCamera* cam, int32_t P, int64_t D, uint32_t max_tile_instances,
                      void* geom_state, void* bin_state, uint32_t* point_list, void* image_state,
                      float* out_color, float* out_depth, float* out_opacity, float* out_depth_sq,
                      void* backward_scratch, gs_stream_t stream);

int gs_render_backward(const GsCamera* cam, int32_t P, int64_t D,
                       const float* means3D, const float* shs, const float* colors_precomp,
                       const float* scales, const float* rotations, const float* cov3D_precomp,
                       const int32_t* radii, const void* geom_state, const uint32_t* point_list,
                       const void* image_state, const float* dL_dcolor, const float* dL_ddepth,
                       float* dL_dmeans2D, float* dL_dmeans3D, float* dL_dopacities,
                       float* dL_dcolors_precomp, float* dL_dshs, float* dL_dscales,
                       float* dL_drotations, float* dL_dcov3D, void* scratch, int32_t scratch_zeroed,
                       int32_t have_sh_jacobian, gs_stream_t stream);

int gs_preprocess_forward_raw(const GsCamera* cam, int32_t P, const float* means3D, const float* shs, const float* colors_precomp,
                              const float* logit_opacities, const float* log_scales, const float* unnorm_rotations,
                              const float* h_pose7, int32_t isotropic, float* max_2D_radius, uint8_t* seen, int32_t* radii, void* geom_state,
                              void* image_state, uint32_t* d_counts, uint32_t* h_counts, int32_t want_backward, gs_stream_t stream);
int gs_render_backward_raw(const GsCamera* cam, int32_t P, int64_t D, const float* means3D, const float* shs, const float* colors_precomp,
                           const float* logit_opacities, const float* log_scales, const float* unnorm_rotations, const float* h_pose7,
                           int32_t isotropic, int32_t accumulate, const int32_t* radii, const void* geom_state, const uint32_t* point_list,
                           const void* image_state, const float* dL_dcolor, const float* dL_ddepth, float* dL_dmeans2D, float* dL_dmeans3D,
                           float* dL_dlogit_opacities, float* dL_dcolors_precomp, float* dL_dshs, float* dL_dlog_scales,
                           float* dL_dunnorm_rotations, void* scratch, int32_t scratch_zeroed, int32_t have_sh_jacobian, gs_stream_t stream);

uint64_t gs_pose_grad_scratch_bytes(int32_t P);
int gs_render_backward_raw_pose(const GsCamera* cam, int32_t P, int64_t D, const float* means3D, const float* shs, const float* colors_precomp,
                                const float* logit_opacities, const float* log_scales, const float* unnorm_rotations, const float* h_pose7,
                                int32_t isotropic, int32_t accumulate, const int32_t* radii, const void* geom_state, const uint32_t* point_list,
                                const void* image_state, const float* dL_dcolor, const float* dL_ddepth, float* dL_dmeans2D, float* dL_dmeans3D,
                                float* dL_dlogit_opacities, float* dL_dcolors_precomp, float* dL_dshs, float* dL_dlog_scales,
                                float* dL_dunnorm_rotations, void* scratch, int32_t scratch_zeroed, int32_t have_sh_jacobian, int32_t pose_only,
                                float* dL_dpose7, void* pose_scratch, gs_stream_t stream);

typedef struct GsImageGrads {
    const float* dL_dcolor;
    const float* dL_ddepth;
    const float* dL_dopacity;
    const float* dL_ddepth_sq;
} GsImageGrads;
int gs_render_backward_grads(const GsCamera* cam, int32_t P, int64_t D,
                             const float* means3D, const float* shs, const float* colors_precomp,
                             const float* scales, const float* rotations, const float* cov3D_precomp,
                             const int32_t* radii, const void* geom_state, const uint32_t* point_list,
                             const void* image_state, const GsImageGrads* grads,
                             float* dL_dmeans2D, float* dL_dmeans3D, float* dL_dopacities,
                             float* dL_dcolors_precomp, float* dL_dshs, float* dL_dscales,
                             float* dL_drotations, float* dL_dcov3D, void* scratch, int32_t scratch_zeroed,
                             int32_t have_sh_jacobian, gs_stream_t stream);
int gs_render_backward_raw_grads(const GsCamera* cam, int32_t P, int64_t D, const float* means3D, const float* shs, const float* colors_precomp,
                                 const float* logit_opacities, const float* log_scales, const float* unnorm_rotations, const float* h_pose7,
                                 int32_t isotropic, int32_t accumulate, const int32_t* radii, const void* geom_state, const uint32_t* point_list,
                                 const void* image_state, const GsImageGrads* grads, float* dL_dmeans2D, float* dL_dmeans3D,
                                 float* dL_dlogit_opacities, float* dL_dcolors_precomp, float* dL_dshs, float* dL_dlog_scales,
                                 float* dL_dunnorm_rotations, void* scratch, int32_t scratch_zeroed, int32_t have_sh_jacobian, gs_stream_t stream);
int gs_render_backward_raw_pose_grads(const GsCamera* cam, int32_t P, int64_t D, const float* means3D, const float* shs, const float* colors_precomp,
                                      const float* logit_opacities, const float* log_scales, const float* unnorm_rotations, const float* h_pose7,
                                      int32_t isotropic, int32_t accumulate, const int32_t* radii, const void* geom_state,
                                      const uint32_t* point_list, const void* image_state, const GsImageGrads* grads, float* dL_dmeans2D,
                                      float* dL_dmeans3D, float* dL_dlogit_opacities, float* dL_dcolors_precomp, float* dL_dshs,
                                      float* dL_dlog_scales, float* dL_dunnorm_rotations, void* scratch, int32_t scratch_zeroed,
                                      int32_t have_sh_jacobian, int32_t pose_only, float* dL_dpose7, void* pose_scratch, gs_stream_t stream);

int gs_adam_step(int64_t n, float* param, const float* grad, float* exp_avg, float* exp_avg_sq,
                 double lr, double beta1, double beta2, double eps, int32_t step, gs_stream_t stream);

typedef struct GsAdamTensor {
    int64_t n;
// ... 201 lines not shown
```

Measured before the change: 1562 frames/s.

## Pack per-tile 4x4 sub-block coverage masks into sorted point list IDs

During tile binning, each Gaussian's tile entry gets an 8-bit mask of which 4-pixel row and column bands its extent touches, packed into the low bits of the ID. A list-format word records the shift. Forward and backward blend kernels use these masks to skip geometry loads and per-block overlap tests, replacing scan_blocks with cheap bit ops. This adds preprocessing work (box computation, fallback geom reads for wide Gaussians), caps P below 2^24, and disables half-quadrant mode when active. Python capture paths unpack the IDs.

```diff
diff --git a/activesplat_amd/_lib.py b/activesplat_amd/_lib.py
--- a/activesplat_amd/_lib.py
+++ b/activesplat_amd/_lib.py
@@ -23,7 +23,7 @@
 
 
 class GsImageLayout(C.Structure):
-    _fields_ = [(n, C.c_uint64) for n in ("total_bytes", "ranges", "final_T", "n_contrib", "split_state")]
+    _fields_ = [(n, C.c_uint64) for n in ("total_bytes", "ranges", "final_T", "n_contrib", "split_state", "list_format")]
 
 
 class GsAdamTensor(C.Structure):
@@ -67,7 +67,7 @@
 SORT_AUTO, SORT_TILE_LDS, SORT_RADIX = 0, 1, 2
 
 
-ABI_VERSION = 23
+ABI_VERSION = 24
 
 vp, i32, u32, i64, u64, f32, f64, cint = C.c_void_p, C.c_int32, C.c_uint32, C.c_int64, C.c_uint64, C.c_float, C.c_double, C.c_int
 
@@ -83,6 +83,8 @@
     "gs_set_backward_chain_tickets": (cint, [i32]),
     "gs_set_backward_chain_polls": (cint, [i32]),
     "gs_set_forward_priority": (cint, [i32, f32]),
+    "gs_set_block_masks": (cint, [i32]),
+    "gs_block_masks_query": (i32, [i32, i32, i32, i32, u32, i32]),
     "gs_async_status_word": (cint, [C.POINTER(C.POINTER(u32))]),
     "gs_async_status_clear": (cint, []),
     "gs_recorded_cut": (cint, [u32, C.POINTER(u32), C.POINTER(i32)]),
diff --git a/activesplat_amd/csrc/api.hip b/activesplat_amd/csrc/api.hip
--- a/activesplat_amd/csrc/api.hip
+++ b/activesplat_amd/csrc/api.hip
@@ -102,6 +102,7 @@
     k.bg = c->bg; k.view = c->viewmatrix; k.proj = c->projmatrix; k.campos = c->campos;
     k.half = 0; k.split = 0;
     k.act = k.act_iso = k.act_accumulate = 0;
+    k.list_shift = 0; k.use_masks = 0; k.list_format = nullptr;
     return true;
 }
 
@@ -123,6 +124,7 @@
     g.tile_total = (uint32_t*)(b + L.tile_total); g.tile_base = (uint32_t*)(b + L.tile_base);
     g.sh_jac = (float2*)(b + L.sh_jac);
     g.depth_bits = (uint32_t*)(b + L.depth_bits);
+    g.box = g.offsets; g.list_format = nullptr;
     g.vis_max = nullptr; g.vis_seen = nullptr;
     return g;
 }
@@ -201,6 +203,24 @@
     gs::g_fwd_prio_param = param > 0.0f ? param : 0.0f;
     gs::g_fwd_prio = mode;
     return GS_OK;
+}
+
+int gs_set_block_masks(int32_t mode)
+{
+    if (mode > gs::kMaskDefault) return fail(GS_EINVAL, "gs_set_block_masks: mode out of range");
+    gs::g_block_masks = mode < 0 ? gs::kMaskDefault : mode;
+    return GS_OK;
+}
+
+int32_t gs_block_masks_query(int32_t P, int32_t width, int32_t height, int32_t num_views, uint32_t max_tile_instances, int32_t topdown)
+{
+    if (P < 0 || width <= 0 || height <= 0 || num_views > 1 || topdown) return 0;
+    gs::Cam k;
+    k.V = 1; k.gx = tiles_across(width); k.gy = tiles_across(height);
+    if (!gs::block_masks_frame(k, P)) return 0;
+    GsBinLayout BL;
+    if (gs_bin_layout(1, max_tile_instances, width, height, &BL) != GS_OK) return 0;
+    return BL.path == GS_SORT_TILE_LDS && BL.segments <= 1 ? 1 : 0;
 }
 
 int gs_async_status_word(uint32_t** host_word)
@@ -297,7 +317,8 @@
     out->final_T = o; o = align_up(o + hw * 4);
     out->n_contrib = o; o = align_up(o + hw * 4);
     out->split_state = o; o = align_up(o + (tiles <= (uint64_t)gs::kFewTiles ? ((uint64_t)gs::kCutLevels * 5 + 4) * hw + 4
-                                             : (uint64_t)gs::chain_state_words(tiles)) * 4);
+                                             : (uint64_t)gs::chain_state_words(tiles) + 1) * 4);
+    out->list_format = tiles <= (uint64_t)gs::kFewTiles ? 0 : out->split_state + (uint64_t)gs::chain_state_words(tiles) * 4;
     out->total_bytes = o;
     return GS_OK;
 }
@@ -396,6 +417,7 @@
     gs::GeomPtrs gp = carve_geom(c.geom_state, Pv, k);
     if (!(c.want_backward && in.shs)) gp.sh_jac = nullptr;
     gp.vis_max = k.act ? c.max_2D_radius : nullptr; gp.vis_seen = k.act ? c.seen : nullptr;
+    if (!gs::block_masks_possible(k, Pv) || c.pose.source == gs::POSE_BAND) gp.box = nullptr;
     GsImageLayout IL; gs_image_layout(k.W, k.H, &IL);
     uint2* ranges = (uint2*)((char*)c.image_state + IL.ranges);
     const int tiles = k.gx * k.gy;
@@ -534,6 +556,12 @@
     uint2* ranges = (uint2*)(ib + IL.ranges);
     GsBinLayout BL; gs_bin_layout(D, max_tile_instances, k.W, k.H, &BL);
     char* bb = (char*)bin_state;
+    k.list_shift = (BL.path == GS_SORT_TILE_LDS && BL.segments <= 1 && gs::block_masks_frame(k, P)) ? gs::kMaskBits : 0;
+    k.use_masks = k.list_shift ? (gs::g_block_masks.load(std::memory_order_relaxed) & gs::kMaskFwd) : 0;
+    gp.list_format = IL.list_format ? (uint32_t*)(ib + IL.list_format) : nullptr;
+    if (BL.path != GS_SORT_TILE_LDS && gp.list_format) {
+        if (int rc = launched("gs_render_forward", "memset", hipMemsetAsync(gp.list_format, 0, sizeof(uint32_t), st))) return rc;
+    }
     if (int rc = bin_tile_lists("gs_render_forward", k, P, D, max_tile_instances, gp, ranges, BL, bb, point_list, st)) return rc;
     ScopedStage ps(ST_BLEND_FWD, st);
     return launched("gs_render_forward", "blend", gs::launch_blend_forward(k, ranges, point_list, gp.geom, out_color, out_depth, out_opacity,
@@ -661,6 +689,8 @@
     if (int rc = launched("gs_render_backward", "memset", e)) return rc;
     if (c.D > 0) {
         ScopedStage ps(ST_BLEND_BWD, st);
+        k.list_format = IL.list_format ? (const uint32_t*)(ib + IL.list_format) : nullptr;
+        k.use_masks = gs::g_block_masks.load(std::memory_order_relaxed) & gs::kMaskBwd;
         e = gs::launch_blend_backward(k, (const uint2*)(ib + IL.ranges), c.point_list, gp.geom,
                                       (const float*)(ib + IL.split_state),
                                       (const float*)(ib + IL.final_T),
diff --git a/activesplat_amd/csrc/blend.hip b/activesplat_amd/csrc/blend.hip
--- a/activesplat_amd/csrc/blend.hip
+++ b/activesplat_amd/csrc/blend.hip
@@ -249,13 +249,17 @@
     bool done = !inside || stopped_at_entry;
 
     if (SEG == 1 || !__all(done)) {
+        const int sh = SEG == 0 ? cam.list_shift : 0;
+        const bool mk = SEG == 0 && cam.use_masks != 0;
+        const int quad_u = __builtin_amdgcn_readfirstlane(c.quad);
         uint32_t id_next = first + (uint32_t)lane < n ? list[first + lane] : kNoId;
         uint32_t id_next2 = first + (uint32_t)lane + 64u < n ? list[first + lane + 64] : kNoId;
-        if (id_next >= P) id_next = kNoId;
-        if (id_next2 >= P) id_next2 = kNoId;
+        if ((id_next >> sh) >= P) id_next = kNoId;
+        if ((id_next2 >> sh) >= P) id_next2 = kNoId;
         float4 r0 = make_float4(0.f, 0.f, 0.f, 0.f), r1 = r0, r2 = make_float4(0.f, 0.f, -1.f, -1.f);
         if (first < n) {
-            const float4* gr = geom + (size_t)(id_next != kNoId ? id_next : 0u) * 3;
+            const bool want = id_next != kNoId && (!mk || block_mask_quadrant(id_next, quad_u) != 0u);
+            const float4* gr = geom + (size_t)(want ? id_next >> sh : 0u) * 3;
             r0 = gr[0]; r1 = gr[1]; r2 = gr[2];
         }
         for (uint32_t base = first; base < n; base += kWave) {
@@ -285,17 +289,34 @@
             const uint32_t id_cur = id_next;
             id_next = id_next2;
             id_next2 = base + 128u + (uint32_t)lane < n ? list[base + 128u + lane] : kNoId;
-            if (id_next2 >= P) id_next2 = kNoId;
-            {
-                const float4* gr = geom + (size_t)(id_next != kNoId ? id_next : 0u) * 3;
+            if ((id_next2 >> sh) >= P) id_next2 = kNoId;
+            const unsigned long long going = SEG == 1 ? ~0ull : ~__ballot(done);
+            if (mk) {
+                const unsigned gate = ((going & 0xffffull) != 0ull ? 1u : 0u) | ((going & 0xffff0000ull) != 0ull ? 2u : 0u) |
+                                      ((going & 0xffff00000000ull) != 0ull ? 4u : 0u) | ((going >> 48) != 0ull ? 8u : 0u);
+                const unsigned hn = id_next != kNoId ? block_mask_quadrant(id_next, quad_u) & gate : 0u;
+                if (__ballot(hn != 0u) != 0ull) {
+                    const float4* gr = geom + (size_t)(hn != 0u ? id_next >> sh : 0u) * 3;
+                    r0 = gr[0]; r1 = gr[1]; r2 = gr[2];
+                }
+            } else {
+                const float4* gr = geom + (size_t)(id_next != kNoId ? id_next >> sh : 0u) * 3;
                 r0 = gr[0]; r1 = gr[1]; r2 = gr[2];
             }
 
-            const unsigned long long going = SEG == 1 ? ~0ull : ~__ballot(done);
             unsigned long long m_any, mb[4];
-            scan_going_blocks(q0, q2, id_cur != kNoId, c.qx0, c.qy0, going, m_any, mb);
+            if (mk) {
+                const unsigned hc = id_cur != kNoId ? block_mask_quadrant(id_cur, quad_u) : 0u;
+                mb[0] = (going & 0xffffull) != 0ull ? __ballot((hc & 1u) != 0u) : 0ull;
+                mb[1] = (going & 0xffff0000ull) != 0ull ? __ballot((hc & 2u) != 0u) : 0ull;
+                mb[2] = (going & 0xffff00000000ull) != 0ull ? __ballot((hc & 4u) != 0u) : 0ull;
+                mb[3] = (going >> 48) != 0ull ? __ballot((hc & 8u) != 0u) : 0ull;
+                m_any = (mb[0] | mb[1]) | (mb[2] | mb[3]);
+            } else {
+                scan_going_blocks(q0, q2, id_cur != kNoId, c.qx0, c.qy0, going, m_any, mb);
+            }
             if (m_any == 0ull) continue;
-            stage_record(s0, s1, s2, lane, q0, q1, q2, id_cur);
+            stage_record(s0, s1, s2, lane, q0, q1, q2, id_cur >> sh);
             const int ntrips = build_stream_lists(s_list[wave], mb, lane);
             __builtin_amdgcn_wave_barrier();
             uint32_t jj2_next = *reinterpret_cast<const uint16_t*>(my_list);
@@ -790,10 +811,14 @@
     const uint8_t* list_b = s_list[wave] + rb * kWave + tb;
 
     const int cmax = ctop;
+    int sh = 0;
+    if (!FEW && cam.list_format) sh = __builtin_amdgcn_readfirstlane((int)*cam.list_format);
+    const bool mk = !FEW && sh != 0 && cam.use_masks != 0;
+    const int quad_u = __builtin_amdgcn_readfirstlane(c.quad);
     uint32_t id_next = (cmax >= cmin && (uint32_t)cmax * kWave + lane < wmax) ? list[cmax * kWave + lane] : kNoId;
     uint32_t id_next2 = cmax >= cmin + 1 ? list[(cmax - 1) * kWave + lane] : kNoId;
     float4 r0 = make_float4(0.f, 0.f, 0.f, 0.f), r1 = r0, r2 = make_float4(0.f, 0.f, -1.f, -1.f);
-    if (id_next != kNoId) { r0 = geom[(size_t)id_next * 3]; r1 = geom[(size_t)id_next * 3 + 1]; r2 = geom[(size_t)id_next * 3 + 2]; }
+    if (id_next != kNoId) { const size_t i0 = (size_t)(id_next >> sh) * 3; r0 = geom[i0]; r1 = geom[i0 + 1]; r2 = geom[i0 + 2]; }
     if (pieces > 1 && piece > 0) {
         int polls = 0;
         bool handed = cam.chain_polls >= 0;
@@ -820,13 +845,21 @@
         id_next = id_next2;
         id_next2 = ch >= cmin_u + 2 ? list[(ch - 2) * kWave + lane] : kNoId;
         {
-            const float4* gr = geom + (size_t)(id_next != kNoId ? id_next : 0u) * 3;
+            const bool want = id_next != kNoId && (!mk || block_mask_quadrant(id_next, quad_u) != 0u);
+            const float4* gr = geom + (size_t)(want ? id_next >> sh : 0u) * 3;
             r0 = gr[0]; r1 = gr[1]; r2 = gr[2];
         }
 
         const uint32_t cpos = (uint32_t)ch * kWave;
         unsigned long long m_any;
-        const unsigned hf = scan_blocks(q0, q2, id_cur != kNoId && lane < upto, c.qx0, c.qy0, cpos < rm0, cpos < rm1, cpos < rm2, cpos < rm3, m_any);
+        unsigned hf;
+        if (mk) {
+            const unsigned gate = (cpos < rm0 ? 1u : 0u) | (cpos < rm1 ? 2u : 0u) | (cpos < rm2 ? 4u : 0u) | (cpos < rm3 ? 8u : 0u);
+            hf = (id_cur != kNoId && lane < upto) ? block_mask_quadrant(id_cur, quad_u) & gate : 0u;
+            m_any = __ballot(hf != 0u);
+        } else {
+            hf = scan_blocks(q0, q2, id_cur != kNoId && lane < upto, c.qx0, c.qy0, cpos < rm0, cpos < rm1, cpos < rm2, cpos < rm3, m_any);
+        }
         const int n_hit = (int)__popcll(m_any);
         bool split = false;
         if (m_any != 0ull) {
@@ -840,7 +873,7 @@
                 const StagedConic k = staged_conic(q0, q1);
                 s0[slot] = k.s0;
                 s1[slot] = make_float4(k.c, q1.y, q1.z, q1.w);
-                s2[slot] = make_float4(q2.x, __uint_as_float(cpos + (uint32_t)lane), q2.y, __uint_as_float(id_cur));
+                s2[slot] = make_float4(q2.x, __uint_as_float(cpos + (uint32_t)lane), q2.y, __uint_as_float(id_cur >> sh));
                 s_flag[wave][slot] = (uint8_t)hf;
             }
             cnt = __builtin_amdgcn_readfirstlane(cnt + n_stage);
@@ -1018,6 +1051,7 @@
 std::atomic<int> g_chain_polls{kChainPollsDefault};
 std::atomic<int> g_fwd_prio{kFwdPrioDefault};
 std::atomic<float> g_fwd_prio_param{kFwdPrioDefaultParam};
+std::atomic<int> g_block_masks{kMaskDefault};
 uint32_t* g_async_status_dev = nullptr;
 uint32_t* g_chain_fail_dev = nullptr;
 int g_chain_fail_device = -1;
@@ -1040,6 +1074,7 @@
     Cam cam = cam_in;
     const int k_half = g_half_quadrant_tiles.load(std::memory_order_relaxed), k_fseg = g_few_segments.load(std::memory_order_relaxed);
     cam.half = (segments <= 1 || !seg_T) && cam.gx * cam.gy <= k_half;
+    if (cam.list_shift) cam.half = 0;
     cam.split = (cam.V == 1 && split_state && cam.gx * cam.gy <= min(k_half, kFewTiles)) && k_fseg > 1 ? k_fseg : 0;
     cam.chain = (cam.V == 1 && split_state && cam.gx * cam.gy > kFewTiles) ? kChainPieces : 0;
     cam.fwd_prio = g_fwd_prio.load(std::memory_order_relaxed);
diff --git a/activesplat_amd/csrc/gs_common.h b/activesplat_amd/csrc/gs_common.h
--- a/activesplat_amd/csrc/gs_common.h
+++ b/activesplat_amd/csrc/gs_common.h
@@ -42,6 +42,8 @@
     uint32_t* chain_fail;
     int act, act_iso, act_accumulate;
     float act_q[4], act_t[3];
+    int list_shift, use_masks;
+    const uint32_t* list_format;
 };
 
 struct CamDP : Cam {
@@ -172,7 +174,58 @@
     float2* sh_jac;
     float* vis_max;
     uint8_t* vis_seen;
-};
+    uint32_t* box;
+    uint32_t* list_format;
+};
+
+constexpr int kMaskBits = 8;
+constexpr uint32_t kMaskMaxP = 1u << (32 - kMaskBits);
+constexpr int kBoxMaxTiles = 15;
+constexpr uint32_t kBoxNone = 0xffffffffu;
+__host__ __device__ __forceinline__ uint32_t block_box_lo(float l, int X0, int S)
+{
+    return l <= (float)(X0 + S) ? (l > (float)X0 ? (uint32_t)(int)(ceilf(l) - (float)X0) : 0u) : (uint32_t)S;
+}
+__host__ __device__ __forceinline__ uint32_t block_box_hi(float h, int X0, int S)
+{
+    return h >= (float)X0 ? (h < (float)(X0 + S) ? (uint32_t)(int)(floorf(h) - (float)(X0 - 1)) : (uint32_t)S) : 0u;
+}
+__host__ __device__ __forceinline__ uint32_t block_box(float x, float y, float ex, float ey, int x0, int y0, int x1, int y1)
+{
+    if (!(ex >= 0.0f)) return 0u;
+    const int X0 = x0 * kTile, Y0 = y0 * kTile, Sx = (x1 - x0) * kTile, Sy = (y1 - y0) * kTile;
+    return block_box_lo(x - ex, X0, Sx) | (block_box_hi(x + ex, X0, Sx) << 8) | (block_box_lo(y - ey, Y0, Sy) << 16) | (block_box_hi(y + ey, Y0, Sy) << 24);
+}
+__host__ __device__ __forceinline__ uint32_t block_mask(uint32_t box, int kx, int ky)
+{
+    const int xl = (int)(box & 0xffu), xh = (int)((box >> 8) & 0xffu) - 1, yl = (int)((box >> 16) & 0xffu), yh = (int)(box >> 24) - 1;
+    const int ex = kx * kTile, ey = ky * kTile;
+    uint32_t m = 0;
+#pragma unroll
+    for (int j = 0; j < 4; j++) {
+        m |= (xh >= ex + 4 * j && xl <= ex + 4 * j + 3) ? 1u << j : 0u;
+        m |= (yh >= ey + 4 * j && yl <= ey + 4 * j + 3) ? 16u << j : 0u;
+    }
+    return m;
+}
+__host__ __device__ __forceinline__ uint32_t block_mask_record(float x, float y, float ex, float ey, int tx0, int ty0)
+{
+    const float xl = x - ex, xh = x + ex, yl = y - ey, yh = y + ey;
+    if (!(ex >= 0.0f)) return 0u;
+    uint32_t m = 0;
+#pragma unroll
+    for (int j = 0; j < 4; j++) {
+        const float e0 = (float)(tx0 + 4 * j), e1 = (float)(ty0 + 4 * j);
+        m |= (xh >= e0 && xl <= e0 + 3.0f) ? 1u << j : 0u;
+        m |= (yh >= e1 && yl <= e1 + 3.0f) ? 16u << j : 0u;
+    }
+    return m;
+}
+__host__ __device__ __forceinline__ uint32_t block_mask_quadrant(uint32_t mask, int quad)
+{
+    const uint32_t xq = (mask >> (2 * (quad & 1))) & 3u, yq = (mask >> (4 + 2 * (quad >> 1))) & 3u;
+    return ((yq & 1u) ? xq : 0u) | ((yq & 2u) ? xq << 2 : 0u);
+}
 
 #ifndef GS_WAIT_VMEM
 #define GS_WAIT_VMEM() asm volatile("s_waitcnt vmcnt(0)" ::: "memory")
@@ -666,6 +719,18 @@
 }
 extern std::atomic<int> g_few_segments;
 constexpr int kFewTiles = 256;
+constexpr int kMaskFwd = 1, kMaskBwd = 2, kMaskDefault = kMaskFwd | kMaskBwd;
+extern std::atomic<int> g_block_masks;
+inline bool block_masks_possible(const Cam& cam, int64_t P)
+{
+    const int tiles = cam.gx * cam.gy;
+    return cam.V == 1 && P > 0 && P < (int64_t)kMaskMaxP && tiles > kFewTiles && tiles <= kMaxLdsTiles && cam.gx < 2048 && cam.gy < 2048;
+}
+inline bool block_masks_frame(const Cam& cam, int64_t P)
+{
+    return block_masks_possible(cam, P) && g_block_masks.load(std::memory_order_relaxed) != 0 &&
+           cam.gx * cam.gy > g_half_quadrant_tiles.load(std::memory_order_relaxed);
+}
 constexpr int kChainPieces = 3;
 constexpr int kChainMinTiles = 768;
 constexpr int kChainStateFloats = (kChainPieces - 1) * 2 * kWave;
diff --git a/activesplat_amd/csrc/preprocess.hip b/activesplat_amd/csrc/preprocess.hip
--- a/activesplat_amd/csrc/preprocess.hip
+++ b/activesplat_amd/csrc/preprocess.hip
@@ -148,6 +148,10 @@
             gp.geom[(size_t)io * 3] = g0; gp.geom[(size_t)io * 3 + 1] = g1; gp.geom[(size_t)io * 3 + 2] = g2;
             gp.rect[io] = rc;
             gp.depth_bits[io] = __float_as_uint(g2.y);
+            if (gp.box) {
+                const int bx0 = (int)(rc.x & 0xffffu), bx1 = (int)(rc.x >> 16), by0 = (int)(rc.y & 0xffffu), by1 = (int)(rc.y >> 16);
+                if (bx1 - bx0 <= kBoxMaxTiles && by1 - by0 <= kBoxMaxTiles) gp.box[io] = block_box(g0.x, g0.y, g2.z, g2.w, bx0, by0, bx1, by1);
+            }
         }
         gp.tiles[io] = ntiles;
         if (HAS_SH && !gp.sh_jac) gp.clamped[io] = clampbits;
diff --git a/activesplat_amd/csrc/tilebin.hip b/activesplat_amd/csrc/tilebin.hip
--- a/activesplat_amd/csrc/tilebin.hip
+++ b/activesplat_amd/csrc/tilebin.hip
@@ -20,14 +20,13 @@
             const uint32_t k = t - (lo ? incl_w[lo - 1] : 0u);
             const uint32_t xw = s_x0w[j];
             const uint32_t w = xw >> 16, x0 = xw & 0xffffu;
-            const uint32_t tile = (s_y0[j] + k / w) * (uint32_t)gx + x0 + k % w;
-            f(tile, j);
+            f(x0 + k % w, s_y0[j] + k / w, k % w, k / w, j);
         }
     }
 }
 
 template <bool SCATTER, int THREADS>
-__global__ __launch_bounds__(THREADS) void tile_bin_kernel(Cam cam, int P, GeomPtrs gp, int tiles, int chunk,
+__global__ __launch_bounds__(THREADS, SCATTER ? 8 : 1) void tile_bin_kernel(Cam cam, int P, GeomPtrs gp, int tiles, int chunk,
                                                           uint32_t* __restrict__ tile_total,
                                                           uint32_t* __restrict__ tile_base,
                                                           const uint2* __restrict__ ranges,
@@ -38,6 +37,7 @@
     __shared__ uint32_t s_x0w[THREADS];
     __shared__ uint32_t s_y0[THREADS];
     __shared__ uint32_t s_depth[THREADS];
+    __shared__ uint32_t s_box[SCATTER ? kBinChunk : 1];
 
     const int tid = threadIdx.x, lane = tid & 63, wave = tid >> 6;
   const int cper = (nchunks + 7) >> 3;
@@ -49,13 +49,17 @@
     constexpr int kBinRounds = SCATTER ? kBinChunk / THREADS : 1, kBinCursorRounds = SCATTER ? 2 : 1;
     uint32_t rn[kBinRounds], rd[kBinRounds], cur[kBinCursorRounds];
     uint2 rr[kBinRounds];
+    uint32_t rb[kBinRounds];
+    const bool masked = SCATTER && cam.list_shift != 0;
     if (SCATTER) {
+        if (gp.list_format && b == 0 && tid == 0) *gp.list_format = (uint32_t)cam.list_shift;
 #pragma unroll
         for (int q = 0; q < kBinRounds; q++) {
             const int ic = min(cbase + q * THREADS + tid, P - 1);
             rn[q] = gp.tiles[ic];
             rr[q] = gp.rect[ic];
             rd[q] = gp.depth_bits[ic];
+            rb[q] = masked ? gp.box[ic] : 0u;
         }
 #pragma unroll
         for (int k = 0; k < kBinCursorRounds; k++) {
@@ -67,6 +71,13 @@
     if (SCATTER) {
 #pragma unroll
         for (int k = 0; k < kBinCursorRounds; k++) if (tid + k * THREADS < tiles) s_hist[tid + k * THREADS] = cur[k];
+        if (masked) {
+#pragma unroll
+            for (int q = 0; q < kBinRounds; q++) {
+                const bool wide = (rr[q].x >> 16) - (rr[q].x & 0xffffu) > (uint32_t)kBoxMaxTiles || (rr[q].y >> 16) - (rr[q].y & 0xffffu) > (uint32_t)kBoxMaxTiles;
+                s_box[q * THREADS + tid] = wide ? kBoxNone : rb[q];
+            }
+        }
         for (int t = tid + kBinCursorRounds * THREADS; t < tiles; t += THREADS) s_hist[t] = ranges[t].x + my_base[t];
     } else {
         for (int t = tid; t < tiles; t += THREADS) s_hist[t] = 0u;
@@ -76,6 +87,7 @@
         const int i = cbase + r * THREADS + tid;
         if (cbase + r * THREADS >= P) break;
         uint32_t n = 0, x0 = 0, w = 1, y0 = 0, dbits = 0;
+        uint32_t box = 0u;
         if (SCATTER) {
             uint32_t pn = rn[0], pd = rd[0];
             uint2 prc = rr[0];
@@ -83,6 +95,7 @@
             for (int q = 1; q < kBinRounds; q++) if (r == q) { pn = rn[q]; pd = rd[q]; prc = rr[q]; }
             n = i < P ? pn : 0u;
             if (n) { x0 = prc.x & 0xffffu; w = (prc.x >> 16) - x0; y0 = prc.y & 0xffffu; dbits = pd; }
+            if (masked) box = s_box[r * THREADS + tid];
         } else if (i < P) {
             n = gp.tiles[i];
             if (n) {
@@ -92,8 +105,18 @@
             }
         }
         const int gbase = cbase + r * THREADS;
-        auto place = [&](uint32_t tile, uint32_t depth_bits, uint32_t id) {
+        auto place = [&](uint32_t tx, uint32_t ty, uint32_t kx, uint32_t ky, uint32_t depth_bits, uint32_t id, uint32_t bx) {
+            const uint32_t tile = ty * (uint32_t)cam.gx + tx;
             if (SCATTER) {
+                if (masked) {
+                    uint32_t m;
+                    if (bx != kBoxNone) m = block_mask(bx, (int)kx, (int)ky);
+                    else {
+                        const float4 q0 = gp.geom[(size_t)id * 3], q2 = gp.geom[(size_t)id * 3 + 2];
+                        m = block_mask_record(q0.x, q0.y, q2.z, q2.w, (int)tx * kTile, (int)ty * kTile);
+                    }
+                    id = (id << kMaskBits) | m;
+                }
                 const uint32_t slot = atomicAdd(&s_hist[tile], 1u);
                 if (slot < cap) pairs[slot] = ((unsigned long long)depth_bits << 32) | id;
             } else {
@@ -104,7 +127,7 @@
             uint32_t kx = 0, ky = 0;
             for (uint32_t k = 0; __any(k < n); k++) {
                 if (k < n) {
-                    place((y0 + ky) * (uint32_t)cam.gx + x0 + kx, dbits, (uint32_t)i);
+                    place(x0 + kx, y0 + ky, kx, ky, dbits, (uint32_t)i, box);
                     if (++kx == w) { kx = 0; ++ky; }
                 }
             }
@@ -119,8 +142,8 @@
         s_incl[tid] = incl;
         const uint32_t total = __shfl(incl, 63);
         __builtin_amdgcn_wave_barrier();
-        expand_wave(s_incl + wave * kWave, s_x0w, s_y0, wave, lane, total, cam.gx, [&](uint32_t tile, int j) {
-            place(tile, SCATTER ? s_depth[j] : 0u, (uint32_t)(gbase + j));
+        expand_wave(s_incl + wave * kWave, s_x0w, s_y0, wave, lane, total, cam.gx, [&](uint32_t tx, uint32_t ty, uint32_t kx, uint32_t ky, int j) {
+            place(tx, ty, kx, ky, SCATTER ? s_depth[j] : 0u, (uint32_t)(gbase + j), masked ? s_box[r * THREADS + j] : 0u);
         });
         __builtin_amdgcn_wave_barrier();
     }
diff --git a/activesplat_amd/rasterizer.py b/activesplat_amd/rasterizer.py
--- a/activesplat_amd/rasterizer.py
+++ b/activesplat_amd/rasterizer.py
@@ -109,6 +109,15 @@
                         keep["bg"].data_ptr(), keep["view"].data_ptr(), keep["proj"].data_ptr(),
                         keep["campos"].data_ptr())
     return cam, keep
+
+
+def _clean_point_list(image, il, point_list, D, P, W, H, max_tile):
+    if D <= 0 or not _lib.get().gs_block_masks_query(P, W, H, 1, max_tile, 0):
+        return point_list, 0
+    shift = int(image[il.list_format:il.list_format + 4].view(torch.int32).item()) if il.list_format else 0
+    if shift != 8:
+        return point_list, 0
+    return (point_list >> 8) & 0xFFFFFF, 8
 
 
 def _capture_target():
@@ -295,7 +304,9 @@
             ctx.adam = (adam, leaves[:4] + (shs_in if shs_in is not None else leaves[4],))
         cap = _capture_target()
         if cap is not None:
-            cap.update(geom=geom, image=image, binning=binning, point_list=point_list, gl=fr.gl, il=fr.il, bl=bl, D=D, P=P, W=W, H=H)
+            clean, shift = _clean_point_list(image, fr.il, point_list, D, P, W, H, max_tile)
+            cap.update(geom=geom, image=image, binning=binning, point_list=clean, gl=fr.gl, il=fr.il, bl=bl, D=D, P=P, W=W, H=H,
+                       point_list_packed=point_list, list_shift=shift)
         e = torch.empty(0, device=device)
         ctx.save_for_backward(means3D, shs if shs is not None else e, colors_precomp if colors_precomp is not None else e,
                               scales if scales is not None else e, rotations if rotations is not None else e,
@@ -501,8 +512,11 @@
         ws, binning, plist2 = state
         cap_d, cap_tile = (guess if hit else (D, max_tile))
         bl = _lib.GsBinLayout(); _lib.check(lib.gs_bin_layout(cap_d, cap_tile, W, H, C.byref(bl)))
-        cap.update(geom=ws[off[0]:off[0] + off[1]], image=ws[off[2]:off[2] + off[3]], gl=gl, il=il, bl=bl, D=D, P=P, W=W, H=H, binning=binning,
-                   point_list=ws[off[4]:off[4] + 4 * off[5]].view(torch.int32) if hit else plist2)
+        geom_v, image_v = ws[off[0]:off[0] + off[1]], ws[off[2]:off[2] + off[3]]
+        packed = ws[off[4]:off[4] + 4 * off[5]].view(torch.int32) if hit else plist2
+        clean, shift = _clean_point_list(image_v, il, packed, D, P, W, H, max_tile)
+        cap.update(geom=geom_v, image=image_v, gl=gl, il=il, bl=bl, D=D, P=P, W=W, H=H, binning=binning,
+                   point_list=clean, point_list_packed=packed, list_shift=shift)
     _record_launch(key, guess, hit, D, max_tile, P)
     return tuple(out)
 
diff --git a/include/gsplat_hip.h b/include/gsplat_hip.h
--- a/include/gsplat_hip.h
+++ b/include/gsplat_hip.h
@@ -53,6 +53,7 @@
     uint64_t final_T;
     uint64_t n_contrib;
     uint64_t split_state;
+    uint64_t list_format;
 } GsImageLayout;
 
 #define GS_SORT_AUTO 0
@@ -83,6 +84,8 @@
 int gs_set_backward_chain_tickets(int32_t on);
 int gs_set_backward_chain_polls(int32_t polls);
 int gs_set_forward_priority(int32_t mode, float param);
+int gs_set_block_masks(int32_t mode);
+int32_t gs_block_masks_query(int32_t P, int32_t width, int32_t height, int32_t num_views, uint32_t max_tile_instances, int32_t topdown);
 int gs_async_status_word(uint32_t** host_word);
 int gs_async_status_clear(void);
 int gs_recorded_cut(uint32_t target, uint32_t* nearest, int32_t* level);
@@ -91,7 +94,7 @@
 
 const char* gs_last_error(void);
 const char* gs_version(void);
-#define GS_ABI_VERSION 23
+#define GS_ABI_VERSION 24
 int32_t gs_abi_version(void);
 
 int gs_profile_enable(int32_t on);
```

Result: no change. 1567 frames/s (median of 2 runs) (+0.3%).
